# KarolinaBenkova/FEM-FCT-PDECO

Measured on AMD Instinct MI355X. Metric: FCT timesteps/sec (fwd+adj), higher is better.
Workload: dtype f64; 1 GPU; C2 advection_solidbody_FCT_PDECO_finaltime: [-1,1]^2 81x81 P1 (dx=0.025, n=6561), dt=1e-3, 250 fwd + 250 adj FCT steps per cost+gradient evaluation; nodes=6561, num_steps=250, batch_per_gpu=1, parallelism=single trajectory, low_order_solver=jacobi, jacobi_sweeps_max=26, graphs=True, graph_replay=True, kernel_regime=2

## Files before the change

fem-fct-pdeco_amd/_lib.py:

```python
from __future__ import annotations

import ctypes as C
import os

_HERE = os.path.dirname(os.path.abspath(__file__))
LIB_PATH = os.environ.get("FEMFCT_LIB") or os.path.join(_HERE, "lib", "libfemfct.so")

OK, ERR_INVALID, ERR_HIP, ERR_NOT_CONVERGED, ERR_NOMEM = 0, 1, 2, 3, 4
FLAG_MMATRIX_ROWSUM, FLAG_SOLVER_BUDGET, FLAG_COARSE_ITERS, FLAG_CHEBYSHEV, FLAG_ROW_PAIRS = 1, 2, 4, 8, 16
ORDER_VERTEX, ORDER_FENICS = 0, 1
SOLVER_JACOBI, SOLVER_BICGSTAB = 0, 1
REGIME_ROWS, REGIME_STRIPS, REGIME_TILE32, REGIME_PATCH64, REGIME_MESH = 0, 1, 2, 3, 4
ABI_VERSION = 5
MAX_TRIALS = 16
MAX_MEMBERS = 256
MAX_GRAM_FIELDS = 17
MAX_ZONES = 256


class FemFctError(RuntimeError):
    def __init__(self, code, msg):
        super().__init__(f"libfemfct error {code}: {msg}")
        self.code = code


class FemFctValueError(FemFctError, ValueError):
    pass


class NotConverged(FemFctError):
    pass


class StepInfo(C.Structure):
    _fields_ = [("flags", C.c_int32), ("solver_iters", C.c_int32),
                ("solver_resid", C.c_double), ("min_rowsum", C.c_double)]


def _load():
    if not os.path.exists(LIB_PATH):
        raise ImportError(
            f"{LIB_PATH} not found: the HIP library is not built. Run "
            "`python -c 'import __graft_entry__ as g; g.build()'` or "
            "`make -C fem-fct-pdeco_amd/csrc` (needs hipcc, --offload-arch=gfx950). "
            "There is no CPU fallback.")
    lib = C.CDLL(LIB_PATH)
    if lib.femfct_abi_version() != ABI_VERSION:
        raise ImportError("libfemfct.so ABI version mismatch: rebuild the library")
    return lib


lib = _load()

_p = C.c_void_p
_d = C.c_double
_i = C.c_int32
_dp = C.POINTER(C.c_double)
_ip = C.POINTER(C.c_int32)

SIGNATURES = {
    "femfct_abi_version": (C.c_int, []),
    "femfct_build_id": (C.c_char_p, []),
    "femfct_create": (C.c_int, [C.POINTER(_p), C.c_int]),
    "femfct_destroy": (C.c_int, [_p]),
    "femfct_last_error": (C.c_char_p, [_p]),
    "femfct_synchronize": (C.c_int, [_p]),
    "femfct_stream": (_p, [_p]),
    "femfct_set_solver": (C.c_int, [_p, C.c_int, _d, C.c_int]),
    "femfct_set_graphs": (C.c_int, [_p, C.c_int]),
    "femfct_graph_replay_active": (C.c_int, [_p, C.POINTER(C.c_int)]),
    "femfct_rotation_derived": (C.c_int, [_p, C.POINTER(C.c_int)]),
    "femfct_launch_info": (C.c_int, [_p, C.POINTER(C.c_int32)]),
    "femfct_set_fusion": (C.c_int, [_p, C.c_int, C.c_int]),
    "femfct_kernel_regime": (C.c_int, [_p, _i]),
    "femfct_patch_walkers": (C.c_int, [_p, _i, _i]),
    "femfct_lowop_nonzero_fraction": (C.c_int, [_p, _dp]),
    "femfct_set_profiling": (C.c_int, [_p, C.c_int]),
    "femfct_profile_report": (C.c_int, [_p, _p, _p, _i]),
    "femfct_malloc": (C.c_int, [_p, C.POINTER(_p), C.c_size_t]),
    "femfct_free": (C.c_int, [_p, _p]),
    "femfct_memcpy_h2d": (C.c_int, [_p, _p, _p, C.c_size_t]),
    "femfct_memcpy_d2h": (C.c_int, [_p, _p, _p, C.c_size_t]),
    "femfct_memcpy_d2d": (C.c_int, [_p, _p, _p, C.c_size_t]),
    "femfct_memset0": (C.c_int, [_p, _p, C.c_size_t]),
    "femfct_set_pattern_csr": (C.c_int, [_p, _i, _p, _p]),
    "femfct_set_mesh_square": (C.c_int, [_p, _d, _d, _i, _i]),
    "femfct_n": (_i, [_p]),
    "femfct_ell_width": (_i, [_p]),
    "femfct_get_ell_cols": (C.c_int, [_p, _p]),
    "femfct_csr_to_ell": (C.c_int, [_p, _p, _p]),
    "femfct_ell_to_csr": (C.c_int, [_p, _p, _p]),
    "femfct_set_mass": (C.c_int, [_p, _p, _p]),
    "femfct_mass_ell": (_p, [_p]),
    "femfct_stiffness_ell": (_p, [_p]),
    "femfct_lumped_mass": (_p, [_p]),
    "femfct_fct_step": (C.c_int, [_p, _p, _p, _i, _p, _p, _d, _p, _i]),
    "femfct_last_step_info": (C.c_int, [_p, C.POINTER(StepInfo), _i]),
    "femfct_fct_step_host": (C.c_int, [_p, _p, _p, _p, _p, _d, _p, C.POINTER(StepInfo)]),
    "femfct_chebsi": (C.c_int, [_p, _p, _p, _i, _d, _d, _i]),
    "femfct_chebsi_md": (C.c_int, [_p, _p, _p, _p, _i, _d, _d, _i]),
    "femfct_artificial_diffusion": (C.c_int, [_p, _p, _p, _i]),
    "femfct_spmv": (C.c_int, [_p, _p, _p, _d, _d, _p, _i]),
    "femfct_mesh_quad_points": (C.c_int, [_p, _p, _p]),
    "femfct_assemble_convection": (C.c_int, [_p, _p, _d, _p]),
    "femfct_assemble_rotation": (C.c_int, [_p, _d, _p]),
    "femfct_drift_gradient_rhs": (C.c_int, [_p, _p, _p, _p, _d, _d, _d, _p, _i]),
    "femfct_solidbody_forward": (C.c_int, [_p, _p, _p, _i, _p, _i, _d, _d, _d, _d, _d, _i]),
    "femfct_solidbody_forward_src": (C.c_int, [_p, _p, _p, _i, _p, _p, _i, _d, _d, _d, _d, _d, _i]),
    "femfct_solidbody_adjoint": (C.c_int, [_p, _p, _p, _i, _p, _p, _p, _i, _d, _d, _d, _d, _d, _i, _i]),
    "femfct_linear_forward_react": (C.c_int, [_p, _p, _p, _p, _p, _i, _d, _d, _i]),
    "femfct_linear_adjoint_react": (C.c_int, [_p, _p, _p, _p, _p, _p, _i, _d, _d, _i, _i]),
    "femfct_react_load": (C.c_int, [_p, _p, _p, _p, _p, _i]),
    "femfct_solidbody_adjoint_obs": (C.c_int, [_p, _p, _p, _i, _p, _p, _p, _d, _p, _p, _i, _d, _d, _d, _d, _d, _i]),
    "femfct_linear_adjoint_react_obs": (C.c_int, [_p, _p, _p, _p, _p, _p, _d, _p, _p, _i, _d, _d, _i]),
    "femfct_nonlinear_adjoint_obs": (C.c_int, [_p, _p, _p, _p, _p, _d, _p, _p, _i, _d, _d, _i]),
    "femfct_schnak_adjoint_obs": (C.c_int, [_p, _p, _p, _p, _p, _p, _p, _p, _d, _p, _d, _p, _p, _p, _i, _d, _p, _i]),
    "femfct_chtxs_adjoint_obs": (C.c_int, [_p, _p, _p, _p, _p, _p, _d, _p, _d, _p, _p, _p, _p, _i, _d, _p, _d, _p, _i, _i]),
    "femfct_obs_load": (C.c_int, [_p, _p, _p, _p, _i, _d, _p, _p, _i]),
    "femfct_obs_cost": (C.c_int, [_p, _p, _p, _p, _p, _i, _i, _p]),
    "femfct_solidbody_adjoint_bounds": (C.c_int, [_p, _p, _p, _i, _p, _p, _p, _d, _p, _p, _p, _d, _p, _p, _p, _i, _d, _d, _d,
                                                  _d, _d, _i]),
    "femfct_linear_adjoint_react_bounds": (C.c_int, [_p, _p, _p, _p, _p, _p, _d, _p, _p, _p, _d, _p, _p, _p, _i, _d, _d, _i]),
    "femfct_bound_load": (C.c_int, [_p, _p, _p, _p, _p, _i, _d, _p, _p, _p, _p, _p, _d, _p, _p, _i]),
    "femfct_bound_cost": (C.c_int, [_p, _p, _p, _p, _p, _d, _p, _i, _i, _p]),
    "femfct_assemble_weighted_mass": (C.c_int, [_p, _p, _p]),
    "femfct_traj_info": (C.c_int, [_p, C.POINTER(StepInfo), _i, _i]),
    "femfct_descent_pointwise": (C.c_int, [_p, C.c_int64, _d, _p, _d, _p, _p, _d, _p]),
    "femfct_ell_transpose": (C.c_int, [_p, _p, _p]),
    "femfct_axpby": (C.c_int, [_p, C.c_int64, _d, _p, _d, _p, _p]),
    "femfct_set_krylov": (C.c_int, [_p, _d, _i]),
    "femfct_set_species_solver": (C.c_int, [_p, _i]),
    "femfct_bicgstab": (C.c_int, [_p, _p, _i, _p, _p, _p, _i, C.POINTER(StepInfo)]),
    "femfct_nonlinear_forward": (C.c_int, [_p, _p, _p, _p, _i, _d, _d, _i]),
    "femfct_nonlinear_adjoint": (C.c_int, [_p, _p, _p, _p, _p, _i, _d, _d, _i]),
    "femfct_schnak_forward": (C.c_int, [_p, _p, _p, _p, _p, _i, _d, _p, _d, _i]),
    "femfct_schnak_adjoint": (C.c_int, [_p, _p, _p, _p, _p, _p, _p, _p, _i, _d, _p, _i, _i]),
    "femfct_schnak_forward_tw": (C.c_int, [_p, _p, _p, _p, _p, _p, _i, _d, _p, _d, _i]),
    "femfct_schnak_adjoint_tw": (C.c_int, [_p, _p, _p, _p, _p, _p, _p, _p, _p, _i, _d, _p, _i, _i]),
    "femfct_chtxs_forward": (C.c_int, [_p, _p, _p, _p, _i, _d, _p, _d, _i]),
    "femfct_nonlinear_forward_ct": (C.c_int, [_p, _p, _p, _i, _p, _i, _d, _d, _i]),
    "femfct_schnak_forward_ct": (C.c_int, [_p, _p, _p, _p, _i, _p, _p, _i, _d, _p, _d, _i]),
    "femfct_chtxs_forward_ct": (C.c_int, [_p, _p, _i, _p, _p, _i, _d, _p, _d, _i]),
    "femfct_chtxs_forward_g": (C.c_int, [_p, _p, _i, _i, _p, _p, _i, _d, _p, _d, _p, _i]),
    "femfct_chtxs_adjoint_g": (C.c_int, [_p, _p, _p, _p, _p, _p, _p, _p, _i, _d, _p, _d, _i, _p, _i]),
    "femfct_nonlinear_adjoint_alltime": (C.c_int, [_p, _p, _p, _p, _i, _p, _i, _d, _d, _i]),
    "femfct_chtxs_adjoint": (C.c_int, [_p, _p, _p, _p, _p, _p, _p, _p, _i, _d, _p, _d, _i, _i]),
    "femfct_traj_krylov_info": (C.c_int, [_p, C.POINTER(StepInfo), _i, _i]),
    "femfct_l2_norm_sq_Q": (C.c_int, [_p, _p, _p, _i, _d, _p, _i]),
    "femfct_l2_norm_sq_Omega": (C.c_int, [_p, _p, _p, _p, _i]),
    "femfct_cost_functional": (C.c_int, [_p, _p, _p, _p, _i, _i, _d, _d, _i, _p, _p, _p, _i]),
    "femfct_project_control": (C.c_int, [_p, _p, _d, _p, _d, _d, _p, C.c_int64]),
    "femfct_linear_trial_costs": (C.c_int, [_p, _p, _p, _p, _p, _p, _d, _i, _d, _d, _d, _i, _d, _i, _p, _p]),
    "femfct_source_trials": (C.c_int, [_p, _p, _p, _p, _d, _i, _d, _d, C.c_int64, _p, _p]),
    "femfct_trial_controls": (C.c_int, [_p, _p, _p, _p, _i, _i, _d, _d, C.c_int64, _p]),
    "femfct_member_costs": (C.c_int, [_p, _p, _p, _i, _p, _p, _p, _i, _i, _i, _d, _i, _p, _p]),
    "femfct_time_restrict": (C.c_int, [_p, _p, _p, _i, _i, _i, _p]),
    "femfct_time_prolong": (C.c_int, [_p, _p, _p, _i, _i, _i, _p]),
    "femfct_free_set": (C.c_int, [_p, _p, _p, _d, _d, C.c_int64, _p]),
    "femfct_q_gram": (C.c_int, [_p, _p, _i, _p, _i, _d, _p]),
    "femfct_q_combine": (C.c_int, [_p, _p, _p, _i, _p, _p, _d, C.c_int64, _p]),
    "femfct_prox_trials": (C.c_int, [_p, _p, _p, _p, _d, _i, _d, _d, _d, C.c_int64, _p, _p]),
    "femfct_l1_norm_Q": (C.c_int, [_p, _p, _i, _d, _p, _i]),
    "femfct_sparse_trial_stats": (C.c_int, [_p, _p, _p, _i, _i, _d, _p, _p, _p]),
    "femfct_ensemble_drift_gradient_rhs": (C.c_int, [_p, _p, _p, _p, _p, _i, _d, _d, _d, _p, _i]),
    "femfct_ensemble_costs": (C.c_int, [_p, _p, _p, _p, _p, _p, _p, _p, _i, _d, _i, _d, _p, _p, _p]),
    "femfct_initial_trials": (C.c_int, [_p, _p, _p, _p, _i, _d, _d, _p, _i]),
    "femfct_initial_trial_stats": (C.c_int, [_p, _p, _p, _p, _i, _i, _p]),
    "femfct_initial_gradient": (C.c_int, [_p, _p, _p, _p, _d, _p, _d, _d, _p]),
    "femfct_omega_gram": (C.c_int, [_p, _p, _i, _p, _p]),
    "femfct_set_control_zones": (C.c_int, [_p, _p, _i]),
    "femfct_zone_restrict": (C.c_int, [_p, _p, C.c_int64, _i, _p]),
    "femfct_zone_prolong": (C.c_int, [_p, _p, _p, C.c_int64, _p]),
    "femfct_smooth_cost": (C.c_int, [_p, _p, _i, _d, _p, _i]),
    "femfct_smooth_rhs": (C.c_int, [_p, _p, _d, _d, _i, _d, _p, _i]),
    "femfct_drift_gradient_rhs_smooth": (C.c_int, [_p, _p, _p, _p, _d, _d, _d, _d, _p, _i, _d, _d]),
}

for _name, (_res, _args) in SIGNATURES.items():
    _fn = getattr(lib, _name)
    _fn.restype = _res
    _fn.argtypes = _args


def check(ctx_handle, code):
    if code == OK:
        return
    msg = lib.femfct_last_error(ctx_handle)
    msg = msg.decode() if msg else ""
    if code == ERR_INVALID:
        raise FemFctValueError(code, msg)
    if code == ERR_NOT_CONVERGED:
        raise NotConverged(code, msg)
    raise FemFctError(code, msg)
```

fem-fct-pdeco_amd/csrc/ctx.hip:

```cpp
#include "femfct_internal.h"
#include "build_id.h"
#include "device_utils.h"

#include <dlfcn.h>
#include <stdarg.h>
#include <stdio.h>
#include <stdlib.h>
#include <string.h>
#include <algorithm>
#include <tuple>

int femfct_enqueue_artdiff(femfct_ctx* ctx, const double* K, double* D, int32_t batch);
int femfct_enqueue_spmv(femfct_ctx* ctx, const double* A, const double* x, double alpha, double beta, double* y,
                        int32_t batch);
int femfct_enqueue_cheb(femfct_ctx* ctx, const double* b, double* y_out, int iters, double lmin, double lmax,
                        int32_t batch, bool first_done_in_y1, const double* mdv = nullptr);
int femfct_mesh_release(femfct_ctx* ctx);
int femfct_build_structured_csr(femfct_ctx* ctx);

int femfct_fail(femfct_ctx* ctx, int code, const char* fmt, ...) {
    char buf[1024];
    va_list ap;
    va_start(ap, fmt);
    vsnprintf(buf, sizeof buf, fmt, ap);
// ... 87 lines not shown
    dev_free(&ctx->d_wscale); ctx->wscale_count = 0;
    dev_free(&ctx->d_zero_traj); ctx->zero_traj_count = 0;
    dev_free(&ctx->d_trMat); dev_free(&ctx->d_trBase); dev_free(&ctx->d_trBase2); dev_free(&ctx->d_trRhs2); dev_free(&ctx->d_trTmp);
    ctx->implicit_cols = false;
    ctx->n = 0; ctx->W = 0; ctx->nnz_csr = 0; ctx->ws_batch = 0; ctx->have_mass = false; ctx->structured = false; ctx->mass_is_mesh = false;
    ctx->sweep_budget = std::min(femfct_ctx().sweep_budget, ctx->max_iters);
    femfct_forget_jacobi_budgets(ctx);
}

void femfct_prof_begin(femfct_ctx* ctx, int cls) {
    if (!ctx->prof_on) return;
    femfct_ctx::ProfRec r;
    r.cls = cls;
    hipEventCreate(&r.a);
    hipEventCreate(&r.b);
    hipEventRecord(r.a, ctx->stream);
    ctx->prof.push_back(r);
}

void femfct_prof_end(femfct_ctx* ctx) {
    if (!ctx->prof_on || ctx->prof.empty()) return;
    hipEventRecord(ctx->prof.back().b, ctx->stream);
}

void femfct_drop_graphs(femfct_ctx* ctx) {
    for (auto& kv : ctx->graphs) hipGraphExecDestroy(kv.second);
    ctx->graphs.clear();
}

int femfct_ensure_workspace(femfct_ctx* ctx, int32_t batch) {
    if (ctx->solver == FEMFCT_SOLVER_BICGSTAB) {
        int rk = femfct_ensure_krylov_ws(ctx, batch);
        if (rk != FEMFCT_OK) return rk;
    }
#ifdef FEMFCT_TUNING
    if (!ctx->d_mesh_trace && getenv("FEMFCT_MESH_TRACE"))
        HIP_TRY(ctx, hipMalloc((void**)&ctx->d_mesh_trace, 16 * sizeof(unsigned long long)));
#endif
    if (!ctx->d_zero && ctx->n > 0) {
        int rz = dev_alloc(ctx, &ctx->d_zero, (size_t)ctx->n);
        if (rz != FEMFCT_OK) return rz;
        HIP_TRY(ctx, hipMemsetAsync(ctx->d_zero, 0, sizeof(double) * ctx->n, ctx->stream));
    }
    if (batch <= ctx->ws_batch) return FEMFCT_OK;
    femfct_drop_graphs(ctx);
    size_t nv = (size_t)batch * ctx->n, nm = nv * ctx->W;
    int rc;
#define A_(p, c) if ((rc = dev_alloc(ctx, &ctx->p, (c))) != FEMFCT_OK) return rc
    A_(d_L, nm + 1); A_(d_D, nm); A_(d_F, nm);
    HIP_TRY(ctx, hipMemsetAsync(ctx->d_L + nm, 0, sizeof(double), ctx->stream));
    A_(d_b, nv); A_(d_xa, nv); A_(d_xb, nv); A_(d_du, nv); A_(d_y0, nv); A_(d_y1, nv); A_(d_y2, nv);
    A_(d_rdu, nv); A_(d_rp, nv); A_(d_rm, nv);
    A_(d_part, (size_t)batch * 4 * FEMFCT_MAX_PARTIALS);
    A_(d_ctl, (size_t)batch);
    A_(d_partk, (size_t)batch * 16 * FEMFCT_MAX_PARTIALS);
    {
        const size_t words = ((size_t)batch * (size_t)ctx->n + 7) / 8 + 1;
        A_(d_Lmask, words);
        HIP_TRY(ctx, hipMemsetAsync(ctx->d_Lmask, 0, words * 8, ctx->stream));
    }
    {
        TilePlan tp;
        ctx->bigpart_count = 0;
        if (femfct_tile_plan(ctx, &tp, false) && femfct_tile_big(ctx, tp)) {
            ctx->bigpart_count = (int64_t)tp.tiles * tp.tiles;
            A_(d_bigpart, (size_t)batch * ctx->bigpart_count);
        }
    }
#undef A_
    HIP_TRY(ctx, hipMemsetAsync(ctx->d_ctl, 0, sizeof(StepCtl) * batch, ctx->stream));
    ctx->ws_batch = batch;
    return FEMFCT_OK;
}

static int fusion_mode(const femfct_ctx* ctx, int* K) {
    TilePlan tp;
    if (femfct_tile_plan(ctx, &tp, false)) {
        *K = tp.K;
        return femfct_tile_big(ctx, tp) ? 1 : 2;
    }
    StripPlan pl;
    if (femfct_strip_plan(ctx, &pl)) { *K = pl.K; return 1; }
    *K = 1;
    return 0;
}

int femfct_fused_k(const femfct_ctx* ctx) {
    int K;
    fusion_mode(ctx, &K);
    return K;
}

int femfct_next_budget(const femfct_ctx* ctx, int worst, bool coarse) {
    int K;
    const int mode = fusion_mode(ctx, &K);
    int b;
    if (mode == 2) b = std::max(worst, 1) + ((coarse || !ctx->exact_iters) ? 0 : 1);
    else if (mode == 1) b = std::max(worst, 1);
    else b = std::max(8, worst + worst / 8 + 2);
    return std::min(ctx->max_iters, b);
}

int femfct_grow_budget(const femfct_ctx* ctx, int budget) {
    int K;
    const int mode = fusion_mode(ctx, &K);
    if (mode == 2) return std::min(ctx->max_iters, budget + 2);
    if (mode == 1) return std::min(ctx->max_iters, budget + K);
    return std::min(ctx->max_iters, budget * 2);
}

int femfct_round_budget(const femfct_ctx* ctx, int b) {
    int K;
    if (fusion_mode(ctx, &K) == 0) b = (b + 3) & ~3;
    if (b < 1) b = 1;
    if (b > ctx->max_iters) b = ctx->max_iters;
    return b;
}

int femfct_install_pattern(femfct_ctx* ctx, int32_t n, int32_t W, const std::vector<int32_t>& cols,
                           const std::vector<uint8_t>& tslot) {
    int rc;
    ctx->n = n;
    ctx->W = W;
    if ((rc = dev_alloc(ctx, &ctx->d_cols, (size_t)W * n)) != FEMFCT_OK) return rc;
    if ((rc = dev_alloc(ctx, &ctx->d_tslot, (size_t)W * n)) != FEMFCT_OK) return rc;
    HIP_TRY(ctx, hipMemcpy(ctx->d_cols, cols.data(), sizeof(int32_t) * W * n, hipMemcpyHostToDevice));
    HIP_TRY(ctx, hipMemcpy(ctx->d_tslot, tslot.data(), sizeof(uint8_t) * W * n, hipMemcpyHostToDevice));
    if ((rc = dev_alloc(ctx, &ctx->d_M, (size_t)W * n)) != FEMFCT_OK) return rc;
    if ((rc = dev_alloc(ctx, &ctx->d_ml, (size_t)n)) != FEMFCT_OK) return rc;
    ctx->h_cols = cols;
    int32_t bwmax = 0;
    for (int32_t s = 1; s < W; ++s)
        for (int32_t i = 0; i < n; ++i) {
            int32_t d = cols[(size_t)s * n + i] - i;
            if (d < 0) d = -d;
            if (d > bwmax) bwmax = d;
        }
    ctx->bandwidth = bwmax;
    if (const char* e = getenv("FEMFCT_STRIPS")) ctx->use_strips = atoi(e) != 0;
    if (const char* e = getenv("FEMFCT_STRIP_K")) ctx->strip_k = atoi(e);
    if (const char* e = getenv("FEMFCT_TILES")) ctx->use_tiles = atoi(e) != 0;
    if (const char* e = getenv("FEMFCT_EXACT")) ctx->exact_iters = atoi(e) != 0;
    if (const char* e = getenv("FEMFCT_FUSE_BUILD")) ctx->fuse_build = atoi(e) != 0;
    if (const char* e = getenv("FEMFCT_PREASSEMBLE")) ctx->preassemble = atoi(e) != 0;
    if (const char* e = getenv("FEMFCT_PREASSEMBLE_MAX_GB")) ctx->preassemble_max_bytes = atof(e) * 1024.0 * 1024.0 * 1024.0;
    if (const char* e = getenv("FEMFCT_PREBUILD_LOW")) ctx->prebuild_low = atoi(e) != 0;
    if (const char* e = getenv("FEMFCT_WG_SLOTS")) ctx->wg_slots = std::max(1, atoi(e));
    if (const char* e = getenv("FEMFCT_DEEP_HALO")) ctx->deep_halo = atoi(e) != 0;
    if (const char* e = getenv("FEMFCT_FUSE_FLUX")) ctx->fuse_flux = atoi(e) != 0;
    if (const char* e = getenv("FEMFCT_FUSE_DUDT")) ctx->fuse_dudt = atoi(e) != 0;
    if (const char* e = getenv("FEMFCT_TILE_LEAN")) ctx->tile_lean = atoi(e) != 0;
    if (const char* e = getenv("FEMFCT_TILE_CONE")) ctx->tile_cone = atoi(e) != 0;
    if (const char* e = getenv("FEMFCT_TILE_FIT")) ctx->tile_fit = atoi(e) != 0;
    if (const char* e = getenv("FEMFCT_FUSE_END")) ctx->fuse_end = atoi(e) != 0;
    if (const char* e = getenv("FEMFCT_TILE4")) ctx->tile4_mode = atoi(e);
    if (const char* e = getenv("FEMFCT_LMASK")) ctx->l_mask = atoi(e) != 0;
    if (const char* e = getenv("FEMFCT_T4_XCD")) ctx->t4_xcd = atoi(e) != 0;
    if (const char* e = getenv("FEMFCT_T4_WALK")) ctx->t4_walk = atoi(e);
    if (const char* e = getenv("FEMFCT_T4_SNAKE")) ctx->t4_snake = atoi(e) != 0;
    if (const char* e = getenv("FEMFCT_T4_PAIR")) ctx->t4_pair = atoi(e) != 0;
#ifdef FEMFCT_TUNING
    if (const char* e = getenv("FEMFCT_PAIR_SHAPE")) ctx->pair_shape = atoi(e);
    if (const char* e = getenv("FEMFCT_PAIR_PRIO")) ctx->pair_prio = atoi(e);
    if (const char* e = getenv("FEMFCT_PAIR_SPLIT")) ctx->pair_split = std::min(90, std::max(10, atoi(e)));
    if (getenv("FEMFCT_PAIR_TRACE") && !ctx->d_pair_trace) {
        if (hipMalloc((void**)&ctx->d_pair_trace, sizeof(unsigned long long) * (FEMFCT_MAX_PARTIALS * 16 * 5 + 16)) == hipSuccess)
            hipMemset(ctx->d_pair_trace, 0, sizeof(unsigned long long) * (FEMFCT_MAX_PARTIALS * 16 * 5 + 16));
    }
    if (const char* e = getenv("FEMFCT_PAIR_STAGGER_US")) ctx->pair_stagger = (int)(atof(e) * 100.0);
#endif
    if (const char* e = getenv("FEMFCT_DEFER_CHECK")) ctx->defer_check = atoi(e) != 0;
    if (const char* e = getenv("FEMFCT_T4_INT")) ctx->t4_int = atoi(e) != 0;
    if (const char* e = getenv("FEMFCT_T4_WALKERS")) { int v = atoi(e); if (v > 0) ctx->num_cus = v; }
    if (const char* e = getenv("FEMFCT_INLINE_OPS")) ctx->inline_ops = atoi(e) != 0;
    if (const char* e = getenv("FEMFCT_HALF_D")) ctx->half_d = atoi(e) != 0;
    if (const char* e = getenv("FEMFCT_T4_STAGGER_US")) {
        const double us = atof(e);
        int pat = 7;
        if (const char* p = getenv("FEMFCT_T4_STAGGER_PAT")) pat = atoi(p);
        ctx->t4_stagger = us > 0 ? ((int)(us * 100.0) & 0xffffff) | ((pat & 15) << 24) : 0;
    }
    if (const char* e = getenv("FEMFCT_SINGLE_PATCH_BATCH")) { int v = atoi(e); ctx->single_patch_min_batch = v > 0 ? v : (1 << 30); }
    if (const char* e = getenv("FEMFCT_MESH_SOLVE")) ctx->mesh_solve = atoi(e) != 0;
    if (const char* e = getenv("FEMFCT_GEOM_MASS")) ctx->geom_mass = atoi(e) != 0;
    if (const char* e = getenv("FEMFCT_GEOM_ROT")) ctx->geom_rot = atoi(e) != 0;
    if (const char* e = getenv("FEMFCT_FORM_GROUPS")) ctx->form_groups = atoi(e) != 0;
    if (const char* e = getenv("FEMFCT_MESH_STEP")) ctx->mesh_step = atoi(e) != 0;
    if (const char* e = getenv("FEMFCT_MESH_STEP_BATCH")) ctx->mesh_step_min_batch = std::max(1, atoi(e));
    if (const char* e = getenv("FEMFCT_MESH_STEP_BATCH_LARGE")) ctx->mesh_step_min_batch_large = std::max(1, atoi(e));
    if (const char* e = getenv("FEMFCT_T4_DPP")) ctx->t4_dpp = atoi(e) != 0;
    if (const char* e = getenv("FEMFCT_T4_K")) ctx->t4_k = std::min(8, std::max(1, atoi(e)));
    if (const char* e = getenv("FEMFCT_SPECIES_SOLVER")) ctx->species_solver = atoi(e);
    if (const char* e = getenv("FEMFCT_STEPS_PER_GRAPH")) ctx->steps_per_graph = std::max(1, atoi(e));
    return femfct_strip_init(ctx);
}

static int build_csr_map(femfct_ctx* ctx) {
    const int32_t n = ctx->n, W = ctx->W;
    ctx->nnz_csr = ctx->h_indptr[n];
    ctx->h_csr2ell.assign(ctx->nnz_csr, 0);
    for (int32_t i = 0; i < n; ++i) {
        for (int32_t k = ctx->h_indptr[i]; k < ctx->h_indptr[i + 1]; ++k) {
            int32_t j = ctx->h_indices[k];
            int32_t s_found = -1;
            if (j == i) s_found = 0;
            else
                for (int32_t s = 1; s < W; ++s)
                    if (ctx->h_cols[(size_t)s * n + i] == j) { s_found = s; break; }
            if (s_found < 0) return femfct_fail(ctx, FEMFCT_ERR_INVALID, "CSR entry (%d,%d) not in the ELL pattern", i, j);
            ctx->h_csr2ell[k] = (int32_t)((size_t)s_found * n + i);
        }
    }
    int rc;
    if ((rc = dev_alloc(ctx, &ctx->d_csr2ell, (size_t)ctx->nnz_csr)) != FEMFCT_OK) return rc;
    HIP_TRY(ctx, hipMemcpy(ctx->d_csr2ell, ctx->h_csr2ell.data(), sizeof(int32_t) * ctx->nnz_csr, hipMemcpyHostToDevice));
    if ((rc = dev_alloc(ctx, &ctx->d_hcsr, (size_t)ctx->nnz_csr)) != FEMFCT_OK) return rc;
    return FEMFCT_OK;
}

extern "C" {

int femfct_abi_version(void) { return FEMFCT_ABI_VERSION; }
const char* femfct_build_id(void) { return FEMFCT_BUILD_ID; }

}

bool femfct_profiler_attached() {
    for (const char* name : {"librocprofiler-sdk.so.1", "librocprofiler-sdk.so"}) {
        if (void* h = dlopen(name, RTLD_LAZY | RTLD_NOLOAD)) {
            dlclose(h);
            return true;
        }
    }
    return false;
}

extern "C" {

int femfct_create(femfct_ctx** out, int device_id) {
    if (!out) return FEMFCT_ERR_INVALID;
    *out = nullptr;
    int count = 0;
    if (hipGetDeviceCount(&count) != hipSuccess || count <= 0) return FEMFCT_ERR_HIP;
    if (device_id < 0 || device_id >= count) return FEMFCT_ERR_INVALID;
    if (hipSetDevice(device_id) != hipSuccess) return FEMFCT_ERR_HIP;
    femfct_ctx* ctx = new (std::nothrow) femfct_ctx();
    if (!ctx) return FEMFCT_ERR_NOMEM;
    ctx->device = device_id;
    {
        int cus = 0;
        if (hipDeviceGetAttribute(&cus, hipDeviceAttributeMultiprocessorCount, device_id) == hipSuccess && cus > 0) ctx->num_cus = cus;
    }
    if (hipStreamCreateWithFlags(&ctx->stream, hipStreamNonBlocking) != hipSuccess) {
        delete ctx;
        return FEMFCT_ERR_HIP;
    }
    const char* pg = getenv("FEMFCT_PROFILER_GRAPHS");
    ctx->profiler_graphs_ok = pg && atoi(pg) != 0;
    if (!ctx->profiler_graphs_ok && femfct_profiler_attached()) ctx->graphs_blocked = true;
    *out = ctx;
    return FEMFCT_OK;
}

int femfct_graph_replay_active(const femfct_ctx* ctx, int* active_host) {
    if (!ctx || !active_host) return FEMFCT_ERR_INVALID;
    *active_host = (ctx->use_graphs && !ctx->prof_on && !ctx->graphs_blocked) ? 1 : 0;
    return FEMFCT_OK;
}

int femfct_rotation_derived(const femfct_ctx* ctx, int* derived_host) {
    if (!ctx || !derived_host) return FEMFCT_ERR_INVALID;
    *derived_host = ctx->last_rot_geom ? 1 : 0;
    return FEMFCT_OK;
}

int femfct_destroy(femfct_ctx* ctx) {
    if (!ctx) return FEMFCT_OK;
    hipSetDevice(ctx->device);
    hipStreamSynchronize(ctx->stream);
    if (ctx->d_pair_trace) {
        if (const char* path = getenv("FEMFCT_PAIR_TRACE")) {
            std::vector<unsigned long long> h((size_t)FEMFCT_MAX_PARTIALS * 16 * 5 + 16);
            if (hipMemcpy(h.data(), ctx->d_pair_trace, h.size() * sizeof(unsigned long long), hipMemcpyDeviceToHost) == hipSuccess)
                if (FILE* f = fopen(path, "wb")) { fwrite(h.data(), sizeof(unsigned long long), h.size(), f); fclose(f); }
        }
        hipFree(ctx->d_pair_trace);
        ctx->d_pair_trace = nullptr;
    }
#ifdef FEMFCT_TUNING
    if (const char* path = getenv("FEMFCT_TILE_TRACE")) femfct_tile_phase_dump(path);
#endif
    femfct_release_pattern(ctx);
    hipStreamDestroy(ctx->stream);
    delete ctx;
    return FEMFCT_OK;
}

const char* femfct_last_error(const femfct_ctx* ctx) { return ctx ? ctx->err.c_str() : "null context"; }

int femfct_synchronize(femfct_ctx* ctx) {
    FEMFCT_ENTER(ctx);
    ARG_TRY(ctx, ctx, "null ctx");
    HIP_TRY(ctx, hipStreamSynchronize(ctx->stream));
    return FEMFCT_OK;
}

void* femfct_stream(femfct_ctx* ctx) { return ctx ? (void*)ctx->stream : nullptr; }

int femfct_set_solver(femfct_ctx* ctx, int solver, double rel_tol, int max_iters) {
    FEMFCT_ENTER(ctx);
    ARG_TRY(ctx, ctx, "null ctx");
    ARG_TRY(ctx, solver == FEMFCT_SOLVER_JACOBI || solver == FEMFCT_SOLVER_BICGSTAB, "unknown solver");
    ARG_TRY(ctx, rel_tol > 0 && rel_tol < 1 && max_iters >= 1, "bad tolerance / iteration cap");
    ctx->solver = solver;
    ctx->solver_user = solver;
    femfct_forget_bicgstab_handovers(ctx);
    ctx->rel_tol = rel_tol;
    ctx->max_iters = max_iters;
    if (ctx->sweep_budget > max_iters) ctx->sweep_budget = max_iters;
    femfct_forget_jacobi_budgets(ctx);
    femfct_drop_graphs(ctx);
    return FEMFCT_OK;
}

int femfct_set_fusion(femfct_ctx* ctx, int strips, int tiles) {
    FEMFCT_ENTER(ctx);
    ARG_TRY(ctx, ctx, "null ctx");
    HIP_TRY(ctx, hipStreamSynchronize(ctx->stream));
    ctx->use_strips = strips != 0;
    ctx->use_tiles = tiles != 0;
    femfct_drop_graphs(ctx);
    femfct_forget_jacobi_budgets(ctx);
    ctx->ws_batch = 0;
    return FEMFCT_OK;
}

int femfct_kernel_regime(const femfct_ctx* ctx, int32_t batch) {
    if (!ctx || ctx->n <= 0) return -1;
    if (femfct_mesh_step_wanted(ctx, batch)) return FEMFCT_REGIME_MESH;
    if (femfct_tile4_wanted(ctx, batch)) return FEMFCT_REGIME_PATCH64;
    TilePlan tp;
    if (ctx->use_strips && femfct_tile_plan(ctx, &tp, true, 0, batch)) return FEMFCT_REGIME_TILE32;
    StripPlan sp;
    if (femfct_strip_plan(ctx, &sp)) return FEMFCT_REGIME_STRIPS;
    return FEMFCT_REGIME_ROWS;
}

int femfct_patch_walkers(const femfct_ctx* ctx, int32_t batch, int32_t sweeps) {
    if (!ctx || ctx->n <= 0 || batch < 1 || !femfct_tile4_wanted(ctx, batch) || femfct_single_patch(ctx, batch)) return 0;
    return femfct_tile4_walkers(ctx, femfct_tile4_halo(ctx, sweeps > 0 ? sweeps : 36), batch, false);
}

int femfct_launch_info(const femfct_ctx* ctx, int32_t* out4_host) {
    if (!ctx || !out4_host) return FEMFCT_ERR_INVALID;
    for (int k = 0; k < 4; ++k) out4_host[k] = ctx->last_launch[k];
    return FEMFCT_OK;
}

int femfct_lowop_nonzero_fraction(femfct_ctx* ctx, double* fraction_host) {
    FEMFCT_ENTER(ctx);
    ARG_TRY(ctx, fraction_host, "null argument");
    *fraction_host = 1.0;
    if (!ctx->d_Lmask || ctx->n <= 0 || !ctx->l_mask || !femfct_tile4_wanted(ctx, 1) || !ctx->t4_dpp ||
        ctx->solver != FEMFCT_SOLVER_JACOBI)
        return FEMFCT_OK;
    unsigned long long* d_cnt = nullptr;
    HIP_TRY(ctx, hipMalloc((void**)&d_cnt, sizeof(unsigned long long)));
    hipLaunchKernelGGL(k_mask_popcount, dim3(1), dim3(256), 0, ctx->stream, (int64_t)ctx->n, ctx->d_Lmask + 1, d_cnt);
    unsigned long long cnt = 0;
    HIP_TRY(ctx, hipMemcpyAsync(&cnt, d_cnt, sizeof cnt, hipMemcpyDeviceToHost, ctx->stream));
    HIP_TRY(ctx, hipStreamSynchronize(ctx->stream));
    hipFree(d_cnt);
    *fraction_host = (double)cnt / (6.0 * (double)ctx->n);
    return FEMFCT_OK;
}

int femfct_set_graphs(femfct_ctx* ctx, int enable) {
    FEMFCT_ENTER(ctx);
    ARG_TRY(ctx, ctx, "null ctx");
    ctx->use_graphs = enable != 0;
    if (!enable) femfct_drop_graphs(ctx);
    return FEMFCT_OK;
}

int femfct_set_profiling(femfct_ctx* ctx, int enable) {
    FEMFCT_ENTER(ctx);
    ARG_TRY(ctx, ctx, "null ctx");
    HIP_TRY(ctx, hipStreamSynchronize(ctx->stream));
    for (auto& r : ctx->prof) { hipEventDestroy(r.a); hipEventDestroy(r.b); }
    ctx->prof.clear();
    ctx->prof_on = enable != 0;
    return FEMFCT_OK;
}

int femfct_profile_report(femfct_ctx* ctx, double* total_ms_host, int32_t* launches_host, int32_t n_classes) {
    FEMFCT_ENTER(ctx);
    ARG_TRY(ctx, ctx && total_ms_host && launches_host && n_classes >= KC_COUNT, "need >= 8 classes");
    HIP_TRY(ctx, hipStreamSynchronize(ctx->stream));
    for (int k = 0; k < n_classes; ++k) { total_ms_host[k] = 0.0; launches_host[k] = 0; }
    for (auto& r : ctx->prof) {
        float ms = 0.f;
        if (hipEventElapsedTime(&ms, r.a, r.b) == hipSuccess) {
            total_ms_host[r.cls] += ms;
            launches_host[r.cls] += 1;
        }
        hipEventDestroy(r.a);
        hipEventDestroy(r.b);
    }
    ctx->prof.clear();
    return FEMFCT_OK;
}

int femfct_malloc(femfct_ctx* ctx, void** dev_ptr, size_t bytes) {
    FEMFCT_ENTER(ctx);
    ARG_TRY(ctx, ctx && dev_ptr, "null argument");
    HIP_TRY(ctx, hipSetDevice(ctx->device));
    hipError_t e = hipMalloc(dev_ptr, bytes ? bytes : 8);
    if (e != hipSuccess) return femfct_fail(ctx, FEMFCT_ERR_NOMEM, "hipMalloc(%zu) failed: %s", bytes, hipGetErrorString(e));
    return FEMFCT_OK;
}
int femfct_free(femfct_ctx* ctx, void* p) {
    FEMFCT_ENTER(ctx);
    ARG_TRY(ctx, ctx, "null ctx");
    HIP_TRY(ctx, hipStreamSynchronize(ctx->stream));
    HIP_TRY(ctx, hipFree(p));
    return FEMFCT_OK;
}
int femfct_memcpy_h2d(femfct_ctx* ctx, void* d, const void* h, size_t bytes) {
    FEMFCT_ENTER(ctx);
    ARG_TRY(ctx, ctx && (bytes == 0 || (d && h)), "null argument");
    HIP_TRY(ctx, hipMemcpyAsync(d, h, bytes, hipMemcpyHostToDevice, ctx->stream));
    HIP_TRY(ctx, hipStreamSynchronize(ctx->stream));
    return FEMFCT_OK;
}
int femfct_memcpy_d2h(femfct_ctx* ctx, void* h, const void* d, size_t bytes) {
    FEMFCT_ENTER(ctx);
    ARG_TRY(ctx, ctx && (bytes == 0 || (d && h)), "null argument");
    HIP_TRY(ctx, hipMemcpyAsync(h, d, bytes, hipMemcpyDeviceToHost, ctx->stream));
    HIP_TRY(ctx, hipStreamSynchronize(ctx->stream));
    return FEMFCT_OK;
}
int femfct_memcpy_d2d(femfct_ctx* ctx, void* d, const void* s, size_t bytes) {
    FEMFCT_ENTER(ctx);
    ARG_TRY(ctx, ctx && (bytes == 0 || (d && s)), "null argument");
    HIP_TRY(ctx, hipMemcpyAsync(d, s, bytes, hipMemcpyDeviceToDevice, ctx->stream));
    return FEMFCT_OK;
}
int femfct_memset0(femfct_ctx* ctx, void* d, size_t bytes) {
    FEMFCT_ENTER(ctx);
    ARG_TRY(ctx, ctx && (bytes == 0 || d), "null argument");
    HIP_TRY(ctx, hipMemsetAsync(d, 0, bytes, ctx->stream));
    return FEMFCT_OK;
}

int femfct_set_pattern_csr(femfct_ctx* ctx, int32_t n, const int32_t* indptr, const int32_t* indices) {
    FEMFCT_ENTER(ctx);
    ARG_TRY(ctx, ctx && indptr && indices && n > 0, "null/empty pattern");
    HIP_TRY(ctx, hipSetDevice(ctx->device));
    HIP_TRY(ctx, hipStreamSynchronize(ctx->stream));
    femfct_release_pattern(ctx);
    ARG_TRY(ctx, indptr[0] == 0, "indptr[0] must be 0");
    int32_t W = 1;
    for (int32_t i = 0; i < n; ++i) {
        ARG_TRY(ctx, indptr[i + 1] >= indptr[i], "indptr not monotone");
        int32_t len = 0;
        bool diag = false;
        for (int32_t k = indptr[i]; k < indptr[i + 1]; ++k) {
            int32_t j = indices[k];
            ARG_TRY(ctx, j >= 0 && j < n, "column index out of range");
            if (j == i) diag = true; else ++len;
        }
        ARG_TRY(ctx, diag, "pattern must contain the full diagonal");
        W = std::max(W, len + 1);
    }
    if (W > FEMFCT_MAX_W) return femfct_fail(ctx, FEMFCT_ERR_INVALID, "row with %d entries exceeds FEMFCT_MAX_W=%d", W, FEMFCT_MAX_W);
    std::vector<int32_t> cols((size_t)W * n);
    std::vector<uint8_t> tslot((size_t)W * n);
    for (int32_t s = 0; s < W; ++s)
        for (int32_t i = 0; i < n; ++i) { cols[(size_t)s * n + i] = i; tslot[(size_t)s * n + i] = (uint8_t)s; }
    for (int32_t i = 0; i < n; ++i) {
        int32_t s = 1;
        for (int32_t k = indptr[i]; k < indptr[i + 1]; ++k) {
            int32_t j = indices[k];
            if (j == i) continue;
            for (int32_t q = 1; q < s; ++q)
                ARG_TRY(ctx, cols[(size_t)q * n + i] != j, "duplicate column in a row");
            cols[(size_t)s * n + i] = j;
            ++s;
        }
    }
    for (int32_t i = 0; i < n; ++i)
        for (int32_t s = 1; s < W; ++s) {
            int32_t j = cols[(size_t)s * n + i];
            if (j == i) continue;
            int32_t ts = -1;
            for (int32_t q = 1; q < W; ++q)
                if (cols[(size_t)q * n + j] == i) { ts = q; break; }
            if (ts < 0) return femfct_fail(ctx, FEMFCT_ERR_INVALID, "pattern not symmetric: (%d,%d) has no transpose", i, j);
            tslot[(size_t)s * n + i] = (uint8_t)ts;
        }
    int rc = femfct_install_pattern(ctx, n, W, cols, tslot);
    if (rc != FEMFCT_OK) return rc;
    ctx->h_indptr.assign(indptr, indptr + n + 1);
    ctx->h_indices.assign(indices, indices + indptr[n]);
    return build_csr_map(ctx);
}

int32_t femfct_n(const femfct_ctx* ctx) { return ctx ? ctx->n : 0; }
// ... 185 lines not shown
```

fem-fct-pdeco_amd/csrc/femfct_internal.h:

```cpp
#pragma once

#include <hip/hip_runtime.h>
#include <stdint.h>
#include <string.h>
#include <string>
#include <vector>
#include <map>
#include <tuple>

#include "../../include/femfct.h"

#define FEMFCT_MAX_W 16
#ifndef FEMFCT_MAX_PARTIALS
#define FEMFCT_MAX_PARTIALS 2048
#endif

struct StepCtl {
    int32_t flags;
    int32_t iters;
    int32_t done;
    int32_t parity;
    double  resid;
    double  bnorm;
    double  min_rowsum;
    double  rs[2];
    double  pad;
};

enum SweepKind {
    SWEEP_SOLIDBODY_FORWARD = 2, SWEEP_SOLIDBODY_ADJOINT = 3,
    SWEEP_NONLINEAR_FORWARD = 10, SWEEP_NONLINEAR_ADJOINT = 11,
    SWEEP_SCHNAK_FORWARD = 12, SWEEP_SCHNAK_ADJOINT = 13,
    SWEEP_CHTXS_FORWARD = 14, SWEEP_CHTXS_ADJOINT = 15,
    SWEEP_NONLINEAR_ADJOINT_ALLTIME = 16,
};

struct SweepKindState {
    int budget = 48;
    int good = 0;
    int fail = 0;
    int mesh_cap = 0;
    int cheb_budget = 40;
    int bicg_budget = 40;
    bool full_rows = false;
    bool low_bicg = false;
    bool cheb_off = false;
};

struct femfct_ctx {
    int device = 0;
    hipStream_t stream = nullptr;
    std::string err;

    int32_t n = 0;
    int32_t W = 0;
    int64_t nnz_csr = 0;
    int32_t* d_cols = nullptr;
    uint8_t* d_tslot = nullptr;
    int32_t* d_csr2ell = nullptr;
    std::vector<int32_t> h_indptr, h_indices, h_csr2ell, h_cols;
    bool structured = false;
    bool mass_is_mesh = false;
    double a1 = 0, a2 = 0, h = 0;
    int32_t n_cells = 0, N = 0, order = 0;
    int32_t* d_d2v = nullptr;

    double* d_M = nullptr;
    double* d_Ad = nullptr;
    double* d_ml = nullptr;
    bool have_mass = false;

    int solver = FEMFCT_SOLVER_JACOBI;
    int solver_user = FEMFCT_SOLVER_JACOBI;
    double rel_tol = 1e-13;
    int max_iters = 400;
    int sweep_budget = 48;
    std::map<int, SweepKindState> kinds;
    bool use_graphs = true;
    bool graphs_blocked = false;
    int graph_captures = 0;
    bool profiler_graphs_ok = false;
    int32_t steps_per_graph = 50;
    bool use_strips = true;
    bool use_tiles = true;
    bool mesh_solve = true;
    bool mesh_solve_attr[8] = {false, false, false, false, false, false, false, false};
    int single_patch_min_batch = 8;
    bool form_groups = true;
    bool geom_rot = true;
    double rot_om = 0.0;
    bool rot_om_set = false;
    int* d_rot_check = nullptr;
    bool last_rot_geom = false;
    bool geom_mass = true;
    bool t4_dpp = true;
    int t4_k = 8;
    int t4_snake = 1;
    bool t4_pair = true;
    int pair_stagger = 0;
    int32_t last_launch[4] = {0, 0, 0, 0};
    unsigned long long* d_pair_trace = nullptr;
    int pair_prio = 0, pair_split = 50;
    int pair_shape = 5;
    bool pair_rows = false;
    bool mesh_step = true;
    int mesh_step_min_batch = 1;
    int mesh_step_min_batch_large = 64;
    bool mesh_step_attr[6] = {false, false, false, false, false, false};
    double* d_zero = nullptr;
    unsigned long long* d_mesh_trace = nullptr;
    int defer_check = 1;
    int t4_int = 1;
    int t4_walk = 1;
    int num_cus = 256;
    int t4_xcd = 0;
    int t4_stagger = 600 | (7 << 24);
    int tile4_mode = 1;
    bool fuse_end = true;
    bool fuse_build = true;
    int wg_slots = 256;
    bool deep_halo = true;
    bool fuse_flux = true;
    bool fuse_dudt = true;
    int tile_lean = 1;
    int tile_cone = 0;
    int tile_fit = 1;
    bool exact_iters = false;
    int32_t bandwidth = 0;
    int32_t strip_k = 0;
    bool implicit_cols = false;

    int32_t ws_batch = 0;
    double *d_L = nullptr, *d_D = nullptr, *d_F = nullptr;
    double *d_b = nullptr, *d_xa = nullptr, *d_xb = nullptr;
    double *d_du = nullptr, *d_y0 = nullptr, *d_y1 = nullptr, *d_y2 = nullptr, *d_rdu = nullptr;
    double *d_rp = nullptr, *d_rm = nullptr;
    double *d_part = nullptr;
    StepCtl* d_ctl = nullptr;
    double* d_partk = nullptr;
    double* d_bigpart = nullptr;
    unsigned long long* d_Lmask = nullptr;
    bool half_d = true;
    bool inline_ops = true;
    bool l_mask = true;
    int64_t bigpart_count = 0;
    double *d_hA = nullptr, *d_hN = nullptr, *d_hrhs = nullptr, *d_hu = nullptr, *d_hout = nullptr, *d_hcsr = nullptr;

    typedef std::vector<uint64_t> GraphKey;
    std::map<GraphKey, hipGraphExec_t> graphs;

    int32_t tr_batch = 0, tr_steps = 0;
    double* d_trAall = nullptr;
    size_t trAall_count = 0;
    bool preassemble = true;
    double preassemble_max_bytes = 16.0 * 1024 * 1024 * 1024;
    bool prebuild_low = true;
    double* d_lowall = nullptr;
    size_t lowall_count = 0, low_doff = 0;
    const double* low_src = nullptr;
    double low_dt = 0.0;
    double *d_trA = nullptr, *d_trN = nullptr, *d_trRhs = nullptr;
    int32_t* d_level = nullptr;
    StepCtl* d_log = nullptr;
    unsigned* d_ticket = nullptr;
    int level_bias = 0, ord_bias = 0, rep_total = 1;
    bool rep_last = true;
    int end_req_delta = 0;
    bool end_req_krylov = false, end_fused = false;
    std::vector<StepCtl> h_log;
    int32_t log_steps = 0, log_batch = 0;

    bool prof_on = false;
    struct ProfRec { int cls; hipEvent_t a, b; };
    std::vector<ProfRec> prof;

    int32_t kry_batch = 0;
    double* d_kry = nullptr;
    double* d_kry_part = nullptr;
    void* d_kry_ctl = nullptr;
    void* d_kry_ctl2 = nullptr;
    double kry_tol = 1e-13;
    int kry_max_iters = 2000;
    int kry_budget = 40;
    void* d_klog = nullptr;
    int species_solver = 0;
    double* d_chs_om = nullptr;
    double* d_chs_scale = nullptr;
    int chs_om_cap = 0;
    std::vector<char> h_klog;
    double *d_trMat = nullptr, *d_trBase = nullptr, *d_trBase2 = nullptr;
    double *d_trRhs2 = nullptr, *d_trTmp = nullptr;
    double* d_wscale = nullptr;
    size_t wscale_count = 0;
    double* d_zero_traj = nullptr;
    size_t zero_traj_count = 0;

    double* d_scratch = nullptr;
    size_t scratch_count = 0;
    int32_t* d_ttab = nullptr;
    size_t ttab_count = 0;
    std::vector<int32_t> h_ttab;
    int32_t* d_ztab = nullptr;
    int32_t zn_m = 0, zn_items = 0, zn_nparts = 0, zn_listed = 0, zn_maxlen = 0;
};

int femfct_fail(femfct_ctx* ctx, int code, const char* fmt, ...);
#define HIP_TRY(ctx, expr)                                                          \
    do {                                                                            \
        hipError_t _e = (expr);                                                     \
        if (_e != hipSuccess)                                                       \
            return femfct_fail((ctx), FEMFCT_ERR_HIP, "%s failed: %s (%s:%d)", #expr, \
                               hipGetErrorString(_e), __FILE__, __LINE__);          \
    } while (0)
#define ARG_TRY(ctx, cond, msg)                                                     \
    do {                                                                            \
        if (!(cond)) return femfct_fail((ctx), FEMFCT_ERR_INVALID, "%s", msg);      \
    } while (0)

#define FEMFCT_ENTER(ctx)                                                           \
    do {                                                                            \
        if (!(ctx)) return FEMFCT_ERR_INVALID;                                      \
        HIP_TRY((ctx), hipSetDevice((ctx)->device));                                \
    } while (0)

int femfct_ensure_workspace(femfct_ctx* ctx, int32_t batch);
int femfct_ensure_krylov_ws(femfct_ctx* ctx, int32_t batch);
void femfct_drop_graphs(femfct_ctx* ctx);
void femfct_release_pattern(femfct_ctx* ctx);
int femfct_round_budget(const femfct_ctx* ctx, int b);
#define FEMFCT_INTERNAL __attribute__((visibility("hidden")))
FEMFCT_INTERNAL void femfct_forget_jacobi_budgets(femfct_ctx* ctx);
FEMFCT_INTERNAL void femfct_forget_bicgstab_handovers(femfct_ctx* ctx);
FEMFCT_INTERNAL void femfct_forget_cheb_off(femfct_ctx* ctx);
FEMFCT_INTERNAL int femfct_ensure_scratch(femfct_ctx* ctx, size_t doubles);
FEMFCT_INTERNAL void femfct_enqueue_reduce_levels(femfct_ctx* ctx, int32_t batch, int levels, int G, const double* partial,
                                                  int trapezoid, double scale, int accumulate, double* out_dev);

static inline uint64_t key_bits(const void* p) { return (uint64_t)(uintptr_t)p; }
static inline uint64_t key_bits(double d) { uint64_t u; memcpy(&u, &d, 8); return u; }
static inline uint64_t key_bits(int64_t v) { return (uint64_t)v; }
static inline uint64_t key_bits(int32_t v) { return (uint64_t)(int64_t)v; }
template <class F>
int femfct_run_graph(femfct_ctx* ctx, const femfct_ctx::GraphKey& key, F&& enqueue);

static inline bool femfct_tiles_usable(const femfct_ctx* ctx) {
    return ctx->use_strips && ctx->use_tiles && ctx->implicit_cols && ctx->W == 7;
}

struct StripPlan { int K, R, bw, rpt, S; };
bool femfct_strip_plan(const femfct_ctx* ctx, StripPlan* pl);
int femfct_strip_init(femfct_ctx* ctx);
int femfct_enqueue_strip_jacobi(femfct_ctx* ctx, const StripPlan& pl, const double* L, const double* b, double* xa,
                                double* xb, int launch, int g_build, int32_t batch);
int femfct_enqueue_strip_cheb(femfct_ctx* ctx, const StripPlan& pl, const double* b, const double* in_mid,
                              const double* in_old, double* y_out, int k_first, int k_last, const double* omegas,
                              double md_scale, double* bufA0, double* bufA1, double* bufB0, double* bufB1,
                              int32_t batch);

struct TilePlan { int tiles, K, H; };
bool femfct_tile_plan(const femfct_ctx* ctx, TilePlan* pl, bool need_partials = true, int budget = 0, int batch = 1);
bool femfct_tile_big(const femfct_ctx* ctx, const TilePlan& pl);
bool femfct_cheb_flux_fusable(const femfct_ctx* ctx, int32_t batch);
bool femfct_tile_fit(const femfct_ctx* ctx, int32_t batch);
#ifdef FEMFCT_TUNING
void femfct_tile_phase_dump(const char* path);
#endif
bool femfct_geom_mass(const femfct_ctx* ctx);
int femfct_enqueue_tile_build_jacobi(femfct_ctx* ctx, const TilePlan& pl, struct MatRef A, const double* Nm, int32_t nshared,
                                     struct VecRef rhs, int64_t rhs_bstride, struct VecRef u_n, int64_t u_bstride, double dt,
                                     int32_t batch, bool pre = false);
int femfct_enqueue_low_seq(femfct_ctx* ctx, const double* A, double* L, double* D, int32_t entries, double dt);
int femfct_enqueue_tile_jacobi(femfct_ctx* ctx, const TilePlan& pl, const double* L, const double* b, double* xa,
                               double* xb, int launch, int g_build, int32_t batch, bool last, int bn_launch = 0, int defer = 0);
__attribute__((visibility("hidden"))) void femfct_launch_reduce_resid(femfct_ctx* ctx, int64_t count, int launch, int32_t batch);
int femfct_enqueue_tile_dudt_cheb(femfct_ctx* ctx, struct MatRef A, struct VecRef rhs, int64_t rhs_bstride, double* ulow,
                                  int budget_units, int part_count, int iters_per_unit, int exact_k, int iters,
                                  const double* omegas, double md_scale, int32_t batch, int* tail_first = nullptr);
int femfct_enqueue_tile_cheb(femfct_ctx* ctx, const TilePlan& pl, const double* b, const double* in_mid,
                             const double* in_old, double* y_out, int k_first, int k_last, const double* omegas,
                             double md_scale, double* bufA0, double* bufA1, double* bufB0, double* bufB1, int32_t batch,
                             const struct ChebIO* io = nullptr);
int femfct_enqueue_tile_cheb_flux_limit(femfct_ctx* ctx, const double* b, const double* in_mid, const double* in_old,
                                        int k_first, int k_last, const double* omegas, double md_scale, struct MatRef D,
                                        const double* ulow, double dt, struct VecRef out, int64_t out_bstride, int32_t batch,
                                        bool fuse_end);
int femfct_enqueue_tile_flux_limit(femfct_ctx* ctx, const double* D, const double* ulow, const double* du, double dt,
                                   struct VecRef out, int64_t out_bstride, int32_t batch, bool* fuse_end_io, int half_d = 0);

bool femfct_tile4_wanted(const femfct_ctx* ctx, int32_t batch);
bool femfct_single_patch(const femfct_ctx* ctx, int32_t batch);
int femfct_tile4_tiles(const femfct_ctx* ctx, int H = 8);
int femfct_tile4_halo(const femfct_ctx* ctx, int sweeps);
int femfct_tile4_walkers(const femfct_ctx* ctx, int H, int32_t batch, bool pair);
bool femfct_jacobi_pair_wanted(const femfct_ctx* ctx, int H, int32_t batch, bool have_lmask, bool assume_upwind_rows = false);
int femfct_tile4_init(femfct_ctx* ctx);
int femfct_enqueue_tile4_jacobi(femfct_ctx* ctx, const double* L, const double* b, double* xa, double* xb, int launch,
                                int g_build, int32_t batch, int H = 8, int K = 8, int check_every = 0,
                                const uint8_t* lmask = nullptr);
int femfct_enqueue_tile4_cheb(femfct_ctx* ctx, const double* b, const double* in_mid, const double* in_old, double* y_out,
                              int k_first, int k_last, const double* omegas, double md_scale, double* bufA0, double* bufA1,
                              double* bufB0, double* bufB1, int32_t batch,
                              const struct ChebIO* io = nullptr);

bool femfct_rotation_is_geometric(femfct_ctx* ctx, const double* Arot, double* om_out);
bool femfct_jacobi_plan(const femfct_ctx* ctx, int budget, int batch, int* K, int* launches);
bool femfct_mesh_step_wanted(const femfct_ctx* ctx, int32_t batch, bool have_nm = false);
int femfct_enqueue_mesh_step(femfct_ctx* ctx, struct MatRef A, const double* Nm, int32_t nshared, struct VecRef rhs,
                             int64_t rhs_bstride, struct VecRef u_n, int64_t u_bstride, double dt, struct VecRef u_out,
                             int64_t out_bstride, int32_t batch, int32_t budget, bool fuse_end);
int femfct_fused_k(const femfct_ctx* ctx);
int femfct_next_budget(const femfct_ctx* ctx, int worst_iters, bool coarse = false);
int femfct_grow_budget(const femfct_ctx* ctx, int budget);

enum { KC_BUILD_LOW = 0, KC_JACOBI, KC_DUDT_RHS, KC_CHEB, KC_FLUX, KC_LIMIT, KC_ASSEMBLE, KC_OTHER, KC_COUNT };
void femfct_prof_begin(femfct_ctx* ctx, int cls);
void femfct_prof_end(femfct_ctx* ctx);

struct LaunchGeom { dim3 grid; dim3 block; };
LaunchGeom femfct_geom(const femfct_ctx* ctx, int32_t batch);

int femfct_enqueue_step(femfct_ctx* ctx, const double* A, const double* N, int32_t nshared,
                        const double* rhs, const double* u_n, double dt, double* u_out,
                        int32_t batch, int32_t budget);

bool femfct_profiler_attached();

template <class F>
int femfct_run_graph(femfct_ctx* ctx, const femfct_ctx::GraphKey& key, F&& enqueue) {
    if (!ctx->use_graphs || ctx->prof_on || ctx->graphs_blocked) return enqueue();
    auto it = ctx->graphs.find(key);
    if (it == ctx->graphs.end()) {
        if (!ctx->profiler_graphs_ok && femfct_profiler_attached()) {
            ctx->graphs_blocked = true;
            return enqueue();
        }
        if (ctx->graphs.size() > 64) femfct_drop_graphs(ctx);
        ++ctx->graph_captures;
        hipGraph_t graph = nullptr;
        HIP_TRY(ctx, hipStreamBeginCapture(ctx->stream, hipStreamCaptureModeThreadLocal));
        int rc = enqueue();
        hipError_t e = hipStreamEndCapture(ctx->stream, &graph);
        if (rc != FEMFCT_OK) { if (graph) hipGraphDestroy(graph); return rc; }
        if (e != hipSuccess) return femfct_fail(ctx, FEMFCT_ERR_HIP, "hipStreamEndCapture: %s", hipGetErrorString(e));
        hipGraphExec_t exec = nullptr;
        e = hipGraphInstantiate(&exec, graph, nullptr, nullptr, 0);
        hipGraphDestroy(graph);
        if (e != hipSuccess) return femfct_fail(ctx, FEMFCT_ERR_HIP, "hipGraphInstantiate: %s", hipGetErrorString(e));
        it = ctx->graphs.emplace(key, exec).first;
    }
    HIP_TRY(ctx, hipGraphLaunch(it->second, ctx->stream));
    return FEMFCT_OK;
}
```

fem-fct-pdeco_amd/csrc/kernels_step.hip:

```cpp
#include "femfct_internal.h"
#include "device_utils.h"
#include "solve_ctl.h"
#include "forms.h"
#include "solidbody_op.h"

#include <math.h>
#include <stdlib.h>

namespace {



template <int IMP>
__device__ __forceinline__ unsigned nb_mask(int i, int Nw) {
    if (!IMP) return 0u;
    const int iy = i / Nw, ix = i - iy * Nw;
    const unsigned e = ix < Nw - 1, w = ix > 0, nn = iy < Nw - 1, ss = iy > 0;
    return (e << 1) | ((e & nn) << 2) | (nn << 3) | (w << 4) | ((w & ss) << 5) | (ss << 6);
}

template <int IMP>
__device__ __forceinline__ int col_of(const int32_t* __restrict__ cols, int n, int Nw, unsigned mask, int s, int i) {
    if (IMP) {
        const int off = (s == 1) ? 1 : (s == 2) ? Nw + 1 : (s == 3) ? Nw : (s == 4) ? -1 : (s == 5) ? -Nw - 1 : -Nw;
// ... 433 lines not shown
    const int64_t moff = (int64_t)blockIdx.y * W * n, voff = (int64_t)blockIdx.y * n;
    const double* A = A_ + moff;
    const double* x = x_ + voff;
    double* y = y_ + voff;
    RowRange rr = block_rows(n);
    for (int i = rr.begin + threadIdx.x; i < rr.end; i += blockDim.x) {
        double acc = A[i] * x[i];
        for (int s = 1; s < W; ++s) {
            int64_t idx = (int64_t)s * n + i;
            acc += A[idx] * x[cols[idx]];
        }
        y[i] = (beta != 0.0) ? alpha * acc + beta * y[i] : alpha * acc;
    }
}

}

LaunchGeom femfct_geom(const femfct_ctx* ctx, int32_t batch) {
    int bs = (ctx->n <= 65536) ? 64 : 256;
    if (const char* e = getenv("FEMFCT_BLOCK")) { int v = atoi(e); if (v == 64 || v == 256) bs = v; }
    int64_t g = ((int64_t)ctx->n + bs - 1) / bs;
    if (g > FEMFCT_MAX_PARTIALS) g = FEMFCT_MAX_PARTIALS;
    if (g < 1) g = 1;
    return LaunchGeom{dim3((unsigned)g, (unsigned)batch, 1), dim3((unsigned)bs, 1, 1)};
}

static void cheb_omegas(int iters, double lmin, double lmax, std::vector<double>& om) {
    double rho = (lmax - lmin) / (lmax + lmin);
    double w = 0.0;
    om.resize(iters);
    for (int k = 1; k <= iters; ++k) {
        if (k == 2) w = 1.0 / (1.0 - rho * rho / 2.0);
        else w = 1.0 / (1.0 - (w * rho * rho) / 4.0);
        om[k - 1] = w;
    }
}

#define LAUNCH_W(cls, kern, geom, stream, ...)                                                          \
    do {                                                                                                \
        femfct_prof_begin(ctx, cls);                                                                    \
        if (ctx->W == 7 && ctx->implicit_cols) {                                                        \
            if (geom.block.x == 64) hipLaunchKernelGGL((kern<7, 64, 1>), geom.grid, geom.block, 0, stream, __VA_ARGS__);  \
            else hipLaunchKernelGGL((kern<7, 256, 1>), geom.grid, geom.block, 0, stream, __VA_ARGS__);   \
        } else if (ctx->W == 7) {                                                                       \
            if (geom.block.x == 64) hipLaunchKernelGGL((kern<7, 64, 0>), geom.grid, geom.block, 0, stream, __VA_ARGS__);  \
            else hipLaunchKernelGGL((kern<7, 256, 0>), geom.grid, geom.block, 0, stream, __VA_ARGS__);   \
        } else {                                                                                        \
            if (geom.block.x == 64) hipLaunchKernelGGL((kern<0, 64, 0>), geom.grid, geom.block, 0, stream, __VA_ARGS__);  \
            else hipLaunchKernelGGL((kern<0, 256, 0>), geom.grid, geom.block, 0, stream, __VA_ARGS__);   \
        }                                                                                               \
        femfct_prof_end(ctx);                                                                           \
    } while (0)

int femfct_enqueue_cheb(femfct_ctx* ctx, const double* b, double* y_out, int iters, double lmin, double lmax,
                        int32_t batch, bool first_done_in_y1, const double* mdv = nullptr) {
    LaunchGeom g = femfct_geom(ctx, batch);
    std::vector<double> om;
    cheb_omegas(iters, lmin, lmax, om);
    const double md_scale = (lmin + lmax) / 2.0;
    if (mdv) {
        double* bufv[3] = {ctx->d_y0, ctx->d_y1, ctx->d_y2};
        for (int k = 1; k <= iters; ++k) {
            const double* mid = (k >= 2) ? bufv[(k - 1) % 3] : nullptr;
            const double* old = (k >= 3) ? bufv[(k - 2) % 3] : nullptr;
            double* out = (k == iters) ? y_out : bufv[k % 3];
            LAUNCH_W(KC_CHEB, k_cheb, g, ctx->stream, ctx->n, ctx->W, ctx->N, ctx->d_cols, ctx->d_M, b, mid, old, out, om[k - 1],
                     md_scale, mdv);
        }
        return FEMFCT_OK;
    }
    if (femfct_tile4_wanted(ctx, batch)) {
        if (first_done_in_y1)
            return femfct_enqueue_tile4_cheb(ctx, b, ctx->d_y1, nullptr, y_out, 2, iters, om.data(), md_scale, ctx->d_y0,
                                             ctx->d_y2, ctx->d_y1, ctx->d_rp, batch);
        return femfct_enqueue_tile4_cheb(ctx, b, nullptr, nullptr, y_out, 1, iters, om.data(), md_scale, ctx->d_y0,
                                         ctx->d_y2, ctx->d_y1, ctx->d_rp, batch);
    }
    TilePlan tp;
    if (femfct_tile_plan(ctx, &tp, false)) {
        if (first_done_in_y1)
            return femfct_enqueue_tile_cheb(ctx, tp, b, ctx->d_y1, nullptr, y_out, 2, iters, om.data(), md_scale,
                                            ctx->d_y0, ctx->d_y2, ctx->d_y1, ctx->d_rp, batch);
        return femfct_enqueue_tile_cheb(ctx, tp, b, nullptr, nullptr, y_out, 1, iters, om.data(), md_scale, ctx->d_y0,
                                        ctx->d_y2, ctx->d_y1, ctx->d_rp, batch);
    }
    StripPlan pl;
    if (femfct_strip_plan(ctx, &pl)) {
        if (first_done_in_y1)
            return femfct_enqueue_strip_cheb(ctx, pl, b, ctx->d_y1, nullptr, y_out, 2, iters, om.data(), md_scale,
                                             ctx->d_y0, ctx->d_y2, ctx->d_y1, ctx->d_rp, batch);
        return femfct_enqueue_strip_cheb(ctx, pl, b, nullptr, nullptr, y_out, 1, iters, om.data(), md_scale, ctx->d_y0,
                                         ctx->d_y2, ctx->d_y1, ctx->d_rp, batch);
    }
    double* buf[3] = {ctx->d_y0, ctx->d_y1, ctx->d_y2};
    int n = ctx->n, W = ctx->W;
    for (int k = 1; k <= iters; ++k) {
        if (k == 1 && first_done_in_y1) continue;
        const double* mid = (k >= 2) ? buf[(k - 1) % 3] : nullptr;
        const double* old = (k >= 3) ? buf[(k - 2) % 3] : nullptr;
        double* out = (k == iters) ? y_out : buf[k % 3];
        LAUNCH_W(KC_CHEB, k_cheb, g, ctx->stream, n, W, ctx->N, ctx->d_cols, ctx->d_M, b, mid, old, out, om[k - 1], md_scale,
                 (const double*)nullptr);
    }
    return FEMFCT_OK;
}

int femfct_enqueue_step_mat(femfct_ctx* ctx, MatRef A, const double* N, int32_t nshared, VecRef rhs, int64_t rhs_bstride,
                            VecRef u_n, int64_t u_bstride, double dt, VecRef u_out, int64_t out_bstride, int32_t batch,
                            int32_t budget);

int femfct_enqueue_step_ref(femfct_ctx* ctx, const double* A, const double* N, int32_t nshared, VecRef rhs,
                            int64_t rhs_bstride, VecRef u_n, int64_t u_bstride, double dt, VecRef u_out,
                            int64_t out_bstride, int32_t batch, int32_t budget) {
    return femfct_enqueue_step_mat(ctx, MatRef{A, nullptr, 0, 0, (int64_t)ctx->W * ctx->n}, N, nshared, rhs, rhs_bstride, u_n,
                                   u_bstride, dt, u_out, out_bstride, batch, budget);
}

int femfct_enqueue_step_op(femfct_ctx* ctx, MatRef A, const SbOpArgs* sb, const double* N, int32_t nshared, VecRef rhs,
                           int64_t rhs_bstride, VecRef u_n, int64_t u_bstride, double dt, VecRef u_out,
                           int64_t out_bstride, int32_t batch, int32_t budget);

bool femfct_inline_ops_wanted(const femfct_ctx* ctx, int32_t batch) {
    if (femfct_mesh_step_wanted(ctx, batch)) return false;
    return ctx->inline_ops && ctx->structured && ctx->implicit_cols && ctx->W == 7 && femfct_tile4_wanted(ctx, batch);
}

int femfct_enqueue_step_mat(femfct_ctx* ctx, MatRef A, const double* N, int32_t nshared, VecRef rhs,
                            int64_t rhs_bstride, VecRef u_n, int64_t u_bstride, double dt, VecRef u_out,
                            int64_t out_bstride, int32_t batch, int32_t budget) {
    return femfct_enqueue_step_op(ctx, A, nullptr, N, nshared, rhs, rhs_bstride, u_n, u_bstride, dt, u_out, out_bstride, batch,
                                  budget);
}

int femfct_enqueue_step_op(femfct_ctx* ctx, MatRef A, const SbOpArgs* sb, const double* N, int32_t nshared, VecRef rhs,
                           int64_t rhs_bstride, VecRef u_n, int64_t u_bstride, double dt, VecRef u_out,
                           int64_t out_bstride, int32_t batch, int32_t budget) {
    if (sb && (!femfct_inline_ops_wanted(ctx, batch) || N))
        return femfct_fail(ctx, FEMFCT_ERR_INVALID, "inline solid-body operator outside its regime");
    if (!sb && femfct_mesh_step_wanted(ctx, batch, N != nullptr)) {
        const bool fuse_end = ctx->end_req_delta != 0 && ctx->d_ticket && ctx->d_level && ctx->d_log && !ctx->prof_on;
        int r = femfct_enqueue_mesh_step(ctx, A, N, nshared, rhs, rhs_bstride, u_n, u_bstride, dt, u_out, out_bstride, batch,
                                         budget, fuse_end);
        if (r == FEMFCT_OK && fuse_end) ctx->end_fused = true;
        return r;
    }
    LaunchGeom g = femfct_geom(ctx, batch);
    hipStream_t st = ctx->stream;
    int n = ctx->n, W = ctx->W;
    StripPlan pl;
    TilePlan tp;
    const bool tiles = femfct_tile_plan(ctx, &tp, false, budget, batch) && (!femfct_tile_big(ctx, tp) || ctx->d_bigpart);
    const bool strips = !tiles && femfct_strip_plan(ctx, &pl);
    int units = budget, part_count = 0, ipu = 1, exact_k = 0;
    const bool tile4 = tiles && femfct_tile4_wanted(ctx, batch);
    const bool fused_build = ctx->fuse_build && tiles && !tile4 && !femfct_tile_big(ctx, tp) &&
                             ctx->solver != FEMFCT_SOLVER_BICGSTAB && (budget + tp.K - 1) / tp.K >= 2;
    uint8_t* lmask = (tile4 && ctx->l_mask && ctx->t4_dpp && W == 7 && ctx->solver == FEMFCT_SOLVER_JACOBI)
                         ? reinterpret_cast<uint8_t*>(ctx->d_Lmask + 1) : nullptr;
    const int half_d = (tile4 && ctx->half_d && ctx->structured && ctx->implicit_cols && W == 7) ? 1 : 0;
    MatRef L_pre = A, D_pre{ctx->d_D, nullptr, 0, 0, (int64_t)W * n};
    const bool pre_low = fused_build && !N && A.level && A.base == ctx->low_src && dt == ctx->low_dt && ctx->fuse_dudt &&
                         femfct_cheb_flux_fusable(ctx, batch);
    if (pre_low) {
        L_pre.base = ctx->d_lowall;
        D_pre = A;
        D_pre.base = ctx->d_lowall + ctx->low_doff;
    }
    if (sb) {
        femfct_prof_begin(ctx, KC_BUILD_LOW);
        if (sb->rot_geom)
            hipLaunchKernelGGL((k_build_low_sb<256, true>), g.grid, dim3(256), 0, st, n, ctx->N, ctx->h, *sb, rhs, u_n, rhs_bstride,
                               u_bstride, ctx->d_ml, dt, ctx->d_L, ctx->d_D, ctx->d_b, ctx->d_xa, ctx->d_part, ctx->d_ctl, lmask, half_d);
        else
            hipLaunchKernelGGL((k_build_low_sb<256, false>), g.grid, dim3(256), 0, st, n, ctx->N, ctx->h, *sb, rhs, u_n, rhs_bstride,
                               u_bstride, ctx->d_ml, dt, ctx->d_L, ctx->d_D, ctx->d_b, ctx->d_xa, ctx->d_part, ctx->d_ctl, lmask, half_d);
        femfct_prof_end(ctx);
    } else if (!fused_build)
        LAUNCH_W(KC_BUILD_LOW, k_build_low, g, st, n, W, ctx->N, ctx->d_cols, ctx->d_tslot, A, N, nshared, rhs, u_n,
                 rhs_bstride, u_bstride, ctx->d_ml, dt, ctx->d_L, ctx->d_D, ctx->d_b, ctx->d_xa, ctx->d_part, ctx->d_ctl,
                 lmask, half_d);
    if (ctx->solver == FEMFCT_SOLVER_BICGSTAB) {
        int r = femfct_enqueue_bicgstab(ctx, ctx->d_L, 0, ctx->d_b, make_ref(ctx->d_xa), n, make_ref(ctx->d_xa), n, batch,
                                        budget, true);
        if (r != FEMFCT_OK) return r;
        femfct_enqueue_kry_to_stepctl(ctx, (int)g.grid.x, batch);
        units = 0;
    } else if (tile4) {
        const bool single = femfct_single_patch(ctx, batch);
        const int h4 = femfct_tile4_halo(ctx, budget);
        const int t4 = femfct_tile4_tiles(ctx, h4);
        const bool big4 = (int64_t)t4 * t4 > FEMFCT_MAX_PARTIALS;
        const int k4 = single ? budget : std::min(ctx->t4_k == 8 ? h4 : ctx->t4_k, h4);
        units = (budget + k4 - 1) / k4;
        const bool pair4 = !single && femfct_jacobi_pair_wanted(ctx, h4, batch, lmask != nullptr);
        const int walkers = single ? 0 : femfct_tile4_walkers(ctx, h4, batch, pair4);
        part_count = walkers > 0 ? walkers : big4 ? -1 : t4 * t4;
        ipu = k4;
        for (int s = 0; s < units; ++s)
            femfct_enqueue_tile4_jacobi(ctx, ctx->d_L, ctx->d_b, ctx->d_xa, ctx->d_xb, s, (int)g.grid.x, batch, h4, k4,
                                        single ? 2 : 0, lmask);
    } else if (tiles) {
        units = (budget + tp.K - 1) / tp.K;
        part_count = femfct_tile_big(ctx, tp) ? -1 : tp.tiles * tp.tiles;
        ipu = tp.K;
        exact_k = (femfct_tile_big(ctx, tp) || !ctx->exact_iters) ? 0 : tp.K;
        const bool defer = ctx->defer_check && fused_build && units >= 2 && units <= 4 && exact_k == 0 && ctx->fuse_dudt;
        if (defer) exact_k = -units;
        if (fused_build) {
            int r = femfct_enqueue_tile_build_jacobi(ctx, tp, pre_low ? L_pre : A, N, nshared, rhs, rhs_bstride, u_n, u_bstride,
                                                     dt, batch, pre_low);
            if (r != FEMFCT_OK) return r;
        }
        for (int s = fused_build ? 1 : 0; s < units; ++s)
            femfct_enqueue_tile_jacobi(ctx, tp, ctx->d_L, ctx->d_b, ctx->d_xa, ctx->d_xb, s,
                                       fused_build ? tp.tiles * tp.tiles : (int)g.grid.x, batch,
                                       exact_k > 0 && s == units - 1, fused_build ? 1 : 0, defer ? 1 : 0);
    } else if (strips) {
        units = (budget + pl.K - 1) / pl.K;
        part_count = pl.S;
        ipu = pl.K;
        for (int s = 0; s < units; ++s)
            femfct_enqueue_strip_jacobi(ctx, pl, ctx->d_L, ctx->d_b, ctx->d_xa, ctx->d_xb, s, (int)g.grid.x, batch);
    } else {
        for (int s = 0; s < budget; ++s)
            LAUNCH_W(KC_JACOBI, k_jacobi, g, st, n, W, ctx->N, ctx->d_cols, ctx->d_L, ctx->d_b, ctx->d_xa, ctx->d_xb,
                     ctx->d_part, ctx->d_ctl, s, ctx->rel_tol);
    }
    double* ulow = ctx->d_b;
    bool step_done = false;
    if (tiles && !tile4 && !femfct_tile_big(ctx, tp) && ctx->fuse_dudt) {
        std::vector<double> om;
        cheb_omegas(20, 0.5, 2.0, om);
        int tail = 0;
        const bool fuse_tail = femfct_cheb_flux_fusable(ctx, batch);
        femfct_enqueue_tile_dudt_cheb(ctx, A, rhs, rhs_bstride, ulow, units, part_count, ipu, exact_k, 20, om.data(), 1.25,
                                      batch, fuse_tail ? &tail : nullptr);
        if (fuse_tail && tail > 0) {
            const bool fuse_end = ctx->end_req_delta != 0 && ctx->d_ticket && ctx->d_level && ctx->d_log && !ctx->prof_on;
            int r = femfct_enqueue_tile_cheb_flux_limit(ctx, ctx->d_rdu, ctx->d_y0, ctx->d_y2, tail, 20, om.data(), 1.25,
                                                        D_pre, ulow, dt, u_out, out_bstride, batch, fuse_end);
            if (r != FEMFCT_OK) return r;
            if (fuse_end) ctx->end_fused = true;
            step_done = true;
        } else if (fuse_tail) {
            return femfct_fail(ctx, FEMFCT_ERR_INVALID, "fused Chebyshev tail: nothing left to fuse");
        }
    } else {
        if (sb) {
            femfct_prof_begin(ctx, KC_DUDT_RHS);
            if (sb->rot_geom)
                hipLaunchKernelGGL((k_dudt_rhs_sb<256, true>), g.grid, dim3(256), 0, st, n, ctx->N, ctx->h, *sb, rhs, rhs_bstride,
                                   ctx->d_M, ctx->d_xa, ctx->d_xb, ulow, ctx->d_rdu, ctx->d_y1, ctx->d_part, ctx->d_ctl, units,
                                   part_count, ipu, ctx->rel_tol, 1.25, 1.0, (const double*)nullptr, 0);
            else
                hipLaunchKernelGGL((k_dudt_rhs_sb<256, false>), g.grid, dim3(256), 0, st, n, ctx->N, ctx->h, *sb, rhs, rhs_bstride,
                                   ctx->d_M, ctx->d_xa, ctx->d_xb, ulow, ctx->d_rdu, ctx->d_y1, ctx->d_part, ctx->d_ctl, units,
                                   part_count, ipu, ctx->rel_tol, 1.25, 1.0, (const double*)nullptr, 0);
            femfct_prof_end(ctx);
        } else {
            LAUNCH_W(KC_DUDT_RHS, k_dudt_rhs, g, st, n, W, ctx->N, ctx->d_cols, A, rhs, rhs_bstride, ctx->d_M, ctx->d_xa,
                     ctx->d_xb, ulow, ctx->d_rdu, ctx->d_y1, ctx->d_part, ctx->d_ctl, units, part_count, ipu, ctx->rel_tol,
                     1.25, 1.0, exact_k ? ctx->d_partk : nullptr, exact_k);
        }
        femfct_enqueue_cheb(ctx, ctx->d_rdu, ctx->d_du, 20, 0.5, 2.0, batch, true);
    }
    if (step_done) {
    } else if (tiles) {
        bool fuse_end = ctx->end_req_delta != 0 && ctx->d_ticket && ctx->d_level && ctx->d_log && !ctx->prof_on;
        femfct_enqueue_tile_flux_limit(ctx, ctx->d_D, ulow, ctx->d_du, dt, u_out, out_bstride, batch, &fuse_end, half_d);
        if (fuse_end) ctx->end_fused = true;
    } else {
        LAUNCH_W(KC_FLUX, k_flux, g, st, n, W, ctx->N, ctx->d_cols, ctx->d_M, ctx->d_D, ulow, ctx->d_du, ctx->d_ml, dt,
                 ctx->d_F, ctx->d_rp, ctx->d_rm);
        LAUNCH_W(KC_LIMIT, k_limit, g, st, n, W, ctx->N, ctx->d_cols, ctx->d_F, ctx->d_rp, ctx->d_rm, ulow, ctx->d_ml, dt,
                 u_out, out_bstride);
    }
    hipError_t e = hipGetLastError();
    if (e != hipSuccess) return femfct_fail(ctx, FEMFCT_ERR_HIP, "kernel launch failed: %s", hipGetErrorString(e));
    return FEMFCT_OK;
}

bool femfct_jacobi_plan(const femfct_ctx* ctx, int budget, int batch, int* K, int* launches) {
    TilePlan tp;
    if (!femfct_tile_plan(ctx, &tp, false, budget, batch)) return false;
    if (femfct_tile4_wanted(ctx, batch) && femfct_single_patch(ctx, batch)) {
        *K = budget;
    } else if (femfct_tile4_wanted(ctx, batch)) {
        const int h4 = femfct_tile4_halo(ctx, budget);
        *K = std::min(ctx->t4_k == 8 ? h4 : ctx->t4_k, h4);
    } else {
        *K = tp.K;
    }
    *launches = (budget + *K - 1) / *K;
    return true;
}

int femfct_enqueue_step(femfct_ctx* ctx, const double* A, const double* N, int32_t nshared, const double* rhs,
                        const double* u_n, double dt, double* u_out, int32_t batch, int32_t budget) {
    return femfct_enqueue_step_ref(ctx, A, N, nshared, make_ref(rhs), ctx->n, make_ref(u_n), ctx->n, dt,
                                   make_ref(u_out), ctx->n, batch, budget);
}

int femfct_enqueue_artdiff(femfct_ctx* ctx, const double* K, double* D, int32_t batch) {
    LaunchGeom g = femfct_geom(ctx, batch);
    hipLaunchKernelGGL(k_artdiff, g.grid, g.block, 0, ctx->stream, ctx->n, ctx->W, ctx->d_cols, ctx->d_tslot, K, D);
    return FEMFCT_OK;
}

int femfct_enqueue_spmv(femfct_ctx* ctx, const double* A, const double* x, double alpha, double beta, double* y,
                        int32_t batch) {
    LaunchGeom g = femfct_geom(ctx, batch);
    hipLaunchKernelGGL(k_spmv, g.grid, g.block, 0, ctx->stream, ctx->n, ctx->W, ctx->d_cols, A, x, alpha, beta, y);
    return FEMFCT_OK;
}
```

fem-fct-pdeco_amd/csrc/kernels_tile32.hip:

```cpp
#include "femfct_internal.h"
#include "device_utils.h"
#include "solve_ctl.h"
#include "forms.h"
#include "step_end.h"
#include "sweep_common.h"

#include <math.h>

#define TILE_T 16
#define TILE_H 8
#define TILE_L 32
#define TILE_LD 33
#define TILE_HMAX 13

namespace {

#ifdef FEMFCT_TUNING
__device__ unsigned long long g_tile_phase[4][4];
#define TILE_STAMP_BEGIN()                                                                                              \
    unsigned long long ts0_ = 0, ts1_ = 0;                                                                              \
    const bool ts_on_ = threadIdx.x == 0 && blockIdx.z == 0 && blockIdx.x == gridDim.x / 2 && blockIdx.y == gridDim.x / 2; \
    if (ts_on_) ts0_ = __builtin_amdgcn_s_memrealtime()
#define TILE_STAMP_LOADED() do { if (ts_on_) { __builtin_amdgcn_s_waitcnt(0); ts1_ = __builtin_amdgcn_s_memrealtime(); } } while (0)
#define TILE_STAMP_END(id) do { if (ts_on_) {                                                                           \
        const unsigned long long ts2_ = __builtin_amdgcn_s_memrealtime();                                               \
        g_tile_phase[id][0] += ts1_ - ts0_; g_tile_phase[id][1] += ts2_ - ts0_; g_tile_phase[id][2] += 1; } } while (0)
#else
#define TILE_STAMP_BEGIN() do { } while (0)
#define TILE_STAMP_LOADED() do { } while (0)
#define TILE_STAMP_END(id) do { } while (0)
#endif

struct TileGeom {
    int lx, ly, gx, gy, i;
    bool inside, owned;
    int kvalid;
    int nb[6];
    int self;
};

template <int T = TILE_T, int H = TILE_H, int PL = TILE_L>
__device__ __forceinline__ TileGeom tile_geom(int N) {
    static_assert(T + 2 * H == PL, "patch edge = tile + 2 halos");
    constexpr int PLD = PL + 1;
    TileGeom g;
    g.lx = threadIdx.x % PL;
    g.ly = threadIdx.x / PL;
    const int x0 = blockIdx.x * T - H, y0 = blockIdx.y * T - H;
    g.gx = x0 + g.lx;
    g.gy = y0 + g.ly;
    g.inside = g.gx >= 0 && g.gx < N && g.gy >= 0 && g.gy < N;
    g.i = g.inside ? g.gy * N + g.gx : 0;
    g.owned = g.inside && g.lx >= H && g.lx < H + T && g.ly >= H && g.ly < H + T;
    int kv = 1 << 20;
    if (x0 > 0) kv = min(kv, g.lx);
    if (x0 + PL - 1 < N - 1) kv = min(kv, PL - 1 - g.lx);
    if (y0 > 0) kv = min(kv, g.ly);
    if (y0 + PL - 1 < N - 1) kv = min(kv, PL - 1 - g.ly);
    g.kvalid = g.inside ? kv : 0;
    const int dx[6] = {1, 1, 0, -1, -1, 0}, dy[6] = {0, 1, 1, 0, -1, -1};
    g.self = g.ly * PLD + g.lx;
#pragma unroll
    for (int s = 0; s < 6; ++s) {
        int nx = min(max(g.lx + dx[s], 0), PL - 1), ny = min(max(g.ly + dy[s], 0), PL - 1);
        g.nb[s] = ny * PLD + nx;
    }
    if (PL * PL % WAVE != 0 && threadIdx.x >= PL * PL) {
        g.inside = g.owned = false;
        g.i = 0;
        g.kvalid = 0;
        g.self = 0;
    }
    return g;
}

template <int PL>
__device__ __forceinline__ bool tile_spare() {
    return PL * PL % WAVE != 0 && threadIdx.x >= PL * PL;
}

template <int H, int PL = TILE_L>
__device__ __forceinline__ int tile_dist(const TileGeom& g) {
    constexpr int T = PL - 2 * H;
    const int ddx = max(max(H - g.lx, g.lx - (H + T - 1)), 0), ddy = max(max(H - g.ly, g.ly - (H + T - 1)), 0);
    return max(ddx, ddy);
}

template <int H, int PL = TILE_L>
__device__ __forceinline__ int tile_hexdist(const TileGeom& g) {
    constexpr int T = PL - 2 * H;
    const int ex = g.lx - min(max(g.lx, H), H + T - 1), ey = g.ly - min(max(g.ly, H), H + T - 1);
    return max(max(abs(ex), abs(ey)), abs(ex - ey));
}

template <int H, int LEAN, int PL = TILE_L>
__device__ __forceinline__ int lean_dist(const TileGeom& g) {
    if constexpr (LEAN == 2) return tile_hexdist<H, PL>(g);
    else return tile_dist<H, PL>(g);
}

struct LeanAddr {
    const double* n0[6];
    double* me0;
};

template <int PL>
__device__ __forceinline__ LeanAddr lean_addr(double (*bufs)[PL * (PL + 1)], const TileGeom& g) {
    LeanAddr a;
    a.me0 = &bufs[0][g.self];
#pragma unroll
    for (int s = 0; s < 6; ++s) a.n0[s] = &bufs[0][g.nb[s]];
    return a;
}

template <int BUF, int LAST>
__device__ __forceinline__ void lean_jacobi_sweep(const LeanAddr& a, bool live, bool owned, const double* lv, double dg,
                                                  double rdg, double bv, double& xo, double& rmax) {
    constexpr int RD = BUF * TILE_L * TILE_LD, WR = (1 - BUF) * TILE_L * TILE_LD;
    if (live) {
        double acc = bv;
#pragma unroll
        for (int s = 0; s < 6; ++s) acc = fma(-lv[s], a.n0[s][RD], acc);
        if (LAST && owned) rmax = nan_max(rmax, fabs(acc - dg * xo));
        xo = acc * rdg;
        a.me0[WR] = xo;
    }
    __syncthreads();
}

__device__ __forceinline__ double lean_jacobi(const LeanAddr& a, int klive, int K, bool owned, const double* lv, double dg,
                                              double rdg, double bv, double xi, double& rmax) {
    double xo = xi;
    int k = 0;
    for (; k + 2 < K; k += 2) {
        lean_jacobi_sweep<0, 0>(a, k < klive, owned, lv, dg, rdg, bv, xo, rmax);
        lean_jacobi_sweep<1, 0>(a, k + 1 < klive, owned, lv, dg, rdg, bv, xo, rmax);
    }
    if (k + 1 < K) {
        lean_jacobi_sweep<0, 0>(a, k < klive, owned, lv, dg, rdg, bv, xo, rmax);
        lean_jacobi_sweep<1, 1>(a, k + 1 < klive, owned, lv, dg, rdg, bv, xo, rmax);
    } else if (k < K) {
        lean_jacobi_sweep<0, 1>(a, k < klive, owned, lv, dg, rdg, bv, xo, rmax);
    }
    return xo;
}

template <int BUF, int PL = TILE_L>
__device__ __forceinline__ void lean_cheb_iter(const LeanAddr& a, bool live, const double* mv, double md, double rmd, double bv,
                                               double wk, double& ym, double& yo) {
    constexpr int RD = BUF * PL * (PL + 1), WR = (1 - BUF) * PL * (PL + 1);
    if (live) {
        double acc = md * ym;
#pragma unroll
        for (int s = 0; s < 6; ++s) acc = fma(mv[s], a.n0[s][RD], acc);
        const double z = (bv - acc) * rmd;
        const double yn = wk * (z + ym - yo) + yo;
        yo = ym;
        ym = yn;
        a.me0[WR] = yn;
    }
    __syncthreads();
}

template <int H, int EXACT, int BIG, int LEAN>
__global__ void __launch_bounds__(STRIP_T)
k_tile_jacobi(int n, int N, const double* __restrict__ L_, const double* __restrict__ b_, double* __restrict__ xa_,
              double* __restrict__ xb_, double* __restrict__ part, StepCtl* __restrict__ ctl_, int launch, int K,
              int g_build, double rel_tol, double* __restrict__ bigpart, double* __restrict__ partk, int bn_launch,
              int defer) {
    constexpr int W = 7;
    __shared__ double xs[2][TILE_L * TILE_LD];
    __shared__ double smem[96];
    const int bz = blockIdx.z;
    StepCtl* ctl = ctl_ + bz;
    if (!defer && ctl->done) return;
    double* p = part + (int64_t)bz * 4 * FEMFCT_MAX_PARTIALS;
    const int nwg = gridDim.x * gridDim.y, wg = blockIdx.y * gridDim.x + blockIdx.x;
    double bnorm;
    double rmax_prev = 0.0;
    bool have_rmax = false;
    if (defer) {
        bnorm = 0.0;
    } else if (launch == bn_launch) {
        double rsmin = INFINITY;
        bnorm = 0.0;
        if (!BIG && launch > 0 && g_build == nwg) {
            const double* pr = p + ((launch - 1) & 1) * FEMFCT_MAX_PARTIALS;
            for (int k = threadIdx.x; k < nwg; k += blockDim.x) {
                bnorm = nan_max(bnorm, p[2 * FEMFCT_MAX_PARTIALS + k]);
                rmax_prev = nan_max(rmax_prev, pr[k]);
                rsmin = nan_min(rsmin, p[3 * FEMFCT_MAX_PARTIALS + k]);
            }
            block_reduce_max_max_min(bnorm, rmax_prev, rsmin, smem);
            have_rmax = true;
        } else {
            bnorm = reduce_partials(p + 2 * FEMFCT_MAX_PARTIALS, g_build, OpMax(), 0.0, smem);
            rsmin = reduce_partials(p + 3 * FEMFCT_MAX_PARTIALS, g_build, OpMin(), INFINITY, smem);
        }
        if (wg == 0 && threadIdx.x == 0) {
            ctl->bnorm = bnorm;
            ctl->min_rowsum = rsmin;
            if (!(rsmin > 0.0)) ctl->flags |= FEMFCT_FLAG_MMATRIX_ROWSUM;
        }
    } else {
        bnorm = ctl->bnorm;
    }
    if (launch > 0 && !defer) {
        double rmax = have_rmax ? rmax_prev
                      : BIG   ? ctl->rs[(launch - 1) & 1]
                              : reduce_partials(p + ((launch - 1) & 1) * FEMFCT_MAX_PARTIALS, nwg, OpMax(), 0.0, smem);
        if (rmax <= rel_tol * bnorm) {
            if (wg == 0 && threadIdx.x == 0) {
                ctl->done = 1; ctl->parity = launch & 1; ctl->iters = launch * K; ctl->flags |= FEMFCT_FLAG_COARSE_ITERS;
                ctl->resid = bnorm != 0.0 ? rmax / bnorm : 0.0;
            }
            return;
        }
    }
    const int64_t moff = (int64_t)bz * W * n, voff = (int64_t)bz * n;
    const double* L = L_ + moff;
    const double* xin = ((launch & 1) ? xb_ : xa_) + voff;
    double* xout = ((launch & 1) ? xa_ : xb_) + voff;
    TILE_STAMP_BEGIN();
    const TileGeom g = tile_geom<TILE_L - 2 * H, H>(N);
    constexpr bool CONE = LEAN == 2;
    double lv[W - 1], dg = 1.0, rdg = 1.0, bv = 0.0, xi = 0.0;
#pragma unroll
    for (int s = 0; s < W - 1; ++s) lv[s] = 0.0;
    if constexpr (CONE) {
        const int dist = tile_hexdist<H>(g);
        if (g.inside && ((dist < K && g.kvalid > 0) || g.owned)) {
            dg = L[g.i];
            rdg = 1.0 / dg;
#pragma unroll
            for (int s = 1; s < W; ++s) lv[s - 1] = L[(int64_t)s * n + g.i];
            bv = b_[voff + g.i];
        }
        if (g.inside && dist <= K) xi = xin[g.i];
    } else if (g.inside) {
        dg = L[g.i];
        rdg = 1.0 / dg;
#pragma unroll
        for (int s = 1; s < W; ++s) lv[s - 1] = L[(int64_t)s * n + g.i];
        bv = b_[voff + g.i];
        xi = xin[g.i];
    }
    xs[0][g.self] = xi;
    if (LEAN) xs[1][g.self] = xi;
    __syncthreads();
    TILE_STAMP_LOADED();
    double rmax = 0.0;
    int cur = 0;
    [[maybe_unused]] double xo = xi;
    [[maybe_unused]] const int klive = min(g.kvalid, K - lean_dist<H, LEAN>(g));
    [[maybe_unused]] const LeanAddr a = lean_addr<TILE_L>(xs, g);
    if (!EXACT) {
        if constexpr (LEAN) xo = lean_jacobi(a, klive, K, g.owned, lv, dg, rdg, bv, xi, rmax);
        else
        for (int k = 0; k < K; ++k) {
            const double* c = xs[cur];
            double xn = c[g.self];
            if (k < g.kvalid) {
                double acc = bv;
#pragma unroll
                for (int s = 0; s < W - 1; ++s) acc = fma(-lv[s], c[g.nb[s]], acc);
                if (k == K - 1 && g.owned) rmax = nan_max(rmax, fabs(acc - dg * xn));
                xn = acc * rdg;
            }
            xs[cur ^ 1][g.self] = xn;
            __syncthreads();
            cur ^= 1;
        }
    } else {
        double rk[H];
#pragma unroll
        for (int k = 0; k < H; ++k) {
            rk[k] = 0.0;
            if (k < K) {
                if constexpr (LEAN) {
                    const int rd = (k & 1) * TILE_L * TILE_LD, wr = ((k + 1) & 1) * TILE_L * TILE_LD;
                    if (k < klive) {
                        double acc = bv;
#pragma unroll
                        for (int s = 0; s < W - 1; ++s) acc = fma(-lv[s], a.n0[s][rd], acc);
                        if (g.owned) rk[k] = fabs(acc - dg * xo);
                        if (k == K - 1) rmax = nan_max(rmax, rk[k]);
                        xo = acc * rdg;
                        a.me0[wr] = xo;
                    }
                    __syncthreads();
                    continue;
                }
                const double* c = xs[cur];
                double xn = c[g.self];
                if (k < g.kvalid) {
                    double acc = bv;
#pragma unroll
                    for (int s = 0; s < W - 1; ++s) acc = fma(-lv[s], c[g.nb[s]], acc);
                    if (g.owned) rk[k] = fabs(acc - dg * xn);
                    if (k == K - 1) rmax = nan_max(rmax, rk[k]);
                    xn = acc * rdg;
                }
                xs[cur ^ 1][g.self] = xn;
                __syncthreads();
                cur ^= 1;
            }
        }
        __shared__ double sk[H][STRIP_T / WAVE];
        const int wid = threadIdx.x / WAVE, lane = threadIdx.x % WAVE;
#pragma unroll
        for (int k = 0; k < H; ++k) {
            double v = wave_reduce(rk[k], OpMax());
            if (lane == 0) sk[k][wid] = v;
        }
        __syncthreads();
        if (threadIdx.x < H) {
            double v = 0.0;
            for (int w = 0; w < STRIP_T / WAVE; ++w) v = nan_max(v, sk[threadIdx.x][w]);
            partk[((int64_t)bz * 16 + threadIdx.x) * FEMFCT_MAX_PARTIALS + wg] = v;
        }
    }
    if (g.owned) xout[g.i] = LEAN ? xo : xs[cur][g.self];
    rmax = block_reduce(rmax, OpMax(), 0.0, smem);
    if (threadIdx.x == 0) {
        if (BIG) bigpart[(int64_t)bz * nwg + wg] = rmax;
        else if (defer) partk[((int64_t)bz * 16 + launch) * FEMFCT_MAX_PARTIALS + wg] = rmax;
        else p[(launch & 1) * FEMFCT_MAX_PARTIALS + wg] = rmax;
    }
    TILE_STAMP_END(1);
}

template <int H, int PRE, int LEAN>
__global__ void __launch_bounds__(STRIP_T)
k_tile_build_jacobi(int n, int N, MatRef A_ref, const double* __restrict__ N_, int nshared,
                    VecRef rhs_ref, int64_t rhs_bstride, VecRef u_ref, int64_t u_bstride,
                    const double* __restrict__ ml, double dt, double* __restrict__ L_, double* __restrict__ D_,
                    double* __restrict__ b_, double* __restrict__ xb_, double* __restrict__ part,
                    StepCtl* __restrict__ ctl_, int K) {
    constexpr int W = 7;
    __shared__ double xs[2][TILE_L * TILE_LD];
    __shared__ double as[PRE ? 1 : 3][TILE_L * TILE_LD];
    __shared__ double smem[96];
    const int bz = blockIdx.z;
    const int wg = blockIdx.y * gridDim.x + blockIdx.x;
    double* p = part + (int64_t)bz * 4 * FEMFCT_MAX_PARTIALS;
    if (wg == 0 && threadIdx.x == 0) {
        StepCtl* c = ctl_ + bz;
        c->flags = 0; c->iters = 0; c->done = 0; c->parity = 0; c->resid = 0.0; c->bnorm = 0.0;
        c->min_rowsum = 0.0;
    }
    const int64_t moff = (int64_t)bz * W * n, voff = (int64_t)bz * n;
    const double* A = mat_ptr(A_ref, bz);
    const double* Nm = N_ ? N_ + (nshared ? 0 : moff) : nullptr;
    const double* rhs = vec_ptr(rhs_ref);
    if (rhs) rhs += bz * rhs_bstride;
    const double* u = vec_ptr(u_ref) + bz * u_bstride;
    TILE_STAMP_BEGIN();
    const TileGeom g = tile_geom<TILE_L - 2 * H, H>(N);
    double lv[W - 1], dv[W - 1], dsum = 0.0, rs = 0.0;
    double dg = 1.0, rdg = 1.0, bv = 0.0, xi = 0.0;
    if constexpr (PRE) {
#pragma unroll
        for (int s = 0; s < W - 1; ++s) lv[s] = 0.0;
        if constexpr (LEAN == 2) {
            const int dist = tile_hexdist<H>(g);
            const bool row = g.inside && ((dist < K && g.kvalid > 0) || g.owned);
            if (row) {
                dg = A[g.i];
#pragma unroll
                for (int s = 1; s < W; ++s) lv[s - 1] = A[(int64_t)s * n + g.i];
            }
#pragma unroll
            for (int s = 0; s < W - 1; ++s) rs += lv[s];
            if (g.inside && dist <= K) xi = u[g.i];
            if (row) {
                const double mli = ml[g.i];
                rs += dg;
                rdg = 1.0 / dg;
                bv = mli * xi + (rhs ? dt * rhs[g.i] : 0.0);
            }
        } else {
            if (g.inside) {
                dg = A[g.i];
#pragma unroll
                for (int s = 1; s < W; ++s) lv[s - 1] = A[(int64_t)s * n + g.i];
            }
#pragma unroll
            for (int s = 0; s < W - 1; ++s) rs += lv[s];
            if (g.inside) {
                const double mli = ml[g.i];
                rs += dg;
                rdg = 1.0 / dg;
                xi = u[g.i];
                bv = mli * xi + (rhs ? dt * rhs[g.i] : 0.0);
            }
        }
    } else {
        const int dx[6] = {1, 1, 0, -1, -1, 0}, dy[6] = {0, 1, 1, 0, -1, -1};
        bool ex[W - 1];
#pragma unroll
        for (int s = 0; s < W - 1; ++s) {
            const int nx = g.gx + dx[s], ny = g.gy + dy[s];
            ex[s] = g.inside && nx >= 0 && nx < N && ny >= 0 && ny < N;
        }
        double av[W - 1], at[W - 1], a0 = 0.0;
#pragma unroll
        for (int s = 0; s < W - 1; ++s) av[s] = 0.0;
        if (g.inside) {
            a0 = A[g.i];
#pragma unroll
            for (int s = 1; s < W; ++s) av[s - 1] = A[(int64_t)s * n + g.i];
        }
#pragma unroll
        for (int s = 0; s < 3; ++s) as[s][g.self] = av[s + 3];
        __syncthreads();
#pragma unroll
        for (int s = 0; s < 3; ++s) at[s] = as[s][g.nb[s]];
        __syncthreads();
#pragma unroll
        for (int s = 0; s < 3; ++s) as[s][g.self] = av[s];
        __syncthreads();
#pragma unroll
        for (int s = 3; s < 6; ++s) at[s] = as[s - 3][g.nb[s]];
#pragma unroll
        for (int s = 0; s < W - 1; ++s) {
            const double a = av[s];
            const double d = ex[s] ? fmax(0.0, fmax(a, at[s])) : 0.0;
            dsum += d;
            double l = dt * (a - d);
            if (Nm && g.inside) l += dt * Nm[(int64_t)(s + 1) * n + g.i];
            lv[s] = l;
            dv[s] = d;
            rs += l;
        }
        if (g.inside) {
            const double mli = ml[g.i];
            double ld = mli + dt * (a0 + dsum);
            if (Nm) ld += dt * Nm[g.i];
            rs += ld;
            dg = ld;
            rdg = 1.0 / dg;
            xi = u[g.i];
            bv = mli * xi + (rhs ? dt * rhs[g.i] : 0.0);
        }
    }
    double bmax = 0.0, rsmin = INFINITY;
    if (g.owned) {
        double* L = L_ + moff;
        L[g.i] = dg;
#pragma unroll
        for (int s = 1; s < W; ++s) L[(int64_t)s * n + g.i] = lv[s - 1];
        if constexpr (!PRE) {
            double* D = D_ + moff;
            D[g.i] = -dsum;
#pragma unroll
            for (int s = 1; s < W; ++s) D[(int64_t)s * n + g.i] = dv[s - 1];
        }
        b_[voff + g.i] = bv;
        bmax = fabs(bv);
        rsmin = rs;
    }
    xs[0][g.self] = xi;
    if (LEAN) xs[1][g.self] = xi;
    __syncthreads();
    TILE_STAMP_LOADED();
    double rmax = 0.0;
    int cur = 0;
    [[maybe_unused]] double xo = xi;
    if constexpr (LEAN) xo = lean_jacobi(lean_addr<TILE_L>(xs, g), min(g.kvalid, K - lean_dist<H, LEAN>(g)), K, g.owned, lv, dg, rdg, bv, xi, rmax);
    else
    for (int k = 0; k < K; ++k) {
        const double* c = xs[cur];
        double xn = c[g.self];
        if (k < g.kvalid) {
            double acc = bv;
#pragma unroll
            for (int s = 0; s < W - 1; ++s) acc = fma(-lv[s], c[g.nb[s]], acc);
            if (k == K - 1 && g.owned) rmax = nan_max(rmax, fabs(acc - dg * xn));
            xn = acc * rdg;
        }
        xs[cur ^ 1][g.self] = xn;
        __syncthreads();
        cur ^= 1;
    }
    if (g.owned) xb_[voff + g.i] = LEAN ? xo : xs[cur][g.self];
    block_reduce_max_max_min(rmax, bmax, rsmin, smem);
    if (threadIdx.x == 0) {
        p[wg] = rmax;
        p[2 * FEMFCT_MAX_PARTIALS + wg] = bmax;
        p[3 * FEMFCT_MAX_PARTIALS + wg] = rsmin;
    }
    TILE_STAMP_END(0);
}

__global__ void __launch_bounds__(256)
k_low_seq(int n, int N, const double* __restrict__ A_, const double* __restrict__ ml, double dt, double* __restrict__ L_,
          double* __restrict__ D_) {
    constexpr int W = 7;
    const int64_t off = (int64_t)blockIdx.y * W * n;
    const double* A = A_ + off;
    double* L = L_ + off;
    double* D = D_ + off;
    const int dx[6] = {1, 1, 0, -1, -1, 0}, dy[6] = {0, 1, 1, 0, -1, -1};
    for (int i = blockIdx.x * blockDim.x + threadIdx.x; i < n; i += gridDim.x * blockDim.x) {
        const int gx = i % N, gy = i / N;
        double av[W - 1], at[W - 1];
        bool ex[W - 1];
        const double a0 = A[i];
#pragma unroll
        for (int s = 0; s < W - 1; ++s) {
            const int nx = gx + dx[s], ny = gy + dy[s];
            ex[s] = nx >= 0 && nx < N && ny >= 0 && ny < N;
            av[s] = A[(int64_t)(s + 1) * n + i];
            at[s] = ex[s] ? A[(int64_t)(s < 3 ? s + 4 : s - 2) * n + ny * N + nx] : 0.0;
        }
        double dsum = 0.0;
#pragma unroll
        for (int s = 0; s < W - 1; ++s) {
            const double a = av[s];
            const double d = ex[s] ? fmax(0.0, fmax(a, at[s])) : 0.0;
            dsum += d;
            L[(int64_t)(s + 1) * n + i] = dt * (a - d);
            D[(int64_t)(s + 1) * n + i] = d;
        }
        L[i] = ml[i] + dt * (a0 + dsum);
        D[i] = -dsum;
    }
}

__global__ void __launch_bounds__(STRIP_T)
k_reduce_resid(const double* __restrict__ bigpart, int64_t count, StepCtl* __restrict__ ctl_, int launch) {
    __shared__ double smem[32];
    const int bz = blockIdx.x;
    if (ctl_[bz].done) return;
    const double* q = bigpart + (int64_t)bz * count;
    double v = 0.0;
    for (int64_t k = threadIdx.x; k < count; k += blockDim.x) v = nan_max(v, q[k]);
    v = block_reduce(v, OpMax(), 0.0, smem);
    if (threadIdx.x == 0) ctl_[bz].rs[launch & 1] = v;
}

template <int H, int LEAN>
__global__ void __launch_bounds__(STRIP_T)
k_tile_cheb(int n, int N, const double* __restrict__ M, const double* __restrict__ b_, const double* __restrict__ ymid_,
            const double* __restrict__ yold_, double* __restrict__ omid_, double* __restrict__ oold_, int K,
            CheOmegas om, double md_scale, ChebIO cio) {
    constexpr int W = 7;
    __shared__ double ys[LEAN ? 2 : 3][TILE_L * TILE_LD];
    const int64_t voff = (int64_t)blockIdx.z * n;
    if (cio.mat) M = cio.mat + (int64_t)blockIdx.z * cio.mat_bs;
    if (cio.scale_dev) md_scale = cio.scale_dev[blockIdx.z];
    const double* omd = cio.om_dev ? cio.om_dev + (int64_t)blockIdx.z * cio.om_bs + cio.k0 : nullptr;
    if (cio.mid_ref.base) ymid_ = vec_ptr(cio.mid_ref) + (int64_t)blockIdx.z * cio.mid_bs - voff;
    if (cio.out_ref.base) omid_ = const_cast<double*>(vec_ptr(cio.out_ref)) + (int64_t)blockIdx.z * cio.out_bs - voff;
    const TileGeom g = tile_geom<TILE_L - 2 * H, H>(N);
    constexpr bool CONE = LEAN == 2;
    double mv[W - 1], md = 1.0, rmd = 1.0, bv = 0.0, ym = 0.0, yo = 0.0;
#pragma unroll
    for (int s = 0; s < W - 1; ++s) mv[s] = 0.0;
    if constexpr (CONE) {
        const int dist = tile_hexdist<H>(g);
        if (g.inside && ((dist < K && g.kvalid > 0) || g.owned)) {
            md = M[g.i];
            rmd = 1.0 / (md_scale * md);
#pragma unroll
            for (int s = 1; s < W; ++s) mv[s - 1] = M[(int64_t)s * n + g.i];
            bv = b_[voff + g.i];
            if (yold_) yo = yold_[voff + g.i];
        }
        if (g.inside && dist <= K && ymid_) ym = ymid_[voff + g.i];
    } else if (g.inside) {
        md = M[g.i];
        rmd = 1.0 / (md_scale * md);
#pragma unroll
        for (int s = 1; s < W; ++s) mv[s - 1] = M[(int64_t)s * n + g.i];
        bv = b_[voff + g.i];
        if (ymid_) ym = ymid_[voff + g.i];
        if (yold_) yo = yold_[voff + g.i];
    }
    if constexpr (LEAN) {
        ys[0][g.self] = ym;
        ys[1][g.self] = ym;
        __syncthreads();
        const int klive = min(g.kvalid, K - lean_dist<H, LEAN>(g));
        const LeanAddr a = lean_addr<TILE_L>(ys, g);
        int k = 0;
        for (; k + 1 < K; k += 2) {
            lean_cheb_iter<0>(a, k < klive, mv, md, rmd, bv, omd ? omd[k] : om.w[k], ym, yo);
            lean_cheb_iter<1>(a, k + 1 < klive, mv, md, rmd, bv, omd ? omd[k + 1] : om.w[k + 1], ym, yo);
        }
        if (k < K) lean_cheb_iter<0>(a, k < klive, mv, md, rmd, bv, omd ? omd[k] : om.w[k], ym, yo);
        if (g.owned) {
            omid_[voff + g.i] = ym;
            if (oold_) oold_[voff + g.i] = yo;
        }
        return;
    }
    ys[0][g.self] = yo;
    ys[1][g.self] = ym;
    __syncthreads();
    int io = 0, im = 1, in_ = 2;
    for (int k = 0; k < K; ++k) {
        const double* ymd = ys[im];
        const double ymv = ymd[g.self];
        double yn = ymv;
        if (k < g.kvalid) {
            double acc = md * ymv;
#pragma unroll
            for (int s = 0; s < W - 1; ++s) acc = fma(mv[s], ymd[g.nb[s]], acc);
            const double z = (bv - acc) * rmd;
            const double yov = ys[io][g.self];
            const double wk = omd ? omd[k] : om.w[k];
            yn = wk * (z + ymv - yov) + yov;
        }
        ys[in_][g.self] = yn;
        __syncthreads();
        int t = io; io = im; im = in_; in_ = t;
    }
    if (g.owned) {
        omid_[voff + g.i] = ys[im][g.self];
        if (oold_) oold_[voff + g.i] = ys[io][g.self];
    }
}


#define FL_H 2
template <int PL>
__device__ __forceinline__ int fl_nb(int s) {
    const int lx = threadIdx.x % PL, ly = threadIdx.x / PL;
    const int dx = (s == 0 || s == 1) ? 1 : (s == 3 || s == 4) ? -1 : 0;
    const int dy = (s == 1 || s == 2) ? 1 : (s == 4 || s == 5) ? -1 : 0;
    return min(max(ly + dy, 0), PL - 1) * (PL + 1) + min(max(lx + dx, 0), PL - 1);
}

template <int FL_L, int GEOM, int HALFD>
__global__ void __launch_bounds__(FL_L * FL_L, FL_L == 32 ? 8 : 1)
k_tile_flux_limit(int n, int N, double h, const double* __restrict__ M, const double* __restrict__ D_,
                  const double* __restrict__ ulow_, const double* __restrict__ du_, const double* __restrict__ ml,
                  double dt, VecRef out_ref, int64_t out_bstride, EndArgs e) {
    constexpr int W = 7;
    constexpr int FL_LD = FL_L + 1, FL_T = FL_L - 2 * FL_H;
    __shared__ double su[FL_L * FL_LD], sd[FL_L * FL_LD], srp[FL_L * FL_LD], srm[FL_L * FL_LD];
    __shared__ double sdf[HALFD ? 3 : 1][HALFD ? FL_L * FL_LD : 1];
    if (FL_L == 16) step_log_early(e);
    const int bz = blockIdx.z;
    const int64_t moff = (int64_t)bz * W * n, voff = (int64_t)bz * n;
    const TileGeom g = tile_geom<FL_T, FL_H, FL_L>(N);
    double ui = 0.0, dui = 0.0, mli = 1.0, dfw[3] = {0.0, 0.0, 0.0};
    if (g.inside) { ui = ulow_[voff + g.i]; dui = du_[voff + g.i]; mli = ml[g.i]; }
    if (HALFD) {
        if (g.inside) {
#pragma unroll
            for (int s = 0; s < 3; ++s) dfw[s] = D_[moff + (int64_t)(s + 1) * n + g.i];
        }
#pragma unroll
        for (int s = 0; s < 3; ++s) sdf[s][g.self] = dfw[s];
    }
    su[g.self] = ui;
    sd[g.self] = dui;
    srp[g.self] = 1.0;
    srm[g.self] = 1.0;
    __syncthreads();
    double f[W - 1];
    const bool have = g.inside && g.kvalid >= 1;
    if (have) {
        double pp = 0.0, pm = 0.0, umax = ui, umin = ui;
        const int pc = (GEOM || HALFD) ? mass_edge_counts(g.gx, g.gy, N - 1) : 0;
        const double mq = (0.5 * h * h) / 12.0;
#pragma unroll
        for (int s = 1; s < W; ++s) {
            const int64_t idx = (int64_t)s * n + g.i;
            const int nbs = fl_nb<FL_L>(s - 1);
            const double uj = su[nbs];
            const double mij = GEOM ? (double)((pc >> (2 * (s - 1))) & 3) * mq : M[idx];
            double dij;
            if (HALFD) {
                const bool exists = ((pc >> (2 * (s - 1))) & 3) != 0;
                dij = s <= 3 ? sdf[s - 1][g.self] : (exists ? sdf[s - 4][nbs] : 0.0);
            } else {
                dij = D_[moff + idx];
            }
            const double fs = mij * (dui - sd[nbs]) + dij * (ui - uj);
            f[s - 1] = fs;
            pp += fmax(fs, 0.0);
            pm += fmin(fs, 0.0);
            const bool live = (mij != 0.0) || (dij != 0.0);
            umax = live ? fmax(umax, uj) : umax;
            umin = live ? fmin(umin, uj) : umin;
        }
        const double qp = umax - ui, qm = umin - ui;
        srp[g.self] = (pp != 0.0) ? fmin(1.0, mli * qp / (dt * pp)) : 1.0;
        srm[g.self] = (pm != 0.0) ? fmin(1.0, mli * qm / (dt * pm)) : 1.0;
    }
    __syncthreads();
    if (g.owned) {
        const double rpi = srp[g.self], rmi = srm[g.self];
        double fbar = 0.0;
#pragma unroll
        for (int s = 0; s < W - 1; ++s) {
            const double fs = f[s];
            const int nbs = fl_nb<FL_L>(s);
            const double a = (fs > 0.0) ? fmin(rpi, srm[nbs]) : fmin(rmi, srp[nbs]);
            fbar += a * fs;
        }
        double* out = const_cast<double*>(vec_ptr(out_ref)) + bz * out_bstride;
        out[g.i] = ui + dt * fbar / mli;
    }
    if (FL_L == 16) step_end_by_last_workgroup(e);
}

template <int GEOM, int LEAN, int PL>
__global__ void __launch_bounds__((PL * PL + WAVE - 1) / WAVE * WAVE, (LEAN && PL == TILE_L) ? 8 : 1)
k_tile_cheb_flux_limit(int n, int N, double h, const double* __restrict__ M, const double* __restrict__ b_,
                       const double* __restrict__ ymid_, const double* __restrict__ yold_, int K, CheOmegas om,
                       double md_scale, MatRef D_ref, const double* __restrict__ ulow_,
                       const double* __restrict__ ml, double dt, VecRef out_ref, int64_t out_bstride, EndArgs e) {
    constexpr int W = 7, HH = 12, PLD = PL + 1;
    constexpr bool CONE = LEAN == 2;
    static_assert(PL == TILE_L || LEAN, "fitted patches run the lean loops only");
    __shared__ double ys[LEAN ? 2 : 3][PL * PLD];
    __shared__ double su[PL * PLD], srp[PL * PLD], srm[PL * PLD];
    const int bz = blockIdx.z;
    const int64_t voff = (int64_t)bz * n;
    const double* D_ = mat_ptr(D_ref, bz);
    TILE_STAMP_BEGIN();
    const TileGeom g = tile_geom<PL - 2 * HH, HH, PL>(N);
    double mv[W - 1], dv[W - 1], md = 1.0, rmd = 1.0, bv = 0.0, ym = 0.0, yo = 0.0, ui = 0.0, mli = 1.0;
#pragma unroll
    for (int s = 0; s < W - 1; ++s) { mv[s] = 0.0; dv[s] = 0.0; }
    [[maybe_unused]] bool flux_node = false;
    if constexpr (CONE) {
        const int dist = tile_hexdist<HH, PL>(g);
        flux_node = g.inside && g.kvalid >= K + 1 && dist <= 1;
        if (g.inside && (min(g.kvalid, K - max(dist - 2, 0)) > 0 || flux_node)) {
            md = M[g.i];
            rmd = 1.0 / (md_scale * md);
            if (GEOM) {
                const int pc = mass_edge_counts(g.gx, g.gy, N - 1);
                const double mq = (0.5 * h * h) / 12.0;
#pragma unroll
                for (int s = 1; s < W; ++s) mv[s - 1] = (double)((pc >> (2 * (s - 1))) & 3) * mq;
            } else {
#pragma unroll
                for (int s = 1; s < W; ++s) mv[s - 1] = M[(int64_t)s * n + g.i];
            }
            bv = b_[voff + g.i];
            yo = yold_[voff + g.i];
        }
        if (g.inside && max(dist - 2, 0) <= K) ym = ymid_[voff + g.i];
        if (g.inside && dist <= 2) {
            ui = ulow_[voff + g.i];
            mli = ml[g.i];
        }
    } else if (g.inside) {
        md = M[g.i];
        rmd = 1.0 / (md_scale * md);
        if (GEOM) {
            const int pc = mass_edge_counts(g.gx, g.gy, N - 1);
            const double mq = (0.5 * h * h) / 12.0;
#pragma unroll
            for (int s = 1; s < W; ++s) mv[s - 1] = (double)((pc >> (2 * (s - 1))) & 3) * mq;
        } else {
#pragma unroll
            for (int s = 1; s < W; ++s) mv[s - 1] = M[(int64_t)s * n + g.i];
        }
        bv = b_[voff + g.i];
        ym = ymid_[voff + g.i];
        yo = yold_[voff + g.i];
        ui = ulow_[voff + g.i];
        mli = ml[g.i];
    }
    if (!tile_spare<PL>()) {
        ys[0][g.self] = LEAN ? ym : yo;
        ys[1][g.self] = ym;
        su[g.self] = ui;
        srp[g.self] = 1.0;
        srm[g.self] = 1.0;
    }
    __syncthreads();
    TILE_STAMP_LOADED();
    step_log_early(e);
    if (g.inside && (!CONE || flux_node)) {
#pragma unroll
        for (int s = 1; s < W; ++s) dv[s - 1] = D_[(int64_t)s * n + g.i];
    }
    int io = 0, im = 1, in_ = 2;
    const bool have = g.inside && g.kvalid >= K + 1 && (!LEAN || lean_dist<HH, LEAN, PL>(g) <= 1);
    if constexpr (LEAN) {
        const int klive = min(g.kvalid, K - max(lean_dist<HH, LEAN, PL>(g) - 2, 0));
        const LeanAddr a = lean_addr<PL>(ys, g);
        int k = 0;
        for (; k + 1 < K; k += 2) {
            lean_cheb_iter<0, PL>(a, k < klive, mv, md, rmd, bv, om.w[k], ym, yo);
            lean_cheb_iter<1, PL>(a, k + 1 < klive, mv, md, rmd, bv, om.w[k + 1], ym, yo);
        }
        if (k < K) lean_cheb_iter<0, PL>(a, k < klive, mv, md, rmd, bv, om.w[k], ym, yo);
        im = K & 1;
    } else
    for (int k = 0; k < K; ++k) {
        const double* ymd = ys[im];
        const double ymv = ymd[g.self];
        double yn = ymv;
        if (k < g.kvalid) {
            double acc = md * ymv;
#pragma unroll
            for (int s = 0; s < W - 1; ++s) acc = fma(mv[s], ymd[g.nb[s]], acc);
            const double z = (bv - acc) * rmd;
            const double yov = ys[io][g.self];
            yn = om.w[k] * (z + ymv - yov) + yov;
        }
        ys[in_][g.self] = yn;
        __syncthreads();
        int t = io; io = im; im = in_; in_ = t;
    }
    const double* sd = ys[im];
    const double dui = LEAN ? ym : sd[g.self];
    double f[W - 1];
    if (have) {
        double pp = 0.0, pm = 0.0, umax = ui, umin = ui;
#pragma unroll
        for (int s = 0; s < W - 1; ++s) {
            const double uj = su[g.nb[s]];
            const double mij = mv[s], dij = dv[s];
            const double fs = mij * (dui - sd[g.nb[s]]) + dij * (ui - uj);
            f[s] = fs;
            pp += fmax(fs, 0.0);
            pm += fmin(fs, 0.0);
            const bool live = (mij != 0.0) || (dij != 0.0);
            umax = live ? fmax(umax, uj) : umax;
            umin = live ? fmin(umin, uj) : umin;
        }
        const double qp = umax - ui, qm = umin - ui;
        srp[g.self] = (pp != 0.0) ? fmin(1.0, mli * qp / (dt * pp)) : 1.0;
        srm[g.self] = (pm != 0.0) ? fmin(1.0, mli * qm / (dt * pm)) : 1.0;
    }
    __syncthreads();
    if (g.owned) {
        const double rpi = srp[g.self], rmi = srm[g.self];
        double fbar = 0.0;
#pragma unroll
        for (int s = 0; s < W - 1; ++s) {
            const double fs = f[s];
            const double a = (fs > 0.0) ? fmin(rpi, srm[g.nb[s]]) : fmin(rmi, srp[g.nb[s]]);
            fbar += a * fs;
        }
        double* out = const_cast<double*>(vec_ptr(out_ref)) + bz * out_bstride;
        out[g.i] = ui + dt * fbar / mli;
    }
    TILE_STAMP_END(3);
    step_end_by_last_workgroup(e);
}

template <int LEAN, int GEOM, int PL>
__global__ void __launch_bounds__((PL * PL + WAVE - 1) / WAVE * WAVE)
k_tile_dudt_cheb(int n, int N, double h, MatRef A_ref, VecRef rhs_ref, int64_t rhs_bstride,
                 const double* __restrict__ M, const double* __restrict__ xa_, const double* __restrict__ xb_,
                 double* __restrict__ ulow_, double* __restrict__ rdu_, double* __restrict__ omid_,
                 double* __restrict__ oold_, double* __restrict__ part, StepCtl* __restrict__ ctl_, int budget,
                 int part_count, int iters_per_unit, double rel_tol, const double* __restrict__ partk, int exact_k,
                 int K, CheOmegas om, double md_scale, double omega1) {
    constexpr int W = 7, H = 10, PLD = PL + 1;
    constexpr bool CONE = LEAN == 2;
    static_assert(PL == TILE_L || LEAN, "fitted patches run the lean loops only");
    __shared__ double ys[LEAN ? 2 : 3][PL * PLD];
    __shared__ double smem[64];
    const int bz = blockIdx.z;
    StepCtl* ctl = ctl_ + bz;
    double* p = part + (int64_t)bz * 4 * FEMFCT_MAX_PARTIALS;
    const int wg = blockIdx.y * gridDim.x + blockIdx.x;
    if (exact_k < 0 && blockIdx.y == gridDim.x) {
        if (blockIdx.x == 0)
            deferred_test_publish(ctl, deferred_test_load(p, partk + (int64_t)bz * 16 * FEMFCT_MAX_PARTIALS, part_count, -exact_k),
                                  -exact_k, iters_per_unit, rel_tol);
        return;
    }
    const int parity = exact_k < 0 ? (budget & 1) : ctl->done ? ctl->parity : (budget & 1);
    if (exact_k >= 0)
        finalize_solve(ctl, p, part_count, budget, iters_per_unit, rel_tol, smem,
                       partk ? partk + (int64_t)bz * 16 * FEMFCT_MAX_PARTIALS : nullptr, exact_k, wg == 0);
    const int64_t voff = (int64_t)bz * n;
    const double* A = mat_ptr(A_ref, bz);
    const double* x = (parity ? xb_ : xa_) + voff;
    const double* rhs = vec_ptr(rhs_ref);
    if (rhs) rhs += bz * rhs_bstride;
    TILE_STAMP_BEGIN();
    const TileGeom g = tile_geom<PL - 2 * H, H, PL>(N);
    double av[W], mv[W - 1], md = 1.0, rmd = 1.0, ui = 0.0, ri = 0.0;
#pragma unroll
    for (int s = 0; s < W; ++s) av[s] = 0.0;
#pragma unroll
    for (int s = 0; s < W - 1; ++s) mv[s] = 0.0;
    bool need_r = g.kvalid >= 1;
    if constexpr (CONE) {
        const int dist = tile_hexdist<H, PL>(g);
        need_r = need_r && dist <= K;
        if (g.inside && need_r) {
            md = M[g.i];
            rmd = 1.0 / (md_scale * md);
#pragma unroll
            for (int s = 0; s < W; ++s) av[s] = A[(int64_t)s * n + g.i];
            ri = rhs ? rhs[g.i] : 0.0;
        }
        if (g.inside && g.kvalid > 1 && dist < K) {
            if (GEOM) {
                const int pc = mass_edge_counts(g.gx, g.gy, N - 1);
                const double mq = (0.5 * h * h) / 12.0;
#pragma unroll
                for (int s = 1; s < W; ++s) mv[s - 1] = (double)((pc >> (2 * (s - 1))) & 3) * mq;
            } else {
#pragma unroll
                for (int s = 1; s < W; ++s) mv[s - 1] = M[(int64_t)s * n + g.i];
            }
        }
        if (g.inside && dist <= K + 1) ui = x[g.i];
    } else if (g.inside) {
        md = M[g.i];
        rmd = 1.0 / (md_scale * md);
#pragma unroll
        for (int s = 0; s < W; ++s) av[s] = A[(int64_t)s * n + g.i];
        if (GEOM) {
            const int pc = mass_edge_counts(g.gx, g.gy, N - 1);
            const double mq = (0.5 * h * h) / 12.0;
#pragma unroll
            for (int s = 1; s < W; ++s) mv[s - 1] = (double)((pc >> (2 * (s - 1))) & 3) * mq;
        } else {
#pragma unroll
            for (int s = 1; s < W; ++s) mv[s - 1] = M[(int64_t)s * n + g.i];
        }
        ui = x[g.i];
        ri = rhs ? rhs[g.i] : 0.0;
    }
    constexpr int UB = LEAN ? 0 : 2;
    const bool spare = tile_spare<PL>();
    if (!spare) ys[UB][g.self] = ui;
    __syncthreads();
    TILE_STAMP_LOADED();
    double r = 0.0, y1 = 0.0;
    if (need_r) {
        double acc = av[0] * ui;
#pragma unroll
        for (int s = 1; s < W; ++s) acc = fma(av[s], ys[UB][g.nb[s - 1]], acc);
        r = -acc + ri;
        y1 = omega1 * (r / (md_scale * md));
    }
    if constexpr (LEAN) {
        if (!spare) ys[1][g.self] = y1;
        __syncthreads();
        if (!spare) ys[0][g.self] = y1;
        double ym = y1, yo = 0.0;
        const int dist = lean_dist<H, LEAN, PL>(g);
        const LeanAddr a = lean_addr<PL>(ys, g);
        auto live = [&](int k) { return k + 1 < g.kvalid && k < K - dist; };
        int k = 0;
        for (; k + 1 < K; k += 2) {
            lean_cheb_iter<1, PL>(a, live(k), mv, md, rmd, r, om.w[k], ym, yo);
            lean_cheb_iter<0, PL>(a, live(k + 1), mv, md, rmd, r, om.w[k + 1], ym, yo);
        }
        if (k < K) lean_cheb_iter<1, PL>(a, live(k), mv, md, rmd, r, om.w[k], ym, yo);
        if (g.owned) {
            ulow_[voff + g.i] = ui;
            rdu_[voff + g.i] = r;
            omid_[voff + g.i] = ym;
            if (oold_) oold_[voff + g.i] = yo;
        }
        TILE_STAMP_END(2);
        return;
    }
    __syncthreads();
    ys[0][g.self] = 0.0;
    ys[1][g.self] = y1;
    __syncthreads();
    int io = 0, im = 1, in_ = 2;
    for (int k = 0; k < K; ++k) {
        const double* ymd = ys[im];
        const double ymv = ymd[g.self];
        double yn = ymv;
        if (k + 1 < g.kvalid) {
            double acc = md * ymv;
#pragma unroll
            for (int s = 0; s < W - 1; ++s) acc = fma(mv[s], ymd[g.nb[s]], acc);
            const double z = (r - acc) * rmd;
            const double yov = ys[io][g.self];
            yn = om.w[k] * (z + ymv - yov) + yov;
        }
        ys[in_][g.self] = yn;
        __syncthreads();
        int t = io; io = im; im = in_; in_ = t;
    }
    if (g.owned) {
        ulow_[voff + g.i] = ui;
        rdu_[voff + g.i] = r;
        omid_[voff + g.i] = ys[im][g.self];
        if (oold_) oold_[voff + g.i] = ys[io][g.self];
    }
    TILE_STAMP_END(2);
}

}

#ifdef FEMFCT_TUNING
void femfct_tile_phase_dump(const char* path) {
    static const char* names[4] = {"k_tile_build_jacobi", "k_tile_jacobi", "k_tile_dudt_cheb", "k_tile_cheb_flux_limit"};
    unsigned long long h[4][4];
    if (hipMemcpyFromSymbol(h, HIP_SYMBOL(g_tile_phase), sizeof(h)) != hipSuccess) return;
    if (FILE* f = fopen(path, "a")) {
        for (int k = 0; k < 4; ++k)
            if (h[k][2])
                fprintf(f, "%-24s launches %8llu  load phase %7.3f us  whole kernel %7.3f us  share %5.1f %%\n", names[k], h[k][2],
                        0.01 * h[k][0] / h[k][2], 0.01 * h[k][1] / h[k][2], 100.0 * h[k][0] / (double)h[k][1]);
        fclose(f);
    }
    memset(h, 0, sizeof(h));
    hipMemcpyToSymbol(HIP_SYMBOL(g_tile_phase), h, sizeof(h));
}
#endif


static int tile_lean_mode(const femfct_ctx* ctx) { return ctx->tile_lean ? (ctx->tile_cone ? 2 : 1) : 0; }

int femfct_enqueue_tile_build_jacobi(femfct_ctx* ctx, const TilePlan& pl, MatRef A, const double* Nm, int32_t nshared,
                                     VecRef rhs, int64_t rhs_bstride, VecRef u_n, int64_t u_bstride, double dt,
                                     int32_t batch, bool pre) {
    if (pre && Nm) return femfct_fail(ctx, FEMFCT_ERR_INVALID, "pre-built low-order operator with a non-flux matrix");
    dim3 grid(pl.tiles, pl.tiles, batch);
    femfct_prof_begin(ctx, KC_JACOBI);
    auto go = [&](auto kernel) {
        hipLaunchKernelGGL(kernel, grid, dim3(STRIP_T), 0, ctx->stream, ctx->n, ctx->N, A, Nm, nshared, rhs, rhs_bstride, u_n,
                           u_bstride, ctx->d_ml, dt, ctx->d_L, ctx->d_D, ctx->d_b, ctx->d_xb, ctx->d_part, ctx->d_ctl, pl.K);
    };
    with_constant<8, TILE_HMAX>(pl.H, [&](auto h) {
        constexpr int H = decltype(h)::value;
        with_constant<0, 2>(tile_lean_mode(ctx), [&](auto l) {
            constexpr int LEAN = decltype(l)::value;
            if (pre) go(k_tile_build_jacobi<H, 1, LEAN>); else go(k_tile_build_jacobi<H, 0, LEAN>);
        });
    });
    femfct_prof_end(ctx);
    return FEMFCT_OK;
}

int femfct_enqueue_low_seq(femfct_ctx* ctx, const double* A, double* L, double* D, int32_t entries, double dt) {
    if (!ctx->implicit_cols || ctx->W != 7 || (int64_t)ctx->N * ctx->N != ctx->n || entries < 1 || entries > 65535)
        return femfct_fail(ctx, FEMFCT_ERR_INVALID, "low-order sequence: structured mesh in vertex order only");
    femfct_prof_begin(ctx, KC_ASSEMBLE);
    hipLaunchKernelGGL(k_low_seq, dim3((ctx->n + 255) / 256, entries), dim3(256), 0, ctx->stream, ctx->n, ctx->N, A, ctx->d_ml,
                       dt, L, D);
    femfct_prof_end(ctx);
    return FEMFCT_OK;
}

int femfct_enqueue_tile_jacobi(femfct_ctx* ctx, const TilePlan& pl, const double* L, const double* b, double* xa,
                               double* xb, int launch, int g_build, int32_t batch, bool last, int bn_launch, int defer) {
    const bool big = femfct_tile_big(ctx, pl);
    double* bigp = big ? ctx->d_bigpart : nullptr;
    double* pk = ((last || defer) && !big) ? ctx->d_partk : nullptr;
    dim3 grid(pl.tiles, pl.tiles, batch);
    femfct_prof_begin(ctx, KC_JACOBI);
    auto go = [&](auto kernel, int defer_arg) {
        hipLaunchKernelGGL(kernel, grid, dim3(STRIP_T), 0, ctx->stream, ctx->n, ctx->N, L, b, xa, xb, ctx->d_part, ctx->d_ctl,
                           launch, pl.K, g_build, ctx->rel_tol, bigp, pk, bn_launch, defer_arg);
    };
    with_constant<0, 2>(tile_lean_mode(ctx), [&](auto l) {
        constexpr int LEAN = decltype(l)::value;
        if (big) {
            go(k_tile_jacobi<8, 0, 1, LEAN>, 0);
            femfct_launch_reduce_resid(ctx, (int64_t)pl.tiles * pl.tiles, launch, batch);
        } else {
            with_constant<8, TILE_HMAX>(pl.H, [&](auto h) {
                constexpr int H = decltype(h)::value;
                if (pk && !defer) go(k_tile_jacobi<H, 1, 0, LEAN>, 0); else go(k_tile_jacobi<H, 0, 0, LEAN>, defer);
            });
        }
    });
    femfct_prof_end(ctx);
    return FEMFCT_OK;
}

void femfct_launch_reduce_resid(femfct_ctx* ctx, int64_t count, int launch, int32_t batch) {
    hipLaunchKernelGGL(k_reduce_resid, dim3(batch), dim3(STRIP_T), 0, ctx->stream, ctx->d_bigpart, count, ctx->d_ctl, launch);
}

int femfct_enqueue_tile_dudt_cheb(femfct_ctx* ctx, MatRef A, VecRef rhs, int64_t rhs_bstride, double* ulow,
                                  int budget_units, int part_count, int iters_per_unit, int exact_k, int iters,
                                  const double* omegas, double md_scale, int32_t batch, int* tail_first) {
    constexpr int H = 10;
    const int T = TILE_L - 2 * H, t = (ctx->N + T - 1) / T;
    const bool fit = femfct_tile_fit(ctx, batch);
    const int tl = fit ? (ctx->N + 5) / 6 : t;
    const int K = std::min(iters - 1, H - 1);
    CheOmegas om;
    for (int k = 0; k < K; ++k) om.w[k] = omegas[k + 1];
    const bool last = (K + 1 == iters);
    double* omid = last ? ctx->d_du : ctx->d_y0;
    double* oold = last ? nullptr : ctx->d_y2;
    femfct_prof_begin(ctx, KC_DUDT_RHS);
    auto go = [&](auto kernel, int PL) {
        hipLaunchKernelGGL(kernel, dim3(tl, exact_k < 0 ? tl + 1 : tl, batch), dim3((PL * PL + WAVE - 1) / WAVE * WAVE), 0,
                           ctx->stream, ctx->n, ctx->N, ctx->h, A, rhs, rhs_bstride, ctx->d_M, ctx->d_xa, ctx->d_xb, ulow, ctx->d_rdu,
                           omid, oold, ctx->d_part, ctx->d_ctl, budget_units, part_count, iters_per_unit, ctx->rel_tol,
                           exact_k ? ctx->d_partk : nullptr, exact_k, K, om, md_scale, omegas[0]);
    };
    with_constant<0, 1>(ctx->tile_lean && femfct_geom_mass(ctx), [&](auto gm) {
        constexpr int GM = decltype(gm)::value;
        if (fit) {
            if (ctx->tile_cone) go(k_tile_dudt_cheb<2, GM, 26>, 26); else go(k_tile_dudt_cheb<1, GM, 26>, 26);
        } else if constexpr (GM) {
            if (ctx->tile_cone) go(k_tile_dudt_cheb<2, 1, TILE_L>, TILE_L); else go(k_tile_dudt_cheb<1, 1, TILE_L>, TILE_L);
        } else {
            with_constant<0, 2>(tile_lean_mode(ctx), [&](auto l) { go(k_tile_dudt_cheb<decltype(l)::value, 0, TILE_L>, TILE_L); });
        }
    });
    femfct_prof_end(ctx);
    if (tail_first) *tail_first = last ? 0 : K + 2;
    if (last || tail_first) return FEMFCT_OK;
    TilePlan tp;
    tp.H = H; tp.K = H; tp.tiles = t;
    return femfct_enqueue_tile_cheb(ctx, tp, ctx->d_rdu, ctx->d_y0, ctx->d_y2, ctx->d_du, K + 2, iters, omegas, md_scale,
                                    ctx->d_y1, ctx->d_rp, ctx->d_y0, ctx->d_y2, batch, nullptr);
}

int femfct_enqueue_tile_cheb(femfct_ctx* ctx, const TilePlan& pl, const double* b, const double* in_mid,
                             const double* in_old, double* y_out, int k_first, int k_last, const double* omegas,
                             double md_scale, double* bufA0, double* bufA1, double* bufB0, double* bufB1, int32_t batch,
                             const ChebIO* io_in) {
    ChebIO io0{};
    if (io_in) io0 = *io_in;
    io0.mid_ref = make_ref(nullptr); io0.mid_bs = 0; io0.out_ref = make_ref(nullptr); io0.out_bs = 0;
    for_cheb_launches(k_first, k_last, pl.K, omegas, in_mid, in_old, y_out, bufA0, bufA1, bufB0, bufB1,
                      [&](int k0, int k1, const CheOmegas& om, const double* mid, const double* old, double* omid, double* oold) {
        femfct_prof_begin(ctx, KC_CHEB);
        ChebIO io = io0;
        io.k0 = k0 - 1;
        if (io_in && k0 == k_first) { io.mid_ref = io_in->mid_ref; io.mid_bs = io_in->mid_bs; }
        if (io_in && k1 == k_last + 1) { io.out_ref = io_in->out_ref; io.out_bs = io_in->out_bs; }
        with_constant<8, TILE_HMAX>(pl.H, [&](auto h) {
            with_constant<0, 2>(tile_lean_mode(ctx), [&](auto l) {
                hipLaunchKernelGGL((k_tile_cheb<decltype(h)::value, decltype(l)::value>), dim3(pl.tiles, pl.tiles, batch),
                                   dim3(STRIP_T), 0, ctx->stream, ctx->n, ctx->N, ctx->d_M, b, mid, old, omid, oold, k1 - k0, om,
                                   md_scale, io);
            });
        });
        femfct_prof_end(ctx);
    });
    return FEMFCT_OK;
}

static EndArgs step_end_args(const femfct_ctx* ctx, int32_t batch, bool fuse_end) {
    EndArgs e{};
    e.level = nullptr;
    if (fuse_end) {
        e.level = ctx->d_level; e.delta = ctx->rep_last ? ctx->end_req_delta * ctx->rep_total : 0;
        e.ord_adv = ctx->rep_last ? ctx->rep_total : 0; e.ord_off = ctx->ord_bias; e.ctl = ctx->d_ctl; e.log = ctx->d_log;
        e.kctl = ctx->end_req_krylov ? (const KrylovCtl*)ctx->d_kry_ctl : nullptr; e.klog = (KrylovCtl*)ctx->d_klog;
        e.batch = batch; e.ticket = ctx->d_ticket;
    }
    return e;
}

int femfct_enqueue_tile_cheb_flux_limit(femfct_ctx* ctx, const double* b, const double* in_mid, const double* in_old,
                                        int k_first, int k_last, const double* omegas, double md_scale, MatRef D,
                                        const double* ulow, double dt, VecRef out, int64_t out_bstride, int32_t batch,
                                        bool fuse_end) {
    const int K = k_last - k_first + 1;
    if (K < 1 || K > 10) return femfct_fail(ctx, FEMFCT_ERR_INVALID, "fused Chebyshev tail: %d iterations", K);
    const EndArgs e = step_end_args(ctx, batch, fuse_end);
    CheOmegas om;
    for (int k = k_first; k <= k_last; ++k) om.w[k - k_first] = omegas[k - 1];
    const bool fit = femfct_tile_fit(ctx, batch);
    const int t = fit ? (ctx->N + 5) / 6 : (ctx->N + 7) / 8;
    femfct_prof_begin(ctx, KC_FLUX);
    auto go = [&](auto kernel, int PL) {
        hipLaunchKernelGGL(kernel, dim3(t, t, batch), dim3((PL * PL + WAVE - 1) / WAVE * WAVE), 0, ctx->stream, ctx->n, ctx->N,
                           ctx->h, ctx->d_M, b, in_mid, in_old, K, om, md_scale, D, ulow, ctx->d_ml, dt, out, out_bstride, e);
    };
    with_constant<0, 1>(femfct_geom_mass(ctx), [&](auto gm) {
        constexpr int GM = decltype(gm)::value;
        if (fit) {
            if (ctx->tile_cone) go(k_tile_cheb_flux_limit<GM, 2, 30>, 30); else go(k_tile_cheb_flux_limit<GM, 1, 30>, 30);
        } else {
            with_constant<0, 2>(tile_lean_mode(ctx), [&](auto l) { go(k_tile_cheb_flux_limit<GM, decltype(l)::value, TILE_L>, TILE_L); });
        }
    });
    femfct_prof_end(ctx);
    return FEMFCT_OK;
}

int femfct_enqueue_tile_flux_limit(femfct_ctx* ctx, const double* D, const double* ulow, const double* du, double dt,
                                   VecRef out, int64_t out_bstride, int32_t batch, bool* fuse_end_io, int half_d) {
    const bool fuse_end = fuse_end_io && *fuse_end_io && ctx->N <= 512;
    if (fuse_end_io) *fuse_end_io = fuse_end;
    const EndArgs e = step_end_args(ctx, batch, fuse_end);
    femfct_prof_begin(ctx, KC_FLUX);
    const bool geom = femfct_geom_mass(ctx);
    auto go = [&](auto kernel, int PL) {
        const int t = (ctx->N + PL - 2 * FL_H - 1) / (PL - 2 * FL_H);
        hipLaunchKernelGGL(kernel, dim3(t, t, batch), dim3(PL * PL), 0, ctx->stream, ctx->n, ctx->N, ctx->h, ctx->d_M, D, ulow, du,
                           ctx->d_ml, dt, out, out_bstride, e);
    };
    with_constant<0, 1>(geom, [&](auto g) {
        with_constant<0, 1>(half_d != 0, [&](auto hd) {
            constexpr int G = decltype(g)::value, HD = decltype(hd)::value;
            if (ctx->N <= 512) go(k_tile_flux_limit<16, G, HD>, 16); else go(k_tile_flux_limit<32, G, HD>, 32);
        });
    });
    femfct_prof_end(ctx);
    return FEMFCT_OK;
}


bool femfct_geom_mass(const femfct_ctx* ctx) {
    return ctx->geom_mass && ctx->structured && ctx->mass_is_mesh && ctx->implicit_cols;
}

bool femfct_cheb_flux_fusable(const femfct_ctx* ctx, int32_t batch) {
    if (!ctx->fuse_flux || ctx->N > 512) return false;
    const int t = (ctx->N + 7) / 8;
    return (int64_t)t * t * batch <= ctx->wg_slots;
}

bool femfct_tile_fit(const femfct_ctx* ctx, int32_t batch) {
    if (!ctx->tile_lean || !ctx->tile_fit) return false;
    const int t = (ctx->N + 5) / 6;
    return (int64_t)t * (t + 1) * batch <= ctx->wg_slots;
}

bool femfct_tile_plan(const femfct_ctx* ctx, TilePlan* pl, bool need_partials, int budget, int batch) {
    if (!femfct_tiles_usable(ctx)) return false;
    int H = 8;
    const bool small = ctx->N <= 512;
    if (small) {
        if (budget <= 0) H = 10;
        else {
            int best = 1 << 30;
            for (int h = 8; h <= TILE_HMAX; ++h) {
                const int T = TILE_L - 2 * h, t = (ctx->N + T - 1) / T;
                if (h > 10 && (!ctx->deep_halo || (int64_t)t * t * batch > ctx->wg_slots)) break;
                int launches = (budget + h - 1) / h;
                if (launches < best) { best = launches; H = h; }
            }
        }
    }
    if (small && ctx->strip_k >= 8 && ctx->strip_k <= TILE_HMAX) H = ctx->strip_k;
    const int T = TILE_L - 2 * H;
    const int t = (ctx->N + T - 1) / T;
    if (need_partials && (int64_t)t * t > FEMFCT_MAX_PARTIALS) return false;
    if (t > 65535) return false;
    pl->tiles = t;
    pl->K = H;
    pl->H = H;
    return true;
}

bool femfct_tile_big(const femfct_ctx* ctx, const TilePlan& pl) {
    return (int64_t)pl.tiles * pl.tiles > FEMFCT_MAX_PARTIALS;
}
```

fem-fct-pdeco_amd/csrc/solve_ctl.h:

```cpp
#pragma once

#include "femfct_internal.h"
#include "device_utils.h"

constexpr int FEMFCT_DEFER_MAX_UNITS = 4;
struct DeferredPartials { double r[FEMFCT_DEFER_MAX_UNITS], bn, rs; };

__device__ __forceinline__ DeferredPartials deferred_test_load(const double* p, const double* partk, int G, int units) {
    DeferredPartials d;
#pragma unroll
    for (int s = 0; s < FEMFCT_DEFER_MAX_UNITS; ++s) d.r[s] = 0.0;
    d.bn = 0.0; d.rs = INFINITY;
    if (threadIdx.x < WAVE) {
#pragma unroll 4
        for (int k = threadIdx.x; k < G; k += WAVE) {
            d.r[0] = nan_max(d.r[0], p[k]);
#pragma unroll
            for (int s = 1; s < FEMFCT_DEFER_MAX_UNITS; ++s)
                if (s < units) d.r[s] = nan_max(d.r[s], partk[(int64_t)s * FEMFCT_MAX_PARTIALS + k]);
            d.bn = nan_max(d.bn, p[2 * FEMFCT_MAX_PARTIALS + k]);
            d.rs = nan_min(d.rs, p[3 * FEMFCT_MAX_PARTIALS + k]);
        }
    }
    return d;
}

__device__ __forceinline__ void deferred_test_publish(StepCtl* ctl, DeferredPartials d, int units, int iters_per_unit,
                                                      double rel_tol) {
    if (threadIdx.x >= WAVE) return;
    double r[FEMFCT_DEFER_MAX_UNITS];
#pragma unroll
    for (int s = 0; s < FEMFCT_DEFER_MAX_UNITS; ++s) r[s] = wave_reduce(d.r[s], OpMax());
    const double bn = wave_reduce(d.bn, OpMax()), rs = wave_reduce(d.rs, OpMin());
    if (threadIdx.x == 0) {
        ctl->bnorm = bn;
        ctl->min_rowsum = rs;
        if (!(rs > 0.0)) ctl->flags |= FEMFCT_FLAG_MMATRIX_ROWSUM;
        const double tolb = rel_tol * bn;
        int first = -1;
        double rlast = 0.0;
#pragma unroll
        for (int s = 0; s < FEMFCT_DEFER_MAX_UNITS; ++s)
            if (s < units) {
                if (first < 0 && r[s] <= tolb) first = s;
                rlast = r[s];
            }
        ctl->iters = (first >= 0 ? first + 1 : units) * iters_per_unit;
        if (first >= 0 && first < units - 1) ctl->flags |= FEMFCT_FLAG_COARSE_ITERS;
        if (first < 0) ctl->flags |= FEMFCT_FLAG_SOLVER_BUDGET;
        ctl->resid = bn != 0.0 ? rlast / bn : 0.0;
    }
}

__device__ __forceinline__ void finalize_solve(StepCtl* ctl, double* p, int G, int budget, int iters_per_unit,
                                               double rel_tol, double* smem, const double* partk, int exact_k,
                                               bool leader) {
    if (ctl->done) return;
    if (partk && exact_k > 0) {
        const double tolb = rel_tol * ctl->bnorm;
        int first = -1;
        double rlast = 0.0;
        for (int k = 0; k < exact_k; ++k) {
            rlast = reduce_partials(partk + (int64_t)k * FEMFCT_MAX_PARTIALS, G, OpMax(), 0.0, smem);
            if (first < 0 && rlast <= tolb) { first = k; break; }
        }
        if (leader && threadIdx.x == 0) {
            const double bn = ctl->bnorm;
            ctl->iters = (first >= 0) ? (budget - 1) * iters_per_unit + first + 1 : budget * iters_per_unit;
            ctl->resid = bn != 0.0 ? rlast / bn : 0.0;
            if (first < 0) ctl->flags |= FEMFCT_FLAG_SOLVER_BUDGET;
        }
        return;
    }
    double rmax = (G < 0) ? ctl->rs[(budget - 1) & 1]
                          : reduce_partials(p + ((budget - 1) & 1) * FEMFCT_MAX_PARTIALS, G, OpMax(), 0.0, smem);
    if (leader && threadIdx.x == 0) {
        double bn = ctl->bnorm;
        ctl->iters = budget * iters_per_unit;
        ctl->resid = bn != 0.0 ? rmax / bn : 0.0;
        if (!(rmax <= rel_tol * bn)) ctl->flags |= FEMFCT_FLAG_SOLVER_BUDGET;
    }
}
```

fem-fct-pdeco_amd/csrc/traj_common.h:

```cpp
#pragma once

#include <chrono>

#include "femfct_internal.h"
#include "device_utils.h"
#include "forms.h"

#include <algorithm>
#include <stdio.h>
#include <stdlib.h>

int femfct_ensure_traj_ws(femfct_ctx* ctx, int32_t batch, int32_t steps);
int femfct_ensure_krylov_ws(femfct_ctx* ctx, int32_t batch);
int femfct_enqueue_step_end(femfct_ctx* ctx, int delta, int32_t batch, bool with_krylov);
void femfct_request_fused_end(femfct_ctx* ctx, int delta, bool with_krylov);
int femfct_enqueue_step_ref(femfct_ctx* ctx, const double* A, const double* N, int32_t nshared, VecRef rhs,
                            int64_t rhs_bstride, VecRef u_n, int64_t u_bstride, double dt, VecRef u_out,
                            int64_t out_bstride, int32_t batch, int32_t budget);
int femfct_enqueue_step_mat(femfct_ctx* ctx, MatRef A, const double* N, int32_t nshared, VecRef rhs, int64_t rhs_bstride,
                            VecRef u_n, int64_t u_bstride, double dt, VecRef u_out, int64_t out_bstride, int32_t batch,
                            int32_t budget);
int femfct_enqueue_axpby(femfct_ctx* ctx, int64_t count, double alpha, const double* a, double beta, const double* b,
                         double* out);
struct SbOpArgs;
bool femfct_inline_ops_wanted(const femfct_ctx* ctx, int32_t batch);
int femfct_enqueue_step_op(femfct_ctx* ctx, MatRef A, const SbOpArgs* sb, const double* N, int32_t nshared, VecRef rhs,
                           int64_t rhs_bstride, VecRef u_n, int64_t u_bstride, double dt, VecRef u_out, int64_t out_bstride,
                           int32_t batch, int32_t budget);

static inline int femfct_round_kry_budget(const femfct_ctx* ctx, int b) {
    b = (b + 3) & ~3;
    if (b < 4) b = 4;
    if (b > ctx->kry_max_iters) b = ctx->kry_max_iters;
    return b;
}

template <class F>
int femfct_run_graph_reps(femfct_ctx* ctx, femfct_ctx::GraphKey key, int reps, int delta, F&& enqueue_one) {
    key.push_back(key_bits((int32_t)reps));
    key.push_back(key_bits((int32_t)ctx->pair_rows));
    key.push_back(key_bits((int32_t)ctx->solver));
    key.push_back(key_bits(ctx->low_src));
    key.push_back(key_bits(ctx->low_dt));
    key.push_back(key_bits((int32_t)(ctx->tile_lean | ctx->tile_cone << 1 | ctx->tile_fit << 2)));
    struct Restore {
        femfct_ctx* c;
        ~Restore() { c->level_bias = 0; c->ord_bias = 0; c->rep_total = 1; c->rep_last = true; }
    } restore{ctx};
    return femfct_run_graph(ctx, key, [&]() {
        for (int r = 0; r < reps; ++r) {
            ctx->level_bias = r * delta; ctx->ord_bias = r; ctx->rep_total = reps; ctx->rep_last = (r == reps - 1);
            int rc = enqueue_one();
            if (rc != FEMFCT_OK) return rc;
        }
        return (int)FEMFCT_OK;
    });
}

static inline VecRef lref(const femfct_ctx* ctx, const double* p, const int32_t* level, int64_t stride, int32_t off) {
    return make_ref(p, level, stride, off + (level ? ctx->level_bias : 0));
}

struct SweepSpec {
    SweepKind kind;
    int32_t num_steps, batch;
    int level0;
    bool krylov;
    bool full_rows;
};
struct SweepPlan {
    int budget, kbudget;
    bool meshp, cheb;
};
enum { FEMFCT_SWEEP_REPEAT = -1 };
FEMFCT_INTERNAL int femfct_sweep_plan(femfct_ctx* ctx, const SweepSpec& sp, SweepPlan* plan);
FEMFCT_INTERNAL int femfct_sweep_fetch_logs(femfct_ctx* ctx, const SweepSpec& sp);
FEMFCT_INTERNAL int femfct_sweep_verdict(femfct_ctx* ctx, const SweepSpec& sp, const SweepPlan& plan);
FEMFCT_INTERNAL void femfct_sweep_report_times(const SweepSpec& sp, const double t[4]);

static inline int femfct_next_kry_budget(const femfct_ctx* ctx, int worst, bool cheb) {
    return std::min(ctx->kry_max_iters, cheb ? std::max(8, worst + 1) : std::max(8, worst + worst / 4 + 2));
}

template <class Begin, class Step>
int femfct_run_sweep(femfct_ctx* ctx, const SweepSpec& sp, Begin&& begin, Step&& step) {
    struct RestoreSolver {
        femfct_ctx* c;
        ~RestoreSolver() { c->solver = c->solver_user; c->pair_rows = false; }
    } restore_solver{ctx};
    const bool dbg_t = getenv("FEMFCT_DEBUG_TIMES") != nullptr;
    auto now = []() { return std::chrono::duration<double, std::milli>(std::chrono::steady_clock::now().time_since_epoch()).count(); };
    for (;;) {
        SweepPlan plan;
        int rc = femfct_sweep_plan(ctx, sp, &plan);
        if (rc != FEMFCT_OK) return rc;
        double t[4] = {dbg_t ? now() : 0.0, 0.0, 0.0, 0.0};
        if ((rc = begin()) != FEMFCT_OK) return rc;
        if (dbg_t) t[1] = now();
        int32_t init[2] = {sp.level0, 0};
        HIP_TRY(ctx, hipMemcpyAsync(ctx->d_level, init, sizeof init, hipMemcpyHostToDevice, ctx->stream));
        const int32_t per_graph = std::max(1, std::min(ctx->steps_per_graph, sp.num_steps));
        for (int32_t k = 0; k < sp.num_steps; k += per_graph) {
            rc = step(plan.budget, plan.kbudget, std::min(per_graph, sp.num_steps - k));
            if (rc != FEMFCT_OK) return rc;
        }
        if (dbg_t) t[2] = now();
        if ((rc = femfct_sweep_fetch_logs(ctx, sp)) != FEMFCT_OK) return rc;
        if (dbg_t) { t[3] = now(); femfct_sweep_report_times(sp, t); }
        rc = femfct_sweep_verdict(ctx, sp, plan);
        if (rc != FEMFCT_SWEEP_REPEAT) return rc;
    }
}
```

fem-fct-pdeco_amd/device.py:

```python
from __future__ import annotations

import ctypes as C

import numpy as np

from . import _lib
from ._lib import lib, check, StepInfo


def _host_ptr(a: np.ndarray):
    return a.ctypes.data_as(C.c_void_p)


def _as_f64(a) -> np.ndarray:
    return np.ascontiguousarray(a, dtype=np.float64)


class DeviceArray:

    def __init__(self, ctx: "Context", count: int):
        self.ctx = ctx
        self.count = int(count)
        ptr = C.c_void_p()
        check(ctx.handle, lib.femfct_malloc(ctx.handle, C.byref(ptr), self.count * 8))
        self.ptr = ptr.value
        ctx._arrays.add(self)

    def data_ptr(self) -> int:
        return self.ptr

    def upload(self, host) -> "DeviceArray":
        h = _as_f64(host).reshape(-1)
        if h.size != self.count:
            raise ValueError(f"upload: host array has {h.size} elements, device array {self.count}")
        check(self.ctx.handle, lib.femfct_memcpy_h2d(self.ctx.handle, self.ptr, _host_ptr(h), h.nbytes))
        return self

    def download(self, out: np.ndarray | None = None) -> np.ndarray:
        if out is None:
            out = np.empty(self.count, dtype=np.float64)
        if out.size != self.count or out.dtype != np.float64 or not out.flags.c_contiguous:
            raise ValueError("download: need a C-contiguous float64 array of matching size")
        check(self.ctx.handle, lib.femfct_memcpy_d2h(self.ctx.handle, _host_ptr(out), self.ptr, out.nbytes))
        return out

    def zero(self) -> "DeviceArray":
        check(self.ctx.handle, lib.femfct_memset0(self.ctx.handle, self.ptr, self.count * 8))
        return self

    def copy_from(self, other, count=None, dst_off=0, src_off=0) -> "DeviceArray":
        count = self.count if count is None else int(count)
        check(self.ctx.handle, lib.femfct_memcpy_d2d(self.ctx.handle, self.ptr + 8 * dst_off,
                                                      dptr(other) + 8 * src_off, count * 8))
        return self

    def free(self):
        if self.ptr:
            lib.femfct_free(self.ctx.handle, self.ptr)
            self.ptr = 0
            self.ctx._arrays.discard(self)


def _wind_scale(wind_scale, num_steps) -> np.ndarray:
    ws = _as_f64(wind_scale).reshape(-1)
    if ws.size != num_steps + 1:
        raise ValueError(f"wind_scale: {ws.size} values, expected num_steps + 1 = {num_steps + 1} (s(t_0) .. s(t_Nt))")
    return ws


def _growth(growth) -> np.ndarray:
    g = _as_f64(growth).reshape(-1)
    if g.size != 3:
        raise ValueError(f"growth: {g.size} values, expected the three coefficients (r0, r1, r2) of u (r0 + r1 u + r2 u^2)")
    return g


MISFITS = {"nodal": 0, "mass": 1}


class DeviceObs:

    def __init__(self, theta_u=None, tau_u=0.0, theta_v=None, tau_v=0.0, window=None):
        self.theta_u, self.tau_u, self.theta_v, self.tau_v, self.window = theta_u, float(tau_u), theta_v, float(tau_v), window


def _misfit(misfit) -> int:
    if misfit not in MISFITS:
        raise ValueError(f"Invalid value for 'misfit': '{misfit}'. Must be one of {sorted(MISFITS)}.")
    return MISFITS[misfit]


def dptr(x) -> int:
    if x is None:
        return 0
    if isinstance(x, int):
        return x
    return int(x.data_ptr())


class Context:

    def __init__(self, device_id: int = 0):
        h = C.c_void_p()
        code = lib.femfct_create(C.byref(h), int(device_id))
        if code != _lib.OK:
            raise _lib.FemFctError(code, f"femfct_create(device {device_id}) failed: no usable HIP device")
        self.handle = h
        self.device_id = int(device_id)
        self._arrays = set()
        self.mesh = None

    def close(self):
        if getattr(self, "handle", None):
            for a in list(self._arrays):
                a.free()
            lib.femfct_destroy(self.handle)
            self.handle = None

    def __del__(self):
        try:
            self.close()
        except Exception:
            pass

    def __enter__(self):
        return self

    def __exit__(self, *exc):
        self.close()

    def set_solver(self, solver=_lib.SOLVER_JACOBI, rel_tol=1e-13, max_iters=400):
        check(self.handle, lib.femfct_set_solver(self.handle, solver, rel_tol, max_iters))

    def set_graphs(self, enable: bool):
        check(self.handle, lib.femfct_set_graphs(self.handle, int(bool(enable))))

    def launch_info(self) -> dict:
        out = (C.c_int32 * 4)()
        check(self.handle, lib.femfct_launch_info(self.handle, out))
        kinds = {0: "other", 1: "k_strip4_jacobi", 2: "k_strip4_jacobi_walk", 3: "k_strip_jacobi_pair_walk"}
        return {"jacobi_kernel": kinds.get(out[0], "?"), "jacobi_walkers": int(out[1]), "cheb_interior_patches": int(out[2]),
                "halo": int(out[3])}

    def graph_replay_active(self) -> bool:
        v = C.c_int(0)
        check(self.handle, lib.femfct_graph_replay_active(self.handle, C.byref(v)))
        return bool(v.value)

    def rotation_derived(self) -> bool:
        v = C.c_int(0)
        check(self.handle, lib.femfct_rotation_derived(self.handle, C.byref(v)))
        return bool(v.value)

    KERNEL_CLASSES = ("build_low", "jacobi", "dudt_rhs", "cheb", "flux", "limit", "assemble", "other")

    def set_profiling(self, enable: bool):
        check(self.handle, lib.femfct_set_profiling(self.handle, int(bool(enable))))

    def profile_report(self):
        ms = np.zeros(8)
        cnt = np.zeros(8, dtype=np.int32)
        check(self.handle, lib.femfct_profile_report(self.handle, _host_ptr(ms), _host_ptr(cnt), 8))
        return {k: (float(ms[i]), int(cnt[i])) for i, k in enumerate(self.KERNEL_CLASSES)}

    def set_fusion(self, strips=True, tiles=True):
        check(self.handle, lib.femfct_set_fusion(self.handle, int(bool(strips)), int(bool(tiles))))

    def patch_walkers(self, batch=1, sweeps=36) -> int:
        return lib.femfct_patch_walkers(self.handle, int(batch), int(sweeps))

    def kernel_regime(self, batch=1) -> int:
        return lib.femfct_kernel_regime(self.handle, int(batch))

    def lowop_nonzero_fraction(self) -> float:
        out = C.c_double(1.0)
        check(self.handle, lib.femfct_lowop_nonzero_fraction(self.handle, C.byref(out)))
        return float(out.value)

    def uses_bandwidth_tiles(self, batch=1) -> bool:
        return self.kernel_regime(batch) == _lib.REGIME_PATCH64

    def synchronize(self):
        check(self.handle, lib.femfct_synchronize(self.handle))

    @property
    def stream(self) -> int:
        return lib.femfct_stream(self.handle) or 0

    def empty(self, count) -> DeviceArray:
        return DeviceArray(self, count)

    def zeros(self, count) -> DeviceArray:
        return DeviceArray(self, count).zero()

    def array(self, host) -> DeviceArray:
        h = _as_f64(host).reshape(-1)
        return DeviceArray(self, h.size).upload(h)

    @property
    def n(self) -> int:
        return lib.femfct_n(self.handle)

    @property
    def W(self) -> int:
        return lib.femfct_ell_width(self.handle)

    def set_pattern_csr(self, indptr, indices):
        ip = np.ascontiguousarray(indptr, dtype=np.int32)
        ix = np.ascontiguousarray(indices, dtype=np.int32)
        check(self.handle, lib.femfct_set_pattern_csr(self.handle, ip.size - 1, _host_ptr(ip), _host_ptr(ix)))
        self.mesh = None

    def set_mesh_square(self, a1, a2, n_cells, order=_lib.ORDER_FENICS):
        check(self.handle, lib.femfct_set_mesh_square(self.handle, float(a1), float(a2), int(n_cells), int(order)))

    def ell_cols(self) -> np.ndarray:
        out = np.empty(self.W * self.n, dtype=np.int32)
        check(self.handle, lib.femfct_get_ell_cols(self.handle, _host_ptr(out)))
        return out.reshape(self.W, self.n)

    def set_mass(self, M_csr_vals, ml):
        m = _as_f64(M_csr_vals)
        l = _as_f64(ml)
        check(self.handle, lib.femfct_set_mass(self.handle, _host_ptr(m), _host_ptr(l)))

    def csr_to_ell(self, csr_vals, out: DeviceArray | None = None) -> DeviceArray:
        v = _as_f64(csr_vals)
        if out is None:
            out = self.empty(self.W * self.n)
        check(self.handle, lib.femfct_csr_to_ell(self.handle, _host_ptr(v), dptr(out)))
        return out

    def ell_to_csr(self, ell, nnz: int) -> np.ndarray:
        out = np.empty(int(nnz), dtype=np.float64)
        check(self.handle, lib.femfct_ell_to_csr(self.handle, dptr(ell), _host_ptr(out)))
        return out

    @property
    def mass_ell(self) -> int:
        return lib.femfct_mass_ell(self.handle) or 0

    @property
    def stiffness_ell(self) -> int:
        return lib.femfct_stiffness_ell(self.handle) or 0

    @property
    def lumped_mass(self) -> int:
        return lib.femfct_lumped_mass(self.handle) or 0

    def fct_step(self, A_ell, u_n, dt, u_out, rhs=None, N_ell=None, N_shared=False, batch=1):
        check(self.handle, lib.femfct_fct_step(self.handle, dptr(A_ell), dptr(N_ell), int(bool(N_shared)),
                                               dptr(rhs), dptr(u_n), float(dt), dptr(u_out), int(batch)))

    def last_step_info(self, batch=1):
        arr = (StepInfo * batch)()
        check(self.handle, lib.femfct_last_step_info(self.handle, arr, int(batch)))
        return [dict(flags=a.flags, solver_iters=a.solver_iters, solver_resid=a.solver_resid,
                     min_rowsum=a.min_rowsum) for a in arr]

    def fct_step_host(self, A_csr_vals, rhs, u_n, dt, N_csr_vals=None):
        a = _as_f64(A_csr_vals)
        u = _as_f64(u_n)
        r = None if rhs is None else _as_f64(rhs)
        nn = None if N_csr_vals is None else _as_f64(N_csr_vals)
        out = np.empty(self.n, dtype=np.float64)
        info = StepInfo()
        check(self.handle, lib.femfct_fct_step_host(
            self.handle, _host_ptr(a), None if nn is None else _host_ptr(nn),
            None if r is None else _host_ptr(r), _host_ptr(u), float(dt), _host_ptr(out), C.byref(info)))
        return out, dict(flags=info.flags, solver_iters=info.solver_iters, solver_resid=info.solver_resid,
                         min_rowsum=info.min_rowsum)

    def chebsi(self, b, y, cheb_iter=20, lmin=0.5, lmax=2.0, batch=1):
        check(self.handle, lib.femfct_chebsi(self.handle, dptr(b), dptr(y), int(cheb_iter), float(lmin),
                                             float(lmax), int(batch)))

    def chebsi_md(self, b, y, md, cheb_iter=20, lmin=0.5, lmax=2.0, batch=1):
        check(self.handle, lib.femfct_chebsi_md(self.handle, dptr(b), dptr(y), dptr(md), int(cheb_iter), float(lmin),
                                                float(lmax), int(batch)))

    def artificial_diffusion(self, K_ell, D_ell, batch=1):
        check(self.handle, lib.femfct_artificial_diffusion(self.handle, dptr(K_ell), dptr(D_ell), int(batch)))

    def spmv(self, mat_ell, x, y, alpha=1.0, beta=0.0, batch=1):
        check(self.handle, lib.femfct_spmv(self.handle, dptr(mat_ell), dptr(x), float(alpha), float(beta),
                                           dptr(y), int(batch)))

    def quad_points(self, n_cells):
        cnt = n_cells * n_cells * 2 * 6
        xq = np.empty(cnt)
        yq = np.empty(cnt)
        check(self.handle, lib.femfct_mesh_quad_points(self.handle, _host_ptr(xq), _host_ptr(yq)))
        return xq, yq

    def assemble_convection(self, wind_q, scale=1.0, out: DeviceArray | None = None) -> DeviceArray:
# ... 429 lines not shown
```

include/femfct.h:

```cpp
#ifndef FEMFCT_H
#define FEMFCT_H

#include <stddef.h>
#include <stdint.h>

#ifdef __cplusplus
extern "C" {
#endif

#define FEMFCT_ABI_VERSION 5

typedef struct femfct_ctx femfct_ctx;

#define FEMFCT_OK                 0
#define FEMFCT_ERR_INVALID        1
#define FEMFCT_ERR_HIP            2
#define FEMFCT_ERR_NOT_CONVERGED  3
#define FEMFCT_ERR_NOMEM          4

#define FEMFCT_FLAG_MMATRIX_ROWSUM 1
#define FEMFCT_FLAG_SOLVER_BUDGET  2
#define FEMFCT_FLAG_COARSE_ITERS   4
#define FEMFCT_FLAG_CHEBYSHEV      8
#define FEMFCT_FLAG_ROW_PAIRS      16

#define FEMFCT_ORDER_VERTEX 0
#define FEMFCT_ORDER_FENICS 1

#define FEMFCT_SOLVER_JACOBI   0
#define FEMFCT_SOLVER_BICGSTAB 1

typedef struct femfct_step_info {
    int32_t flags;
    int32_t solver_iters;
    double  solver_resid;
    double  min_rowsum;
} femfct_step_info;

int         femfct_abi_version(void);
const char* femfct_build_id(void);
int         femfct_create(femfct_ctx** ctx, int device_id);
int         femfct_destroy(femfct_ctx* ctx);
const char* femfct_last_error(const femfct_ctx* ctx);
int         femfct_synchronize(femfct_ctx* ctx);
void*       femfct_stream(femfct_ctx* ctx);
int         femfct_set_solver(femfct_ctx* ctx, int solver, double rel_tol, int max_iters);
int         femfct_set_graphs(femfct_ctx* ctx, int enable);
int         femfct_launch_info(const femfct_ctx* ctx, int32_t* out4_host);
int         femfct_graph_replay_active(const femfct_ctx* ctx, int* active_host);
int         femfct_rotation_derived(const femfct_ctx* ctx, int* derived_host);
int         femfct_set_fusion(femfct_ctx* ctx, int strips, int tiles);
#define FEMFCT_REGIME_ROWS    0
#define FEMFCT_REGIME_STRIPS  1
#define FEMFCT_REGIME_TILE32  2
#define FEMFCT_REGIME_PATCH64 3
#define FEMFCT_REGIME_MESH    4
int         femfct_kernel_regime(const femfct_ctx* ctx, int32_t batch);
int         femfct_patch_walkers(const femfct_ctx* ctx, int32_t batch, int32_t sweeps);
int         femfct_lowop_nonzero_fraction(femfct_ctx* ctx, double* fraction_host);

int femfct_set_profiling(femfct_ctx* ctx, int enable);
int femfct_profile_report(femfct_ctx* ctx, double* total_ms_host, int32_t* launches_host, int32_t n_classes);

int femfct_malloc(femfct_ctx* ctx, void** dev_ptr, size_t bytes);
int femfct_free(femfct_ctx* ctx, void* dev_ptr);
int femfct_memcpy_h2d(femfct_ctx* ctx, void* dev_dst, const void* host_src, size_t bytes);
int femfct_memcpy_d2h(femfct_ctx* ctx, void* host_dst, const void* dev_src, size_t bytes);
int femfct_memcpy_d2d(femfct_ctx* ctx, void* dev_dst, const void* dev_src, size_t bytes);
int femfct_memset0(femfct_ctx* ctx, void* dev_ptr, size_t bytes);

int femfct_set_pattern_csr(femfct_ctx* ctx, int32_t n, const int32_t* indptr_host,
                           const int32_t* indices_host);
int femfct_set_mesh_square(femfct_ctx* ctx, double a1, double a2, int32_t n_cells, int32_t order);
int32_t femfct_n(const femfct_ctx* ctx);
int32_t femfct_ell_width(const femfct_ctx* ctx);
int femfct_get_ell_cols(femfct_ctx* ctx, int32_t* cols_host);

int femfct_csr_to_ell(femfct_ctx* ctx, const double* csr_vals_host, double* ell_dev);
int femfct_ell_to_csr(femfct_ctx* ctx, const double* ell_dev, double* csr_vals_host);
int femfct_set_mass(femfct_ctx* ctx, const double* M_csr_vals_host, const double* ml_host);
const double* femfct_mass_ell(const femfct_ctx* ctx);
const double* femfct_stiffness_ell(const femfct_ctx* ctx);
const double* femfct_lumped_mass(const femfct_ctx* ctx);

int femfct_fct_step(femfct_ctx* ctx, const double* A_ell, const double* N_ell, int32_t N_shared,
                    const double* rhs, const double* u_n, double dt, double* u_out, int32_t batch);
int femfct_last_step_info(femfct_ctx* ctx, femfct_step_info* info_host, int32_t batch);

int femfct_fct_step_host(femfct_ctx* ctx, const double* A_csr_vals, const double* N_csr_vals,
                         const double* rhs, const double* u_n, double dt, double* u_out,
                         femfct_step_info* info);

int femfct_chebsi(femfct_ctx* ctx, const double* b_dev, double* y_dev, int32_t cheb_iter,
                  double lmin, double lmax, int32_t batch);
int femfct_chebsi_md(femfct_ctx* ctx, const double* b_dev, double* y_dev, const double* md_dev, int32_t cheb_iter,
                     double lmin, double lmax, int32_t batch);
int femfct_artificial_diffusion(femfct_ctx* ctx, const double* K_ell, double* D_ell, int32_t batch);
int femfct_spmv(femfct_ctx* ctx, const double* mat_ell, const double* x_dev, double alpha,
                double beta, double* y_dev, int32_t batch);


int femfct_mesh_quad_points(femfct_ctx* ctx, double* xq_host, double* yq_host);
int femfct_assemble_convection(femfct_ctx* ctx, const double* wind_q_host, double scale, double* A_ell_dev);
int femfct_assemble_rotation(femfct_ctx* ctx, double omega, double* A_ell_dev);
int femfct_drift_gradient_rhs(femfct_ctx* ctx, const double* c_dev, const double* u_dev, const double* p_dev,
                              double beta, double bx, double by, double* out_dev, int32_t levels);


int femfct_solidbody_forward(femfct_ctx* ctx, const double* Arot_ell, const double* c_traj, int32_t c_shared,
                             double* u_traj, int32_t num_steps, double dt, double eps, double rot_scale,
                             double bx, double by, int32_t batch);
int femfct_solidbody_forward_src(femfct_ctx* ctx, const double* Arot_ell, const double* c_traj, int32_t c_shared,
                                 const double* src_traj, double* u_traj, int32_t num_steps, double dt, double eps,
                                 double rot_scale, double bx, double by, int32_t batch);
int femfct_solidbody_adjoint(femfct_ctx* ctx, const double* Arot_ell, const double* c_traj, int32_t c_shared,
                             const double* u_traj, const double* uhat, double* p_traj, int32_t num_steps,
                             double dt, double eps, double rot_scale, double bx, double by, int32_t alltime,
                             int32_t batch);
int femfct_linear_forward_react(femfct_ctx* ctx, const double* A_ell, const double* src_traj, const double* g_traj,
                                double* u_traj, int32_t num_steps, double dt, double eps, int32_t batch);
int femfct_linear_adjoint_react(femfct_ctx* ctx, const double* Aadj_ell, const double* g_traj, const double* u_traj,
                                const double* uhat, double* p_traj, int32_t num_steps, double dt, double eps,
                                int32_t alltime, int32_t batch);
int femfct_react_load(femfct_ctx* ctx, const double* src_dev, const double* g_dev, const double* x_dev, double* out_dev,
                      int32_t batch);
int femfct_solidbody_adjoint_obs(femfct_ctx* ctx, const double* Arot_ell, const double* c_traj, int32_t c_shared,
                                 const double* u_traj, const double* uhat_traj, const double* theta, double tau,
                                 const double* window, double* p_traj, int32_t num_steps, double dt, double eps,
                                 double rot_scale, double bx, double by, int32_t batch);
int femfct_linear_adjoint_react_obs(femfct_ctx* ctx, const double* Aadj_ell, const double* g_traj, const double* u_traj,
                                    const double* uhat_traj, const double* theta, double tau, const double* window,
                                    double* p_traj, int32_t num_steps, double dt, double eps, int32_t batch);
int femfct_obs_load(femfct_ctx* ctx, const double* a_dev, const double* b_dev, const double* theta_dev, int32_t level,
                    double dt, const double* window_dev, double* out_dev, int32_t batch);
int femfct_obs_cost(femfct_ctx* ctx, const double* u_traj, const double* uhat_traj, const double* cost_w_dev,
                    const double* window_dev, int32_t num_steps, int32_t batch, double* out_host);
int femfct_solidbody_adjoint_bounds(femfct_ctx* ctx, const double* Arot_ell, const double* c_traj, int32_t c_shared,
                                    const double* u_traj, const double* uhat_traj, const double* theta, double tau,
                                    const double* window, const double* lower, const double* upper, double gamma,
                                    const double* sigma, const double* window_s, double* p_traj, int32_t num_steps,
                                    double dt, double eps, double rot_scale, double bx, double by, int32_t batch);
int femfct_linear_adjoint_react_bounds(femfct_ctx* ctx, const double* Aadj_ell, const double* g_traj, const double* u_traj,
                                       const double* uhat_traj, const double* theta, double tau, const double* window,
                                       const double* lower, const double* upper, double gamma, const double* sigma,
                                       const double* window_s, double* p_traj, int32_t num_steps, double dt, double eps,
                                       int32_t batch);
int femfct_bound_load(femfct_ctx* ctx, const double* uhat_dev, const double* u_dev, const double* theta_dev,
                      const double* sigma_dev, int32_t level, double dt, const double* window_dev, const double* g_dev,
                      const double* x_dev, const double* lower_dev, const double* upper_dev, double gamma,
                      const double* window_s_dev, double* out_dev, int32_t batch);
int femfct_bound_cost(femfct_ctx* ctx, const double* u_traj, const double* sigma_dev, const double* lower_dev,
                      const double* upper_dev, double gamma, const double* window_s_dev, int32_t num_steps, int32_t batch,
                      double* out_host);
int femfct_assemble_weighted_mass(femfct_ctx* ctx, const double* f_dev, double* out_ell);
int femfct_traj_info(femfct_ctx* ctx, femfct_step_info* info_host, int32_t num_steps, int32_t batch);


int femfct_l2_norm_sq_Q(femfct_ctx* ctx, const double* a_dev, const double* b_dev, int32_t num_steps,
                        double dt, double* out_host, int32_t batch);
int femfct_l2_norm_sq_Omega(femfct_ctx* ctx, const double* a_dev, const double* b_dev, double* out_host,
                            int32_t batch);
int femfct_cost_functional(femfct_ctx* ctx, const double* var1, const double* var1_target,
                           const double* control, int32_t control_shared, int32_t num_steps, double dt,
                           double beta, int32_t finaltime, const double* var2, const double* var2_target,
                           double* J_host, int32_t batch);
int femfct_project_control(femfct_ctx* ctx, const double* c_dev, double s, const double* d_dev,
                           double c_lower, double c_upper, double* out_dev, int64_t count);

#define FEMFCT_MAX_TRIALS 16
int femfct_linear_trial_costs(femfct_ctx* ctx, const double* u_dev, const double* w_dev, const double* uhat_dev,
                              const double* c_dev, const double* d_dev, double s0, int32_t K, double c_lower,
                              double c_upper, double beta, int32_t num_steps, double dt, int32_t finaltime,
                              double* J_host, double* dist_host);
int femfct_source_trials(femfct_ctx* ctx, const double* c_dev, const double* d_dev, const double* g_dev, double s0,
                         int32_t K, double c_lower, double c_upper, int64_t count, double* c_out_dev,
                         double* src_out_dev);

#define FEMFCT_MAX_MEMBERS 256
int femfct_trial_controls(femfct_ctx* ctx, const double* c_dev, const double* d_dev, const double* steps_host, int32_t P,
                          int32_t K, double c_lower, double c_upper, int64_t count, double* c_out_dev);
int femfct_member_costs(femfct_ctx* ctx, const double* u_traj, const double* uhat, int32_t uhat_per_problem,
                        const double* c_traj, const double* cref, const double* beta_host, int32_t P, int32_t K,
                        int32_t num_steps, double dt, int32_t finaltime, double* J_host, double* dist_host);

int femfct_time_restrict(femfct_ctx* ctx, const double* x_traj, const int32_t* starts_host, int32_t K, int32_t num_steps,
                         int32_t batch, double* out_dev);
int femfct_time_prolong(femfct_ctx* ctx, const double* y_dev, const int32_t* starts_host, int32_t K, int32_t num_steps,
                        int32_t batch, double* out_traj);

int femfct_free_set(femfct_ctx* ctx, const double* c_dev, const double* g_dev, double c_lower, double c_upper, int64_t count,
                    uint8_t* mask_dev);
#define FEMFCT_MAX_GRAM_FIELDS 17
int femfct_q_gram(femfct_ctx* ctx, const double* const* fields_host, int32_t J, const uint8_t* mask_dev, int32_t num_steps,
                  double dt, double* G_host);
int femfct_q_combine(femfct_ctx* ctx, const double* const* fields_host, const double* coef_host, int32_t J,
                     const uint8_t* mask_dev, const double* fallback_dev, double fallback_scale, int64_t count,
                     double* out_dev);

int femfct_prox_trials(femfct_ctx* ctx, const double* c_dev, const double* d_dev, const double* g_dev, double s0, int32_t K,
                       double alpha, double c_lower, double c_upper, int64_t count, double* c_out_dev, double* src_out_dev);
int femfct_l1_norm_Q(femfct_ctx* ctx, const double* a_dev, int32_t num_steps, double dt, double* out_host, int32_t batch);
// ... 109 lines not shown
```

Measured before the change: 33320 timesteps/s.

## Trim tile kernel epilogues with per-wave partials and relaxed atomic write-through stores

Adds a tile-trim mode, on by default, with two parts. Only the waves that own output nodes now do a wave-level reduction and write their own partial slots, so the tile Jacobi and build-Jacobi kernels skip the block-wide reduction and its __syncthreads; the deferred convergence test then reads the larger set of per-wave partials through a new wide loader. Output stores can also go through agent-scope relaxed atomic stores, presumably so cross-workgroup readers in the fused pipeline see them directly. The cost is more partial slots to reduce downstream, extra template instantiations, and a new graph-cache key bit.

```diff
diff --git a/fem-fct-pdeco_amd/_lib.py b/fem-fct-pdeco_amd/_lib.py
--- a/fem-fct-pdeco_amd/_lib.py
+++ b/fem-fct-pdeco_amd/_lib.py
@@ -71,6 +71,7 @@
     "femfct_graph_replay_active": (C.c_int, [_p, C.POINTER(C.c_int)]),
     "femfct_rotation_derived": (C.c_int, [_p, C.POINTER(C.c_int)]),
     "femfct_launch_info": (C.c_int, [_p, C.POINTER(C.c_int32)]),
+    "femfct_tile_trim_info": (C.c_int, [_p, C.POINTER(C.c_int32)]),
     "femfct_set_fusion": (C.c_int, [_p, C.c_int, C.c_int]),
     "femfct_kernel_regime": (C.c_int, [_p, _i]),
     "femfct_patch_walkers": (C.c_int, [_p, _i, _i]),
diff --git a/fem-fct-pdeco_amd/csrc/ctx.hip b/fem-fct-pdeco_amd/csrc/ctx.hip
--- a/fem-fct-pdeco_amd/csrc/ctx.hip
+++ b/fem-fct-pdeco_amd/csrc/ctx.hip
@@ -263,6 +263,7 @@
     if (const char* e = getenv("FEMFCT_TILE_LEAN")) ctx->tile_lean = atoi(e) != 0;
     if (const char* e = getenv("FEMFCT_TILE_CONE")) ctx->tile_cone = atoi(e) != 0;
     if (const char* e = getenv("FEMFCT_TILE_FIT")) ctx->tile_fit = atoi(e) != 0;
+    if (const char* e = getenv("FEMFCT_TILE_TRIM")) ctx->tile_trim = atoi(e);
     if (const char* e = getenv("FEMFCT_FUSE_END")) ctx->fuse_end = atoi(e) != 0;
     if (const char* e = getenv("FEMFCT_TILE4")) ctx->tile4_mode = atoi(e);
     if (const char* e = getenv("FEMFCT_LMASK")) ctx->l_mask = atoi(e) != 0;
@@ -465,6 +466,13 @@
 int femfct_launch_info(const femfct_ctx* ctx, int32_t* out4_host) {
     if (!ctx || !out4_host) return FEMFCT_ERR_INVALID;
     for (int k = 0; k < 4; ++k) out4_host[k] = ctx->last_launch[k];
+    return FEMFCT_OK;
+}
+
+int femfct_tile_trim_info(const femfct_ctx* ctx, int32_t* out4_host) {
+    if (!ctx || !out4_host) return FEMFCT_ERR_INVALID;
+    out4_host[0] = femfct_tile_trim_mask(ctx);
+    for (int k = 0; k < 3; ++k) out4_host[k + 1] = ctx->trim_seen[k];
     return FEMFCT_OK;
 }
 
diff --git a/fem-fct-pdeco_amd/csrc/femfct_internal.h b/fem-fct-pdeco_amd/csrc/femfct_internal.h
--- a/fem-fct-pdeco_amd/csrc/femfct_internal.h
+++ b/fem-fct-pdeco_amd/csrc/femfct_internal.h
@@ -11,6 +11,8 @@
 #include "../../include/femfct.h"
 
 #define FEMFCT_MAX_W 16
+enum { TILE_TRIM_WAVES = 1, TILE_TRIM_WT = 8 };
+#define TILE_TRIM_DEFAULT (TILE_TRIM_WAVES | TILE_TRIM_WT)
 #ifndef FEMFCT_MAX_PARTIALS
 #define FEMFCT_MAX_PARTIALS 2048
 #endif
@@ -125,6 +127,8 @@
     int tile_lean = 1;
     int tile_cone = 0;
     int tile_fit = 1;
+    int tile_trim = TILE_TRIM_DEFAULT;
+    int32_t trim_seen[3] = {0, 0, 0};
     bool exact_iters = false;
     int32_t bandwidth = 0;
     int32_t strip_k = 0;
@@ -258,6 +262,8 @@
                               int32_t batch);
 
 struct TilePlan { int tiles, K, H; };
+int femfct_tile_trim_mask(const femfct_ctx* ctx);
+int femfct_tile_wave_slots(const femfct_ctx* ctx, const TilePlan& pl);
 bool femfct_tile_plan(const femfct_ctx* ctx, TilePlan* pl, bool need_partials = true, int budget = 0, int batch = 1);
 bool femfct_tile_big(const femfct_ctx* ctx, const TilePlan& pl);
 bool femfct_cheb_flux_fusable(const femfct_ctx* ctx, int32_t batch);
@@ -268,14 +274,16 @@
 bool femfct_geom_mass(const femfct_ctx* ctx);
 int femfct_enqueue_tile_build_jacobi(femfct_ctx* ctx, const TilePlan& pl, struct MatRef A, const double* Nm, int32_t nshared,
                                      struct VecRef rhs, int64_t rhs_bstride, struct VecRef u_n, int64_t u_bstride, double dt,
-                                     int32_t batch, bool pre = false);
+                                     int32_t batch, bool pre = false, bool wave_slots = false);
 int femfct_enqueue_low_seq(femfct_ctx* ctx, const double* A, double* L, double* D, int32_t entries, double dt);
 int femfct_enqueue_tile_jacobi(femfct_ctx* ctx, const TilePlan& pl, const double* L, const double* b, double* xa,
-                               double* xb, int launch, int g_build, int32_t batch, bool last, int bn_launch = 0, int defer = 0);
+                               double* xb, int launch, int g_build, int32_t batch, bool last, int bn_launch = 0, int defer = 0,
+                               bool wave_slots = false);
 __attribute__((visibility("hidden"))) void femfct_launch_reduce_resid(femfct_ctx* ctx, int64_t count, int launch, int32_t batch);
 int femfct_enqueue_tile_dudt_cheb(femfct_ctx* ctx, struct MatRef A, struct VecRef rhs, int64_t rhs_bstride, double* ulow,
                                   int budget_units, int part_count, int iters_per_unit, int exact_k, int iters,
-                                  const double* omegas, double md_scale, int32_t batch, int* tail_first = nullptr);
+                                  const double* omegas, double md_scale, int32_t batch, int* tail_first = nullptr,
+                                  bool wave_slots = false);
 int femfct_enqueue_tile_cheb(femfct_ctx* ctx, const TilePlan& pl, const double* b, const double* in_mid,
                              const double* in_old, double* y_out, int k_first, int k_last, const double* omegas,
                              double md_scale, double* bufA0, double* bufA1, double* bufB0, double* bufB1, int32_t batch,
diff --git a/fem-fct-pdeco_amd/csrc/kernels_step.hip b/fem-fct-pdeco_amd/csrc/kernels_step.hip
--- a/fem-fct-pdeco_amd/csrc/kernels_step.hip
+++ b/fem-fct-pdeco_amd/csrc/kernels_step.hip
@@ -609,6 +609,7 @@
     const bool tiles = femfct_tile_plan(ctx, &tp, false, budget, batch) && (!femfct_tile_big(ctx, tp) || ctx->d_bigpart);
     const bool strips = !tiles && femfct_strip_plan(ctx, &pl);
     int units = budget, part_count = 0, ipu = 1, exact_k = 0;
+    bool wave_slots_used = false;
     const bool tile4 = tiles && femfct_tile4_wanted(ctx, batch);
     const bool fused_build = ctx->fuse_build && tiles && !tile4 && !femfct_tile_big(ctx, tp) &&
                              ctx->solver != FEMFCT_SOLVER_BICGSTAB && (budget + tp.K - 1) / tp.K >= 2;
@@ -663,15 +664,18 @@
         exact_k = (femfct_tile_big(ctx, tp) || !ctx->exact_iters) ? 0 : tp.K;
         const bool defer = ctx->defer_check && fused_build && units >= 2 && units <= 4 && exact_k == 0 && ctx->fuse_dudt;
         if (defer) exact_k = -units;
+        const int wave_slots = defer ? femfct_tile_wave_slots(ctx, tp) : 0;
+        if (defer) ctx->trim_seen[2] = wave_slots;
+        if (wave_slots) { part_count = wave_slots; wave_slots_used = true; }
         if (fused_build) {
             int r = femfct_enqueue_tile_build_jacobi(ctx, tp, pre_low ? L_pre : A, N, nshared, rhs, rhs_bstride, u_n, u_bstride,
-                                                     dt, batch, pre_low);
+                                                     dt, batch, pre_low, wave_slots_used);
             if (r != FEMFCT_OK) return r;
         }
         for (int s = fused_build ? 1 : 0; s < units; ++s)
             femfct_enqueue_tile_jacobi(ctx, tp, ctx->d_L, ctx->d_b, ctx->d_xa, ctx->d_xb, s,
                                        fused_build ? tp.tiles * tp.tiles : (int)g.grid.x, batch,
-                                       exact_k > 0 && s == units - 1, fused_build ? 1 : 0, defer ? 1 : 0);
+                                       exact_k > 0 && s == units - 1, fused_build ? 1 : 0, defer ? 1 : 0, wave_slots_used);
     } else if (strips) {
         units = (budget + pl.K - 1) / pl.K;
         part_count = pl.S;
@@ -690,8 +694,9 @@
         cheb_omegas(20, 0.5, 2.0, om);
         int tail = 0;
         const bool fuse_tail = femfct_cheb_flux_fusable(ctx, batch);
-        femfct_enqueue_tile_dudt_cheb(ctx, A, rhs, rhs_bstride, ulow, units, part_count, ipu, exact_k, 20, om.data(), 1.25,
-                                      batch, fuse_tail ? &tail : nullptr);
+        int rd = femfct_enqueue_tile_dudt_cheb(ctx, A, rhs, rhs_bstride, ulow, units, part_count, ipu, exact_k, 20, om.data(), 1.25,
+                                               batch, fuse_tail ? &tail : nullptr, wave_slots_used);
+        if (rd != FEMFCT_OK) return rd;
         if (fuse_tail && tail > 0) {
             const bool fuse_end = ctx->end_req_delta != 0 && ctx->d_ticket && ctx->d_level && ctx->d_log && !ctx->prof_on;
             int r = femfct_enqueue_tile_cheb_flux_limit(ctx, ctx->d_rdu, ctx->d_y0, ctx->d_y2, tail, 20, om.data(), 1.25,
diff --git a/fem-fct-pdeco_amd/csrc/kernels_tile32.hip b/fem-fct-pdeco_amd/csrc/kernels_tile32.hip
--- a/fem-fct-pdeco_amd/csrc/kernels_tile32.hip
+++ b/fem-fct-pdeco_amd/csrc/kernels_tile32.hip
@@ -16,20 +16,29 @@
 namespace {
 
 #ifdef FEMFCT_TUNING
-__device__ unsigned long long g_tile_phase[4][4];
-#define TILE_STAMP_BEGIN()                                                                                              \
-    unsigned long long ts0_ = 0, ts1_ = 0;                                                                              \
-    const bool ts_on_ = threadIdx.x == 0 && blockIdx.z == 0 && blockIdx.x == gridDim.x / 2 && blockIdx.y == gridDim.x / 2; \
-    if (ts_on_) ts0_ = __builtin_amdgcn_s_memrealtime()
+__device__ unsigned long long g_tile_phase[4][6];
+#define TILE_STAMP_BEGIN(thread)                                                                                        \
+    unsigned long long ts0_ = 0, ts1_ = 0, ts3_ = 0, ts4_ = 0;                                                          \
+    const bool ts_on_ = (int)threadIdx.x == (thread) / WAVE * WAVE && blockIdx.z == 0 && blockIdx.x == gridDim.x / 2 && blockIdx.y == gridDim.x / 2; \
+    if (ts_on_) ts0_ = ts3_ = ts4_ = __builtin_amdgcn_s_memrealtime()
 #define TILE_STAMP_LOADED() do { if (ts_on_) { __builtin_amdgcn_s_waitcnt(0); ts1_ = __builtin_amdgcn_s_memrealtime(); } } while (0)
+#define TILE_STAMP_SWEPT() do { if (ts_on_) ts3_ = __builtin_amdgcn_s_memrealtime(); } while (0)
+#define TILE_STAMP_FLUXES() do { if (ts_on_) ts4_ = __builtin_amdgcn_s_memrealtime(); } while (0)
 #define TILE_STAMP_END(id) do { if (ts_on_) {                                                                           \
         const unsigned long long ts2_ = __builtin_amdgcn_s_memrealtime();                                               \
-        g_tile_phase[id][0] += ts1_ - ts0_; g_tile_phase[id][1] += ts2_ - ts0_; g_tile_phase[id][2] += 1; } } while (0)
+        g_tile_phase[id][0] += ts1_ - ts0_; g_tile_phase[id][1] += ts2_ - ts0_; g_tile_phase[id][2] += 1;               \
+        g_tile_phase[id][3] += ts3_ - ts0_; g_tile_phase[id][4] += ts4_ - ts0_; } } while (0)
 #else
-#define TILE_STAMP_BEGIN() do { } while (0)
+#define TILE_STAMP_BEGIN(thread) do { } while (0)
 #define TILE_STAMP_LOADED() do { } while (0)
+#define TILE_STAMP_SWEPT() do { } while (0)
+#define TILE_STAMP_FLUXES() do { } while (0)
 #define TILE_STAMP_END(id) do { } while (0)
 #endif
+
+#define TILE_OUT(lvalue, value) do {                                                                                    \
+        if constexpr ((TRIM & 8) != 0) __hip_atomic_store(&(lvalue), (value), __ATOMIC_RELAXED, __HIP_MEMORY_SCOPE_AGENT); \
+        else (lvalue) = (value); } while (0)
 
 struct TileGeom {
     int lx, ly, gx, gy, i;
@@ -79,6 +88,13 @@
     return PL * PL % WAVE != 0 && threadIdx.x >= PL * PL;
 }
 
+__host__ __device__ constexpr int tile_owning_waves(int H) { return (TILE_L - 1 - H) / 2 - H / 2 + 1; }
+template <int H>
+__device__ __forceinline__ int tile_owning_wave() {
+    const int w = __builtin_amdgcn_readfirstlane((int)threadIdx.x / WAVE) - H / 2;
+    return w < tile_owning_waves(H) ? w : -1;
+}
+
 template <int H, int PL = TILE_L>
 __device__ __forceinline__ int tile_dist(const TileGeom& g) {
     constexpr int T = PL - 2 * H;
@@ -162,13 +178,15 @@
     __syncthreads();
 }
 
-template <int H, int EXACT, int BIG, int LEAN>
+template <int H, int EXACT, int BIG, int LEAN, int TRIM = 0>
 __global__ void __launch_bounds__(STRIP_T)
 k_tile_jacobi(int n, int N, const double* __restrict__ L_, const double* __restrict__ b_, double* __restrict__ xa_,
               double* __restrict__ xb_, double* __restrict__ part, StepCtl* __restrict__ ctl_, int launch, int K,
               int g_build, double rel_tol, double* __restrict__ bigpart, double* __restrict__ partk, int bn_launch,
               int defer) {
     constexpr int W = 7;
+    static_assert(!TRIM || (LEAN == 1 && !BIG), "trimmed launches: lean loops");
+    static_assert(!(TRIM & 1) || !EXACT, "owning-wave epilogue: deferred test");
     __shared__ double xs[2][TILE_L * TILE_LD];
     __shared__ double smem[96];
     const int bz = blockIdx.z;
@@ -221,7 +239,7 @@
     const double* L = L_ + moff;
     const double* xin = ((launch & 1) ? xb_ : xa_) + voff;
     double* xout = ((launch & 1) ? xa_ : xb_) + voff;
-    TILE_STAMP_BEGIN();
+    TILE_STAMP_BEGIN(H * TILE_L + H);
     const TileGeom g = tile_geom<TILE_L - 2 * H, H>(N);
     constexpr bool CONE = LEAN == 2;
     double lv[W - 1], dg = 1.0, rdg = 1.0, bv = 0.0, xi = 0.0;
@@ -271,6 +289,7 @@
             __syncthreads();
             cur ^= 1;
         }
+        TILE_STAMP_SWEPT();
     } else {
         double rk[H];
 #pragma unroll
@@ -320,7 +339,17 @@
             partk[((int64_t)bz * 16 + threadIdx.x) * FEMFCT_MAX_PARTIALS + wg] = v;
         }
     }
-    if (g.owned) xout[g.i] = LEAN ? xo : xs[cur][g.self];
+    if (g.owned) TILE_OUT(xout[g.i], LEAN ? xo : xs[cur][g.self]);
+    if constexpr (TRIM & 1) {
+        const int ow = tile_owning_wave<H>();
+        if (ow >= 0) {
+            rmax = wave_reduce(rmax, OpMax());
+            if (threadIdx.x % WAVE == 0)
+                partk[((int64_t)bz * 16 + launch) * FEMFCT_MAX_PARTIALS + wg * tile_owning_waves(H) + ow] = rmax;
+        }
+        TILE_STAMP_END(1);
+        return;
+    }
     rmax = block_reduce(rmax, OpMax(), 0.0, smem);
     if (threadIdx.x == 0) {
         if (BIG) bigpart[(int64_t)bz * nwg + wg] = rmax;
@@ -330,7 +359,7 @@
     TILE_STAMP_END(1);
 }
 
-template <int H, int PRE, int LEAN>
+template <int H, int PRE, int LEAN, int TRIM = 0>
 __global__ void __launch_bounds__(STRIP_T)
 k_tile_build_jacobi(int n, int N, MatRef A_ref, const double* __restrict__ N_, int nshared,
                     VecRef rhs_ref, int64_t rhs_bstride, VecRef u_ref, int64_t u_bstride,
@@ -338,6 +367,7 @@
                     double* __restrict__ b_, double* __restrict__ xb_, double* __restrict__ part,
                     StepCtl* __restrict__ ctl_, int K) {
     constexpr int W = 7;
+    static_assert(!TRIM || LEAN == 1, "trimmed launches: lean loops");
     __shared__ double xs[2][TILE_L * TILE_LD];
     __shared__ double as[PRE ? 1 : 3][TILE_L * TILE_LD];
     __shared__ double smem[96];
@@ -355,7 +385,7 @@
     const double* rhs = vec_ptr(rhs_ref);
     if (rhs) rhs += bz * rhs_bstride;
     const double* u = vec_ptr(u_ref) + bz * u_bstride;
-    TILE_STAMP_BEGIN();
+    TILE_STAMP_BEGIN(H * TILE_L + H);
     const TileGeom g = tile_geom<TILE_L - 2 * H, H>(N);
     double lv[W - 1], dv[W - 1], dsum = 0.0, rs = 0.0;
     double dg = 1.0, rdg = 1.0, bv = 0.0, xi = 0.0;
@@ -447,16 +477,16 @@
     double bmax = 0.0, rsmin = INFINITY;
     if (g.owned) {
         double* L = L_ + moff;
-        L[g.i] = dg;
-#pragma unroll
-        for (int s = 1; s < W; ++s) L[(int64_t)s * n + g.i] = lv[s - 1];
+        TILE_OUT(L[g.i], dg);
+#pragma unroll
+        for (int s = 1; s < W; ++s) TILE_OUT(L[(int64_t)s * n + g.i], lv[s - 1]);
         if constexpr (!PRE) {
             double* D = D_ + moff;
             D[g.i] = -dsum;
 #pragma unroll
             for (int s = 1; s < W; ++s) D[(int64_t)s * n + g.i] = dv[s - 1];
         }
-        b_[voff + g.i] = bv;
+        TILE_OUT(b_[voff + g.i], bv);
         bmax = fabs(bv);
         rsmin = rs;
     }
@@ -483,7 +513,24 @@
         __syncthreads();
         cur ^= 1;
     }
-    if (g.owned) xb_[voff + g.i] = LEAN ? xo : xs[cur][g.self];
+    TILE_STAMP_SWEPT();
+    if (g.owned) TILE_OUT(xb_[voff + g.i], LEAN ? xo : xs[cur][g.self]);
+    if constexpr (TRIM & 1) {
+        const int ow = tile_owning_wave<H>();
+        if (ow >= 0) {
+            rmax = wave_reduce(rmax, OpMax());
+            bmax = wave_reduce(bmax, OpMax());
+            rsmin = wave_reduce(rsmin, OpMin());
+            if (threadIdx.x % WAVE == 0) {
+                const int slot = wg * tile_owning_waves(H) + ow;
+                p[slot] = rmax;
+                p[2 * FEMFCT_MAX_PARTIALS + slot] = bmax;
+                p[3 * FEMFCT_MAX_PARTIALS + slot] = rsmin;
+            }
+        }
+        TILE_STAMP_END(0);
+        return;
+    }
     block_reduce_max_max_min(rmax, bmax, rsmin, smem);
     if (threadIdx.x == 0) {
         p[wg] = rmax;
@@ -709,7 +756,7 @@
     if (FL_L == 16) step_end_by_last_workgroup(e);
 }
 
-template <int GEOM, int LEAN, int PL>
+template <int GEOM, int LEAN, int PL, int TRIM = 0>
 __global__ void __launch_bounds__((PL * PL + WAVE - 1) / WAVE * WAVE, (LEAN && PL == TILE_L) ? 8 : 1)
 k_tile_cheb_flux_limit(int n, int N, double h, const double* __restrict__ M, const double* __restrict__ b_,
                        const double* __restrict__ ymid_, const double* __restrict__ yold_, int K, CheOmegas om,
@@ -718,12 +765,13 @@
     constexpr int W = 7, HH = 12, PLD = PL + 1;
     constexpr bool CONE = LEAN == 2;
     static_assert(PL == TILE_L || LEAN, "fitted patches run the lean loops only");
+    static_assert(!TRIM || LEAN == 1, "trimmed launches: lean loops");
     __shared__ double ys[LEAN ? 2 : 3][PL * PLD];
     __shared__ double su[PL * PLD], srp[PL * PLD], srm[PL * PLD];
     const int bz = blockIdx.z;
     const int64_t voff = (int64_t)bz * n;
     const double* D_ = mat_ptr(D_ref, bz);
-    TILE_STAMP_BEGIN();
+    TILE_STAMP_BEGIN(HH * PL + HH);
     const TileGeom g = tile_geom<PL - 2 * HH, HH, PL>(N);
     double mv[W - 1], dv[W - 1], md = 1.0, rmd = 1.0, bv = 0.0, ym = 0.0, yo = 0.0, ui = 0.0, mli = 1.0;
 #pragma unroll
@@ -813,6 +861,7 @@
         __syncthreads();
         int t = io; io = im; im = in_; in_ = t;
     }
+    TILE_STAMP_SWEPT();
     const double* sd = ys[im];
     const double dui = LEAN ? ym : sd[g.self];
     double f[W - 1];
@@ -835,6 +884,7 @@
         srm[g.self] = (pm != 0.0) ? fmin(1.0, mli * qm / (dt * pm)) : 1.0;
     }
     __syncthreads();
+    TILE_STAMP_FLUXES();
     if (g.owned) {
         const double rpi = srp[g.self], rmi = srm[g.self];
         double fbar = 0.0;
@@ -845,13 +895,13 @@
             fbar += a * fs;
         }
         double* out = const_cast<double*>(vec_ptr(out_ref)) + bz * out_bstride;
-        out[g.i] = ui + dt * fbar / mli;
+        TILE_OUT(out[g.i], ui + dt * fbar / mli);
     }
     TILE_STAMP_END(3);
     step_end_by_last_workgroup(e);
 }
 
-template <int LEAN, int GEOM, int PL>
+template <int LEAN, int GEOM, int PL, int TRIM = 0>
 __global__ void __launch_bounds__((PL * PL + WAVE - 1) / WAVE * WAVE)
 k_tile_dudt_cheb(int n, int N, double h, MatRef A_ref, VecRef rhs_ref, int64_t rhs_bstride,
                  const double* __restrict__ M, const double* __restrict__ xa_, const double* __restrict__ xb_,
@@ -862,6 +912,7 @@
     constexpr int W = 7, H = 10, PLD = PL + 1;
     constexpr bool CONE = LEAN == 2;
     static_assert(PL == TILE_L || LEAN, "fitted patches run the lean loops only");
+    static_assert(!TRIM || LEAN == 1, "trimmed launches: lean loops");
     __shared__ double ys[LEAN ? 2 : 3][PL * PLD];
     __shared__ double smem[64];
     const int bz = blockIdx.z;
@@ -869,9 +920,13 @@
     double* p = part + (int64_t)bz * 4 * FEMFCT_MAX_PARTIALS;
     const int wg = blockIdx.y * gridDim.x + blockIdx.x;
     if (exact_k < 0 && blockIdx.y == gridDim.x) {
-        if (blockIdx.x == 0)
-            deferred_test_publish(ctl, deferred_test_load(p, partk + (int64_t)bz * 16 * FEMFCT_MAX_PARTIALS, part_count, -exact_k),
-                                  -exact_k, iters_per_unit, rel_tol);
+        if (blockIdx.x == 0) {
+            const double* pk = partk + (int64_t)bz * 16 * FEMFCT_MAX_PARTIALS;
+            if constexpr (TRIM & 1)
+                deferred_test_publish(ctl, deferred_test_load_wide(p, pk, part_count, -exact_k, &ys[0][0]), -exact_k, iters_per_unit, rel_tol);
+            else
+                deferred_test_publish(ctl, deferred_test_load(p, pk, part_count, -exact_k), -exact_k, iters_per_unit, rel_tol);
+        }
         return;
     }
     const int parity = exact_k < 0 ? (budget & 1) : ctl->done ? ctl->parity : (budget & 1);
@@ -883,7 +938,7 @@
     const double* x = (parity ? xb_ : xa_) + voff;
     const double* rhs = vec_ptr(rhs_ref);
     if (rhs) rhs += bz * rhs_bstride;
-    TILE_STAMP_BEGIN();
+    TILE_STAMP_BEGIN(H * PL + H);
     const TileGeom g = tile_geom<PL - 2 * H, H, PL>(N);
     double av[W], mv[W - 1], md = 1.0, rmd = 1.0, ui = 0.0, ri = 0.0;
 #pragma unroll
@@ -957,11 +1012,12 @@
             lean_cheb_iter<0, PL>(a, live(k + 1), mv, md, rmd, r, om.w[k + 1], ym, yo);
         }
         if (k < K) lean_cheb_iter<1, PL>(a, live(k), mv, md, rmd, r, om.w[k], ym, yo);
+        TILE_STAMP_SWEPT();
         if (g.owned) {
-            ulow_[voff + g.i] = ui;
-            rdu_[voff + g.i] = r;
-            omid_[voff + g.i] = ym;
-            if (oold_) oold_[voff + g.i] = yo;
+            TILE_OUT(ulow_[voff + g.i], ui);
+            TILE_OUT(rdu_[voff + g.i], r);
+            TILE_OUT(omid_[voff + g.i], ym);
+            if (oold_) TILE_OUT(oold_[voff + g.i], yo);
         }
         TILE_STAMP_END(2);
         return;
@@ -987,6 +1043,7 @@
         __syncthreads();
         int t = io; io = im; im = in_; in_ = t;
     }
+    TILE_STAMP_SWEPT();
     if (g.owned) {
         ulow_[voff + g.i] = ui;
         rdu_[voff + g.i] = r;
@@ -1001,13 +1058,15 @@
 #ifdef FEMFCT_TUNING
 void femfct_tile_phase_dump(const char* path) {
     static const char* names[4] = {"k_tile_build_jacobi", "k_tile_jacobi", "k_tile_dudt_cheb", "k_tile_cheb_flux_limit"};
-    unsigned long long h[4][4];
+    unsigned long long h[4][6];
     if (hipMemcpyFromSymbol(h, HIP_SYMBOL(g_tile_phase), sizeof(h)) != hipSuccess) return;
     if (FILE* f = fopen(path, "a")) {
         for (int k = 0; k < 4; ++k)
             if (h[k][2])
-                fprintf(f, "%-24s launches %8llu  load phase %7.3f us  whole kernel %7.3f us  share %5.1f %%\n", names[k], h[k][2],
-                        0.01 * h[k][0] / h[k][2], 0.01 * h[k][1] / h[k][2], 100.0 * h[k][0] / (double)h[k][1]);
+                fprintf(f, "%-24s launches %8llu  load phase %7.3f us  whole kernel %7.3f us  share %5.1f %%  after the last sweep %6.3f us"
+                        "  (limiter: after the fluxes' barrier %6.3f us)\n", names[k], h[k][2], 0.01 * h[k][0] / h[k][2],
+                        0.01 * h[k][1] / h[k][2], 100.0 * h[k][0] / (double)h[k][1], 0.01 * (h[k][1] - h[k][3]) / h[k][2],
+                        k == 3 ? 0.01 * (h[k][1] - h[k][4]) / h[k][2] : 0.0);
         fclose(f);
     }
     memset(h, 0, sizeof(h));
@@ -1018,10 +1077,35 @@
 
 static int tile_lean_mode(const femfct_ctx* ctx) { return ctx->tile_lean ? (ctx->tile_cone ? 2 : 1) : 0; }
 
+static int tile_trim_mode(const femfct_ctx* ctx) { return tile_lean_mode(ctx) == 1 ? ctx->tile_trim & (TILE_TRIM_WAVES | TILE_TRIM_WT) : 0; }
+int femfct_tile_trim_mask(const femfct_ctx* ctx) { return tile_trim_mode(ctx); }
+static void tile_trim_count(femfct_ctx* ctx, int trim) {
+    if (trim & TILE_TRIM_WAVES) ctx->trim_seen[0] = 1;
+    if (trim & TILE_TRIM_WT) ctx->trim_seen[1] = 1;
+}
+
+template <class F>
+static void with_trim(int trim, F&& f) {
+    switch (trim) {
+    case TILE_TRIM_WAVES: f(std::integral_constant<int, TILE_TRIM_WAVES>()); break;
+    case TILE_TRIM_WT: f(std::integral_constant<int, TILE_TRIM_WT>()); break;
+    case TILE_TRIM_WAVES | TILE_TRIM_WT: f(std::integral_constant<int, TILE_TRIM_WAVES | TILE_TRIM_WT>()); break;
+    default: f(std::integral_constant<int, 0>()); break;
+    }
+}
+
+int femfct_tile_wave_slots(const femfct_ctx* ctx, const TilePlan& pl) {
+    if (!(tile_trim_mode(ctx) & TILE_TRIM_WAVES)) return 0;
+    const int64_t slots = (int64_t)pl.tiles * pl.tiles * tile_owning_waves(pl.H);
+    return slots <= FEMFCT_MAX_PARTIALS ? (int)slots : 0;
+}
+
 int femfct_enqueue_tile_build_jacobi(femfct_ctx* ctx, const TilePlan& pl, MatRef A, const double* Nm, int32_t nshared,
                                      VecRef rhs, int64_t rhs_bstride, VecRef u_n, int64_t u_bstride, double dt,
-                                     int32_t batch, bool pre) {
+                                     int32_t batch, bool pre, bool wave_slots) {
     if (pre && Nm) return femfct_fail(ctx, FEMFCT_ERR_INVALID, "pre-built low-order operator with a non-flux matrix");
+    const int trim = tile_trim_mode(ctx) & ((wave_slots ? TILE_TRIM_WAVES : 0) | TILE_TRIM_WT);
+    tile_trim_count(ctx, trim);
     dim3 grid(pl.tiles, pl.tiles, batch);
     femfct_prof_begin(ctx, KC_JACOBI);
     auto go = [&](auto kernel) {
@@ -1030,6 +1114,13 @@
     };
     with_constant<8, TILE_HMAX>(pl.H, [&](auto h) {
         constexpr int H = decltype(h)::value;
+        if (trim) {
+            with_trim(trim, [&](auto t) {
+                constexpr int TRIM = decltype(t)::value;
+                if (pre) go(k_tile_build_jacobi<H, 1, 1, TRIM>); else go(k_tile_build_jacobi<H, 0, 1, TRIM>);
+            });
+            return;
+        }
         with_constant<0, 2>(tile_lean_mode(ctx), [&](auto l) {
             constexpr int LEAN = decltype(l)::value;
             if (pre) go(k_tile_build_jacobi<H, 1, LEAN>); else go(k_tile_build_jacobi<H, 0, LEAN>);
@@ -1050,8 +1141,10 @@
 }
 
 int femfct_enqueue_tile_jacobi(femfct_ctx* ctx, const TilePlan& pl, const double* L, const double* b, double* xa,
-                               double* xb, int launch, int g_build, int32_t batch, bool last, int bn_launch, int defer) {
+                               double* xb, int launch, int g_build, int32_t batch, bool last, int bn_launch, int defer, bool wave_slots) {
     const bool big = femfct_tile_big(ctx, pl);
+    const int trim = big ? 0 : tile_trim_mode(ctx) & (((wave_slots && defer) ? TILE_TRIM_WAVES : 0) | TILE_TRIM_WT);
+    tile_trim_count(ctx, trim);
     double* bigp = big ? ctx->d_bigpart : nullptr;
     double* pk = ((last || defer) && !big) ? ctx->d_partk : nullptr;
     dim3 grid(pl.tiles, pl.tiles, batch);
@@ -1068,6 +1161,16 @@
         } else {
             with_constant<8, TILE_HMAX>(pl.H, [&](auto h) {
                 constexpr int H = decltype(h)::value;
+                if constexpr (LEAN == 1) {
+                    if (trim) {
+                        with_trim(trim, [&](auto t) {
+                            constexpr int TRIM = decltype(t)::value;
+                            if constexpr (!(TRIM & TILE_TRIM_WAVES)) { if (pk && !defer) { go(k_tile_jacobi<H, 1, 0, 1, TRIM>, 0); return; } }
+                            go(k_tile_jacobi<H, 0, 0, 1, TRIM>, defer);
+                        });
+                        return;
+                    }
+                }
                 if (pk && !defer) go(k_tile_jacobi<H, 1, 0, LEAN>, 0); else go(k_tile_jacobi<H, 0, 0, LEAN>, defer);
             });
         }
@@ -1082,8 +1185,12 @@
 
 int femfct_enqueue_tile_dudt_cheb(femfct_ctx* ctx, MatRef A, VecRef rhs, int64_t rhs_bstride, double* ulow,
                                   int budget_units, int part_count, int iters_per_unit, int exact_k, int iters,
-                                  const double* omegas, double md_scale, int32_t batch, int* tail_first) {
+                                  const double* omegas, double md_scale, int32_t batch, int* tail_first, bool wave_slots) {
     constexpr int H = 10;
+    const int trim = tile_trim_mode(ctx) & (((wave_slots && exact_k < 0) ? TILE_TRIM_WAVES : 0) | TILE_TRIM_WT);
+    if (wave_slots && !(tile_trim_mode(ctx) & TILE_TRIM_WAVES))
+        return femfct_fail(ctx, FEMFCT_ERR_INVALID, "per-wave partials outside the trimmed lean launches");
+    tile_trim_count(ctx, trim);
     const int T = TILE_L - 2 * H, t = (ctx->N + T - 1) / T;
     const bool fit = femfct_tile_fit(ctx, batch);
     const int tl = fit ? (ctx->N + 5) / 6 : t;
@@ -1102,7 +1209,12 @@
     };
     with_constant<0, 1>(ctx->tile_lean && femfct_geom_mass(ctx), [&](auto gm) {
         constexpr int GM = decltype(gm)::value;
-        if (fit) {
+        if (trim) {
+            with_trim(trim, [&](auto t) {
+                constexpr int TRIM = decltype(t)::value;
+                if (fit) go(k_tile_dudt_cheb<1, GM, 26, TRIM>, 26); else go(k_tile_dudt_cheb<1, GM, TILE_L, TRIM>, TILE_L);
+            });
+        } else if (fit) {
             if (ctx->tile_cone) go(k_tile_dudt_cheb<2, GM, 26>, 26); else go(k_tile_dudt_cheb<1, GM, 26>, 26);
         } else if constexpr (GM) {
             if (ctx->tile_cone) go(k_tile_dudt_cheb<2, 1, TILE_L>, TILE_L); else go(k_tile_dudt_cheb<1, 1, TILE_L>, TILE_L);
@@ -1168,6 +1280,8 @@
     for (int k = k_first; k <= k_last; ++k) om.w[k - k_first] = omegas[k - 1];
     const bool fit = femfct_tile_fit(ctx, batch);
     const int t = fit ? (ctx->N + 5) / 6 : (ctx->N + 7) / 8;
+    const bool wt = (tile_trim_mode(ctx) & TILE_TRIM_WT) != 0;
+    tile_trim_count(ctx, wt ? TILE_TRIM_WT : 0);
     femfct_prof_begin(ctx, KC_FLUX);
     auto go = [&](auto kernel, int PL) {
         hipLaunchKernelGGL(kernel, dim3(t, t, batch), dim3((PL * PL + WAVE - 1) / WAVE * WAVE), 0, ctx->stream, ctx->n, ctx->N,
@@ -1175,7 +1289,10 @@
     };
     with_constant<0, 1>(femfct_geom_mass(ctx), [&](auto gm) {
         constexpr int GM = decltype(gm)::value;
-        if (fit) {
+        if (wt) {
+            if (fit) go(k_tile_cheb_flux_limit<GM, 1, 30, TILE_TRIM_WT>, 30);
+            else go(k_tile_cheb_flux_limit<GM, 1, TILE_L, TILE_TRIM_WT>, TILE_L);
+        } else if (fit) {
             if (ctx->tile_cone) go(k_tile_cheb_flux_limit<GM, 2, 30>, 30); else go(k_tile_cheb_flux_limit<GM, 1, 30>, 30);
         } else {
             with_constant<0, 2>(tile_lean_mode(ctx), [&](auto l) { go(k_tile_cheb_flux_limit<GM, decltype(l)::value, TILE_L>, TILE_L); });
diff --git a/fem-fct-pdeco_amd/csrc/solve_ctl.h b/fem-fct-pdeco_amd/csrc/solve_ctl.h
--- a/fem-fct-pdeco_amd/csrc/solve_ctl.h
+++ b/fem-fct-pdeco_amd/csrc/solve_ctl.h
@@ -21,6 +21,43 @@
             d.bn = nan_max(d.bn, p[2 * FEMFCT_MAX_PARTIALS + k]);
             d.rs = nan_min(d.rs, p[3 * FEMFCT_MAX_PARTIALS + k]);
         }
+    }
+    return d;
+}
+
+__device__ __forceinline__ DeferredPartials deferred_test_load_wide(const double* p, const double* partk, int S, int units,
+                                                                    double* lds) {
+    static_assert(FEMFCT_DEFER_MAX_UNITS + 2 == 6, "lds layout");
+    DeferredPartials d;
+#pragma unroll
+    for (int s = 0; s < FEMFCT_DEFER_MAX_UNITS; ++s) d.r[s] = 0.0;
+    d.bn = 0.0; d.rs = INFINITY;
+#pragma unroll 2
+    for (int k = threadIdx.x; k < S; k += blockDim.x) {
+        d.r[0] = nan_max(d.r[0], p[k]);
+#pragma unroll
+        for (int s = 1; s < FEMFCT_DEFER_MAX_UNITS; ++s)
+            if (s < units) d.r[s] = nan_max(d.r[s], partk[(int64_t)s * FEMFCT_MAX_PARTIALS + k]);
+        d.bn = nan_max(d.bn, p[2 * FEMFCT_MAX_PARTIALS + k]);
+        d.rs = nan_min(d.rs, p[3 * FEMFCT_MAX_PARTIALS + k]);
+    }
+    const int wid = threadIdx.x / WAVE, nw = (blockDim.x + WAVE - 1) / WAVE;
+#pragma unroll
+    for (int s = 0; s < FEMFCT_DEFER_MAX_UNITS; ++s) d.r[s] = wave_reduce(d.r[s], OpMax());
+    d.bn = wave_reduce(d.bn, OpMax());
+    d.rs = wave_reduce(d.rs, OpMin());
+    if (threadIdx.x % WAVE == 0) {
+#pragma unroll
+        for (int s = 0; s < FEMFCT_DEFER_MAX_UNITS; ++s) lds[6 * wid + s] = d.r[s];
+        lds[6 * wid + 4] = d.bn;
+        lds[6 * wid + 5] = d.rs;
+    }
+    __syncthreads();
+    if ((int)threadIdx.x < nw) {
+#pragma unroll
+        for (int s = 0; s < FEMFCT_DEFER_MAX_UNITS; ++s) d.r[s] = lds[6 * threadIdx.x + s];
+        d.bn = lds[6 * threadIdx.x + 4];
+        d.rs = lds[6 * threadIdx.x + 5];
     }
     return d;
 }
diff --git a/fem-fct-pdeco_amd/csrc/traj_common.h b/fem-fct-pdeco_amd/csrc/traj_common.h
--- a/fem-fct-pdeco_amd/csrc/traj_common.h
+++ b/fem-fct-pdeco_amd/csrc/traj_common.h
@@ -42,7 +42,7 @@
     key.push_back(key_bits((int32_t)ctx->solver));
     key.push_back(key_bits(ctx->low_src));
     key.push_back(key_bits(ctx->low_dt));
-    key.push_back(key_bits((int32_t)(ctx->tile_lean | ctx->tile_cone << 1 | ctx->tile_fit << 2)));
+    key.push_back(key_bits((int32_t)(ctx->tile_lean | ctx->tile_cone << 1 | ctx->tile_fit << 2 | femfct_tile_trim_mask(ctx) << 3)));
     struct Restore {
         femfct_ctx* c;
         ~Restore() { c->level_bias = 0; c->ord_bias = 0; c->rep_total = 1; c->rep_last = true; }
diff --git a/fem-fct-pdeco_amd/device.py b/fem-fct-pdeco_amd/device.py
--- a/fem-fct-pdeco_amd/device.py
+++ b/fem-fct-pdeco_amd/device.py
@@ -141,6 +141,11 @@
         kinds = {0: "other", 1: "k_strip4_jacobi", 2: "k_strip4_jacobi_walk", 3: "k_strip_jacobi_pair_walk"}
         return {"jacobi_kernel": kinds.get(out[0], "?"), "jacobi_walkers": int(out[1]), "cheb_interior_patches": int(out[2]),
                 "halo": int(out[3])}
+
+    def tile_trim_info(self) -> dict:
+        out = (C.c_int32 * 4)()
+        check(self.handle, lib.femfct_tile_trim_info(self.handle, out))
+        return {"mask": int(out[0]), "wave_launches": int(out[1]), "wt_launches": int(out[2]), "wave_slots": int(out[3])}
 
     def graph_replay_active(self) -> bool:
         v = C.c_int(0)
diff --git a/include/femfct.h b/include/femfct.h
--- a/include/femfct.h
+++ b/include/femfct.h
@@ -47,6 +47,7 @@
 int         femfct_set_solver(femfct_ctx* ctx, int solver, double rel_tol, int max_iters);
 int         femfct_set_graphs(femfct_ctx* ctx, int enable);
 int         femfct_launch_info(const femfct_ctx* ctx, int32_t* out4_host);
+int         femfct_tile_trim_info(const femfct_ctx* ctx, int32_t* out4_host);
 int         femfct_graph_replay_active(const femfct_ctx* ctx, int* active_host);
 int         femfct_rotation_derived(const femfct_ctx* ctx, int* derived_host);
 int         femfct_set_fusion(femfct_ctx* ctx, int strips, int tiles);
```

Measured after the change: 37520 timesteps/s (median of 6 runs). 1.13x the previous value.
